# Bioconductor/SparseArray

Hardware: AMD Instinct MI355X
Metric: GNZ/s, SVT crossprod(svt, dense) 1e6x1e4 @1% nnz (higher is better)
Workload: dtype f64

## Files before the change

include/svt_hip.h:

```cpp
#ifndef SVT_HIP_H
#define SVT_HIP_H

#include <stddef.h>
#include <stdint.h>

#ifdef __cplusplus
extern "C" {
#endif

#define SVT_UNSUPPORTED 1

#define SVT_LGLSXP 10
#define SVT_INTSXP 13
#define SVT_REALSXP 14

#define SVT_OP_ANYNA            1
#define SVT_OP_COUNTNAS         2
#define SVT_OP_ANY              3
#define SVT_OP_ALL              4
#define SVT_OP_MIN              5
#define SVT_OP_MAX              6
#define SVT_OP_RANGE            7
#define SVT_OP_SUM              8
#define SVT_OP_PROD             9
// ... 78 lines not shown
int svt_colsum_SVT(const svt_view *x, const int *group, int ngroup, int na_rm,
		   void *out, int *ovflow);
int svt_rowsum_dgCMatrix(int nrow, int ncol, const double *xx, const int *xi,
			 const int *xp, const int *group, int ngroup,
			 int na_rm, double *out);
int svt_colsum_dgCMatrix(int nrow, int ncol, const double *xx, const int *xi,
			 const int *xp, const int *group, int ngroup,
			 int na_rm, double *out);

int svt_colMins_dgCMatrix(int nrow, int ncol, const double *xx, const int *xp,
			  int na_rm, double *out);
int svt_colMaxs_dgCMatrix(int nrow, int ncol, const double *xx, const int *xp,
			  int na_rm, double *out);
int svt_colRanges_dgCMatrix(int nrow, int ncol, const double *xx, const int *xp,
			    int na_rm, double *out);
int svt_colVars_dgCMatrix(int nrow, int ncol, const double *xx, const int *xp,
			  int na_rm, double *out);


typedef struct svt_dev_csc {
	int32_t Rtype;
	int32_t owned;
	int64_t nrow;
	int64_t ncol;
	int64_t nnz;
	int64_t *col_ptr;
	int32_t *row_idx;
	void *val;
	int32_t na_background;
} svt_dev_csc;

svt_dev_csc *svt_upload(const svt_view *x);
svt_dev_csc *svt_wrap_device_csc(int Rtype, int64_t nrow, int64_t ncol,
				 int64_t nnz, int64_t *col_ptr,
				 int32_t *row_idx, void *val);
void svt_release(svt_dev_csc *h);

size_t svt_dev_crossprod_ws_bytes(int64_t nrow, int64_t ncol, int K);
int svt_dev_dense_prepare(const void *Y, int64_t ldY, int64_t nrow, int K,
			  int tr_y, int Rtype, void *ws, size_t ws_bytes,
			  void *stream);
int svt_dev_crossprod_prepared(const svt_dev_csc *A, const void *ws, int K,
			       double *out, int64_t out_stride_c,
			       int64_t out_stride_k, void *stream);
int svt_dev_crossprod_csc_dense(const svt_dev_csc *A, const void *Y,
				int64_t ldY, int K, int tr_y, double *out,
				int64_t out_stride_c, int64_t out_stride_k,
				void *ws, size_t ws_bytes, void *stream);

typedef struct svt_dev_pbc svt_dev_pbc;
svt_dev_pbc *svt_dev_pbc_build(const svt_dev_csc *A, int CBW, int WPB, int logR);
void svt_dev_pbc_release(svt_dev_pbc *P);
void svt_dev_pbc_trim(void);
size_t svt_dev_pbc_bytes(const svt_dev_pbc *P);
size_t svt_dev_crossprod_pbc_ws_bytes(const svt_dev_pbc *P, int K);
int svt_dev_crossprod_pbc(const svt_dev_pbc *P, const svt_dev_csc *A,
			  const double *Y, int64_t ldY, int K, int tr_y,
			  double *out, int64_t out_stride_c,
			  int64_t out_stride_k, void *ws, size_t ws_bytes,
			  void *stream);

void svt_dev_pbc_set_spare_cus(int n);
int svt_dev_pbc_spare_cus(void);

void svt_dev_pbc_set_gather_pacing(int dsync, int spin);

void svt_dev_pbc_set_round_launches(int on);

int svt_dev_crossprod_pbc_from(const svt_dev_pbc *P, const svt_dev_csc *A,
			       const double *Y, int64_t ldY, int K, int tr_y,
			       double *out, int64_t out_stride_c,
			       int64_t out_stride_k, void *ws, size_t ws_bytes,
			       void *stream, int64_t first_col);

enum { SVT_PBC_KERNEL_GENERAL = 0, SVT_PBC_KERNEL_DMA = 1, SVT_PBC_KERNEL_GATHER = 2, SVT_PBC_KERNEL_GATHER2 = 3,
       SVT_PBC_KERNEL_GATHERX = 4 };
typedef struct svt_pbc_plan {
	int kind, kernel, NV, nsplit;
	int64_t panels_per_split;
	int direct, launches, tail_splits, tail_blocks;
} svt_pbc_plan;
int svt_dev_crossprod_pbc_plan(const svt_dev_pbc *P, int K, int tr_y, int64_t out_stride_c,
			       int64_t out_stride_k, int64_t first_col, svt_pbc_plan *plan);

int svt_dev_crossprod_pbc_phase(const svt_dev_pbc *P, const svt_dev_csc *A,
				const double *Y, int64_t ldY, int K, int tr_y,
				double *out, int64_t out_stride_c,
				int64_t out_stride_k, void *ws, size_t ws_bytes,
				void *stream, int phase);

int svt_dev_colstats(const svt_dev_csc *A, int opcode, int na_rm,
		     double center, int64_t inner, void *out, int *warn_flag,
		     void *stream);

int svt_dev_colstats_form(int64_t nseg, int64_t nnz, int *nchunk);

size_t svt_dev_colmedians_ws_bytes(int64_t nnz, int64_t ncol);
int svt_dev_colmedians(const svt_dev_csc *A, int na_rm, double *out, void *ws, size_t ws_bytes,
		       void *stream);

size_t svt_dev_colquantiles_ws_bytes(int64_t nnz, int64_t ncol, int nprobs);
int svt_dev_colquantiles(const svt_dev_csc *A, const double *probs, int nprobs, int na_rm,
			 double *out, void *ws, size_t ws_bytes, void *stream);

size_t svt_dev_colmads_ws_bytes(int64_t nnz, int64_t ncol);
int svt_dev_colmads(const svt_dev_csc *A, const double *center , double constant,
// ... 96 lines not shown
```

sparsearray_amd/_abi.py:

```python
from ctypes import CFUNCTYPE, c_char_p, c_double as D, c_int as I, c_int64 as L, c_size_t as Z, c_void_p as P

ALLOC_FN = CFUNCTYPE(P, Z, P)
FREE_FN = CFUNCTYPE(None, P, P)

PROTOTYPES = {
    "svt_init": (I, [I]),
    "svt_last_error": (c_char_p, []),
    "svt_device_arch": (c_char_p, []),
    "svt_set_devices": (I, [P, I]),
    "svt_get_devices": (I, [P, I]),
    "svt_set_shard_min_nnz": (None, [L]),
    "svt_resident_set_limit": (I, [Z]),
    "svt_resident_clear": (None, []),
    "svt_resident_stats": (None, [P, P, P, P]),
    "svt_crossprod2_SVT_mat": (I, [P, P, I, I, I, I, P]),
    "svt_crossprod2_mat_SVT": (I, [P, I, I, I, P, I, P]),
    "svt_crossprod2_SVT_SVT": (I, [P, P, P]),
    "svt_crossprod1_SVT": (I, [P, P]),
    "svt_matmul_SVT_mat": (I, [P, P, I, I, I, P]),
    "svt_matmul_SVT_SVT": (I, [P, P, P]),
    "svt_tcrossprod1_SVT": (I, [P, P]),
    "svt_tcrossprod2_SVT_SVT": (I, [P, P, P]),
    "svt_colMedians_SVT": (I, [P, I, P]),
    "svt_rowMedians_SVT": (I, [P, I, P]),
    "svt_colQuantiles_SVT": (I, [P, P, I, I, P]),
    "svt_rowQuantiles_SVT": (I, [P, P, I, I, P]),
    "svt_colMads_SVT": (I, [P, P, D, I, P]),
    "svt_rowMads_SVT": (I, [P, P, D, I, P]),
    "svt_colRanks_SVT": (I, [P, I, I, P]),
    "svt_rowRanks_SVT": (I, [P, I, P]),
    "svt_summarize_SVT": (I, [P, I, I, D, P, P, P, P]),
    "svt_colStats_out_Rtype": (I, [I, I]),
    "svt_colStats_SVT": (I, [P, I, I, D, I, P, P]),
    "svt_rowStats_SVT": (I, [P, I, I, P, I, P, P]),
    "svt_rowStatsFull_SVT": (I, [P, I, I, P, I, P, P]),
    "svt_rowsum_SVT": (I, [P, P, I, I, P, P]),
    "svt_colsum_SVT": (I, [P, P, I, I, P, P]),
    "svt_rowsum_dgCMatrix": (I, [I, I, P, P, P, P, I, I, P]),
    "svt_colsum_dgCMatrix": (I, [I, I, P, P, P, P, I, I, P]),
    "svt_colMins_dgCMatrix": (I, [I, I, P, P, I, P]),
    "svt_colMaxs_dgCMatrix": (I, [I, I, P, P, I, P]),
    "svt_colRanges_dgCMatrix": (I, [I, I, P, P, I, P]),
    "svt_colVars_dgCMatrix": (I, [I, I, P, P, I, P]),
    "svt_upload": (P, [P]),
    "svt_wrap_device_csc": (P, [I, L, L, L, P, P, P]),
    "svt_release": (None, [P]),
    "svt_dev_crossprod_ws_bytes": (Z, [L, L, I]),
    "svt_dev_dense_prepare": (I, [P, L, L, I, I, I, P, Z, P]),
    "svt_dev_crossprod_prepared": (I, [P, P, I, P, L, L, P]),
    "svt_dev_crossprod_csc_dense": (I, [P, P, L, I, I, P, L, L, P, Z, P]),
    "svt_dev_pbc_build": (P, [P, I, I, I]),
    "svt_dev_pbc_release": (None, [P]),
    "svt_dev_pbc_trim": (None, []),
    "svt_dev_pbc_bytes": (Z, [P]),
    "svt_dev_crossprod_pbc_ws_bytes": (Z, [P, I]),
    "svt_dev_crossprod_pbc": (I, [P, P, P, L, I, I, P, L, L, P, Z, P]),
    "svt_dev_pbc_set_spare_cus": (None, [I]),
    "svt_dev_pbc_spare_cus": (I, []),
    "svt_dev_pbc_set_gather_pacing": (None, [I, I]),
    "svt_dev_pbc_set_round_launches": (None, [I]),
    "svt_dev_crossprod_pbc_from": (I, [P, P, P, L, I, I, P, L, L, P, Z, P, L]),
    "svt_dev_crossprod_pbc_plan": (I, [P, I, I, L, L, L, P]),
    "svt_dev_crossprod_pbc_phase": (I, [P, P, P, L, I, I, P, L, L, P, Z, P, I]),
    "svt_dev_colstats": (I, [P, I, I, D, L, P, P, P]),
    "svt_dev_colstats_form": (I, [L, L, P]),
    "svt_dev_colmedians_ws_bytes": (Z, [L, L]),
    "svt_dev_colmedians": (I, [P, I, P, P, Z, P]),
    "svt_dev_colquantiles_ws_bytes": (Z, [L, L, I]),
    "svt_dev_colquantiles": (I, [P, P, I, I, P, P, Z, P]),
    "svt_dev_colmads_ws_bytes": (Z, [L, L]),
    "svt_dev_colmads": (I, [P, P, D, I, P, P, Z, P]),
    "svt_dev_colranks_form": (I, [L]),
    "svt_dev_colranks_ws_bytes": (Z, [L, L]),
    "svt_dev_colranks": (I, [P, I, P, P, P, P, Z, P]),
    "svt_dev_rowstats_ws_bytes": (Z, [L, L]),
    "svt_dev_rowsums": (I, [P, I, L, P, P, Z, P]),
    "svt_dev_rowsums_prepare": (I, [P, L, P, Z, P]),
    "svt_dev_rowsums_prepared": (I, [P, I, L, P, P, Z, P]),
    "svt_dev_rowstats_ws_bytes_op": (Z, [P, I, L]),
    "svt_dev_rowstats": (I, [P, I, I, P, L, P, P, P, Z, P]),
    "svt_dev_rowstats_form": (I, [L, L, L, I, I, L, P, P]),
    "svt_dev_rowsum": (I, [P, P, I, I, P, P]),
    "svt_dev_rowsum_gid_bytes": (Z, [P]),
    "svt_dev_rowsum_prepare": (I, [P, P, I, P, Z, P]),
    "svt_dev_rowsum_prepared": (I, [P, P, I, I, P, P]),
    "svt_get_num_procs": (I, []),
    "svt_get_max_threads": (I, []),
    "svt_set_max_threads": (I, [I]),
    "svt_dev_transpose_ws_bytes": (Z, [L, L]),
    "svt_dev_transpose": (I, [P, P, P, P, P, Z, P]),
    "svt_dev_transpose_plan": (I, [L, L, L, L, P]),
    "svt_dev_set_box_nnz": (None, [L]),
    "svt_dev_boxed_calls": (L, [I]),
    "svt_dev_matmul_csc_csc_ws_bytes": (Z, [P]),
    "svt_dev_matmul_csc_csc": (I, [P, P, P, L, P, Z, P, P]),
    "svt_dev_matmul_csc_csc_prepare": (I, [P, P, Z, P]),
    "svt_dev_matmul_csc_csc_prepared": (I, [P, P, P, L, P, Z, P, P]),
    "svt_dev_crossprod_csc_csc_ws_bytes": (Z, [P]),
    "svt_dev_crossprod_csc_csc": (I, [P, P, I, P, L, P, Z, P, P]),
    "svt_dev_crossprod_csc_csc_set_panel": (None, [I, I]),
    "svt_dev_crossprod_csc_csc_dense_buffer": (I, [P, P, P]),
    "svt_sparse_crossprod_set_cost": (None, [D]),
    "svt_dev_aperm_ws_bytes": (Z, [L, I, P]),
    "svt_dev_aperm_perm_ws_bytes": (Z, [L, I, P, P]),
    "svt_dev_aperm": (I, [P, I, P, P, P, P, P, P, Z, P]),
    "svt_dev_aperm_route_counts": (None, [P, I]),
# ... 15 lines not shown
```

sparsearray_amd/csrc/kernels_colstats.hip:

```cpp
#include "svt_common.h"

#define F_NA    1
#define F_NAN   2
#define F_TRUE  4
#define F_ZERO  8
#define F_HAVE 16

template <typename V, typename F>
__device__ inline V grp16(V v, F f)
{
#pragma unroll
	for (int m = 8; m >= 1; m >>= 1) v = f(v, __shfl_xor(v, m, SVT_WAVE));
	return v;
}

template <int NT>
__device__ inline double red_sum(double v, double *sm)
{
	if (NT == 16) return grp16(v, [](double a, double b) { return a + b; });
	v = wave_sum(v);
	if (NT == SVT_WAVE)
		return __shfl(v, 0, SVT_WAVE);
	const int w = threadIdx.x >> 6, l = threadIdx.x & 63;
	__syncthreads();
// ... 444 lines not shown
template <typename T>
__global__ void __launch_bounds__(256)
colstats_thread_kernel(StatsArgs a)
{
	typedef ValTraits<T> VT;
	const bool is_dbl = sizeof(T) == 8;
	const int64_t g = (int64_t) blockIdx.x * blockDim.x + threadIdx.x;
	if (g >= a.nseg) return;
	const T *__restrict__ val = (const T *) a.val;
	const int64_t beg = a.col_ptr[g * a.inner], end = a.col_ptr[(g + 1) * a.inner];
	const int oc = a.opcode;
	const bool narm = a.na_rm != 0;
	const bool is_minmax = oc == SVT_OP_MIN || oc == SVT_OP_MAX, is_min = oc == SVT_OP_MIN;
	ColState st;
	st.flags = 0; st.pad = 0; st.nacnt = 0;
	st.acc = (oc == SVT_OP_PROD) ? 1.0 : 0.0;
	st.mm = is_min ? INFINITY : -INFINITY;
	for (int64_t k = beg; k < end; k++) {
		const T v = val[k];
		if (VT::is_missing(v)) {
			st.nacnt++;
			st.flags |= VT::is_na(v) ? F_NA : F_NAN;
			if (narm || !is_dbl) continue;
		} else {
			st.flags |= (v != (T) 0) ? F_TRUE : F_ZERO;
			st.flags |= F_HAVE;
		}
		const double d = VT::as_double(v);
		if (oc == SVT_OP_PROD) st.acc *= d;
		else if (is_minmax) { if (d == d) st.mm = is_min ? (d < st.mm ? d : st.mm) : (d > st.mm ? d : st.mm); }
		else st.acc += d;
	}
	double c = 0.0, acc2 = 0.0;
	if (oc == SVT_OP_CENTERED_X2_SUM || oc == SVT_OP_VAR1 || oc == SVT_OP_SD1) {
		c = colstats_center(a, st, end - beg);
		for (int64_t k = beg; k < end; k++) {
			const T v = val[k];
			if (VT::is_missing(v) && (narm || !is_dbl)) continue;
			const double d = VT::as_double(v) - c;
			acc2 += d * d;
		}
	}
	colstats_final(a, g, st, end - beg, c, acc2, is_dbl);
}

static int launch_colstats_split(const StatsArgs &a, int nchunk, hipStream_t s)
{
	const bool is_dbl = a.Rtype == SVT_REALSXP;
	const bool two_pass = a.opcode == SVT_OP_CENTERED_X2_SUM || a.opcode == SVT_OP_VAR1 ||
			      a.opcode == SVT_OP_SD1;
	const size_t n = (size_t) a.nseg * nchunk;
	const size_t b_st = (n * sizeof(ColState) + 255) / 256 * 256, b_c = ((size_t) a.nseg * 8 + 255) / 256 * 256;
	char *scr = NULL;
	HIP_TRY(hipMallocAsync((void **) &scr, b_st + b_c + n * 8 + 256, s));
	ColState *st = (ColState *) scr;
	double *centers = (double *) (scr + b_st), *acc2 = (double *) (scr + b_st + b_c);
	dim3 grid((unsigned) nchunk, (unsigned) a.nseg), cgrid((unsigned) ((a.nseg + 255) / 256));
	if (is_dbl) hipLaunchKernelGGL((colstats_chunk_kernel<double, 1>), grid, dim3(256), 0, s, a, nchunk, st, centers, acc2);
	else hipLaunchKernelGGL((colstats_chunk_kernel<int, 1>), grid, dim3(256), 0, s, a, nchunk, st, centers, acc2);
	hipLaunchKernelGGL(colstats_combine_kernel<1>, cgrid, dim3(256), 0, s, a, nchunk, st, centers, acc2,
			   (int) two_pass, (int) is_dbl);
	if (two_pass) {
		if (is_dbl) hipLaunchKernelGGL((colstats_chunk_kernel<double, 2>), grid, dim3(256), 0, s, a, nchunk, st, centers, acc2);
		else hipLaunchKernelGGL((colstats_chunk_kernel<int, 2>), grid, dim3(256), 0, s, a, nchunk, st, centers, acc2);
		hipLaunchKernelGGL(colstats_combine_kernel<2>, cgrid, dim3(256), 0, s, a, nchunk, st, centers, acc2,
				   (int) two_pass, (int) is_dbl);
	}
	HIP_TRY(hipGetLastError());
	HIP_TRY(hipFreeAsync(scr, s));
	return 0;
}

ColStatsRoute colstats_route(int64_t nseg, int64_t nnz)
{
	ColStatsRoute rt = { COLSTATS_LANES16, 1 };
	if (nseg <= 0)
		return rt;
	const int64_t avg = nnz / nseg;
	if (nseg < 512 && avg >= 65536 && nseg <= 65535) {
		int64_t nchunk = (1024 + nseg - 1) / nseg;
		if (nchunk > avg / 16384) nchunk = avg / 16384;
		if (nchunk >= 2) {
			rt.form = COLSTATS_SPLIT;
			rt.nchunk = (int) nchunk;
			return rt;
		}
	}
	if (avg >= 1024)
		rt.form = avg <= 256 * 40 ? COLSTATS_GROUP_CACHED : COLSTATS_GROUP_STREAM;
	else if (avg < 4 && nseg >= 4096)
		rt.form = COLSTATS_THREAD;
	else if (avg < 160)
		rt.form = COLSTATS_LANES16;
	else
		rt.form = COLSTATS_WAVE;
	return rt;
}

template <int NT, int CAP>
static void launch_colstats_form(const StatsArgs &a, hipStream_t s)
{
	const dim3 grid((unsigned) ((a.nseg + 256 / NT - 1) / (256 / NT))), block(256);
	if (a.Rtype == SVT_REALSXP) hipLaunchKernelGGL((colstats_kernel<double, NT, CAP>), grid, block, 0, s, a);
	else hipLaunchKernelGGL((colstats_kernel<int, NT, CAP>), grid, block, 0, s, a);
}

int launch_colstats(const StatsArgs &a, int64_t nnz, hipStream_t s)
{
	if (a.nseg <= 0)
		return 0;
	if (a.nseg > 0x7FFFFFFFLL)
		return svt_set_error("too many generalized columns");
	const ColStatsRoute rt = colstats_route(a.nseg, nnz);
	switch (rt.form) {
	case COLSTATS_SPLIT:
		return launch_colstats_split(a, rt.nchunk, s);
	case COLSTATS_GROUP_CACHED: launch_colstats_form<256, 48>(a, s); break;
	case COLSTATS_GROUP_STREAM: launch_colstats_form<256, 0>(a, s); break;
	case COLSTATS_WAVE: launch_colstats_form<64, 16>(a, s); break;
	case COLSTATS_LANES16: launch_colstats_form<16, 16>(a, s); break;
	case COLSTATS_THREAD: {
		const dim3 gridt((unsigned) ((a.nseg + 255) / 256)), block(256);
// ... 9 lines not shown
```

sparsearray_amd/csrc/kernels_mult_pbc.hip:

```cpp
#include "svt_common.h"

#include <string.h>

#include <mutex>

#include "svt_scan.h"

typedef double d16 __attribute__((ext_vector_type(16)));
typedef double d8 __attribute__((ext_vector_type(8)));

struct svt_dev_pbc {
	int64_t nrow, ncol, nnz, nrec;
	int CBW, WPB, logR;
	int kind;
	int64_t ngroups, nblocks, npanels;
	uint4 *rec;
	int64_t *tile_ptr;
	int *col_has_na;
	int64_t max_leaf_nnz;
	mutable hipStream_t use_s[4];
	mutable int nuse;
	mutable bool use_overflow;
	int device;
};
// ... 325 lines not shown
	}
	__syncthreads();
	if (tid < np) {
		const int start = s_tile0[tid], stop = s_tile0[tid + 1];
		uint32_t *last = (uint32_t *) (dst + ((stop - 8) >> 3) * 96);
		*last |= 0x8000u;
		const int w = (int) (g % 16);
		const int nb = (stop - start) >> 3;
		int bi = (int) pbc_stagger_batch(stag_mode, w, nb);
		if (bi > nb - 1) bi = nb - 1;
		uint32_t *issue = (uint32_t *) (dst + ((start >> 3) + bi) * 96);
		*issue |= 0x4000u;
	}
	if (!in_lds)
		return;
	__syncthreads();
	uint4 *out = (uint4 *) (rec + (base >> 3) * 96);
	for (int64_t i = tid; i < nbytes / 16; i += 256) out[i] = ((const uint4 *) img)[i];
}

__global__ void pbc_max_leaf_kernel(const int64_t *__restrict__ col_ptr, int64_t ncol, unsigned long long *__restrict__ out)
{
	unsigned long long n = 0ULL;
	for (int64_t c = (int64_t) blockIdx.x * blockDim.x + threadIdx.x; c < ncol; c += (int64_t) gridDim.x * blockDim.x) {
		const unsigned long long m = (unsigned long long) (col_ptr[c + 1] - col_ptr[c]);
		n = m > n ? m : n;
	}
	for (int off = 32; off > 0; off >>= 1) {
		const unsigned long long o = __shfl_xor(n, off, 64);
		n = o > n ? o : n;
	}
	if ((threadIdx.x & 63) == 0 && n > 0) atomicMax(out, n);
}

__global__ void pbc_group_limit_kernel(const int64_t *__restrict__ tile_ptr, int64_t npanels,
				       int64_t ngroups, int *__restrict__ flag)
{
	const int64_t g = (int64_t) blockIdx.x * blockDim.x + threadIdx.x;
	if (g >= ngroups) return;
	const int64_t n = tile_ptr[(g + 1) * npanels] - tile_ptr[g * npanels];
	if ((n + PBC_SLACK) * 16 >= ((int64_t) 1 << 32)) *flag = 1;
}

__global__ void pbc_build_finish_kernel(int64_t *__restrict__ tile_ptr, int64_t ntiles, char *__restrict__ rec,
					int rbytes, long long *__restrict__ meta)
{
	const int64_t nrec = tile_ptr[ntiles];
	if (threadIdx.x == 0) meta[0] = nrec;
	if (threadIdx.x < PBC_TP_PAD) tile_ptr[ntiles + 1 + threadIdx.x] = nrec;
	uint32_t *slack = (uint32_t *) (rec + (size_t) nrec * rbytes);
	for (int x = threadIdx.x; x < PBC_SLACK * 4; x += blockDim.x) slack[x] = 0u;
}

#define PBC_POOL_KEEP ((uint64_t) 3 << 30)
#define PBC_MAX_DEV 16
static hipMemPool_t g_pbc_pool[PBC_MAX_DEV];
static bool g_pbc_pool_ok[PBC_MAX_DEV];

static std::mutex g_pbc_pool_mu;

static hipMemPool_t pbc_pool(int dev)
{
	if (dev < 0 || dev >= PBC_MAX_DEV)
		return NULL;
	std::lock_guard<std::mutex> lk(g_pbc_pool_mu);
	if (!g_pbc_pool_ok[dev]) {
		hipMemPoolProps props;
		memset(&props, 0, sizeof(props));
		props.allocType = hipMemAllocationTypePinned;
		props.handleTypes = hipMemHandleTypeNone;
		props.location.type = hipMemLocationTypeDevice;
		props.location.id = dev;
		hipMemPool_t pool = NULL;
		if (hipMemPoolCreate(&pool, &props) != hipSuccess) {
			(void) hipGetLastError();
			return NULL;
		}
		uint64_t keep = PBC_POOL_KEEP;
		(void) hipMemPoolSetAttribute(pool, hipMemPoolAttrReleaseThreshold, &keep);
		g_pbc_pool[dev] = pool;
		g_pbc_pool_ok[dev] = true;
	}
	return g_pbc_pool[dev];
}

static hipError_t pbc_alloc(void **p, size_t n)
{
	int dev = 0;
	(void) hipGetDevice(&dev);
	hipMemPool_t pool = pbc_pool(dev);
	if (pool == NULL)
		return hipMallocAsync(p, n ? n : 16, 0);
	return hipMallocFromPoolAsync(p, n ? n : 16, pool, 0);
}
static void pbc_free(void *p) { if (p) (void) hipFreeAsync(p, 0); }

extern "C" void svt_dev_pbc_trim(void)
{
	for (int d = 0; d < PBC_MAX_DEV; d++)
		if (g_pbc_pool_ok[d])
			(void) hipMemPoolTrimTo(g_pbc_pool[d], 0);
}

static void pbc_note_use(const svt_dev_pbc *P, hipStream_t s)
{
	for (int i = 0; i < P->nuse; i++)
		if (P->use_s[i] == s) return;
	if (P->nuse == 4) { P->use_overflow = true; return; }
	P->use_s[P->nuse++] = s;
}

extern "C" void svt_dev_pbc_release(svt_dev_pbc *h)
{
	if (h == NULL) return;
	bool sync = h->use_overflow;
	for (int i = 0; i < h->nuse && !sync; i++) {
		if (h->use_s[i] == (hipStream_t) 0)
			continue;
		hipEvent_t ev;
		if (hipEventCreateWithFlags(&ev, hipEventDisableTiming) != hipSuccess) { sync = true; break; }
		if (hipEventRecord(ev, h->use_s[i]) != hipSuccess || hipStreamWaitEvent(0, ev, 0) != hipSuccess) {
			(void) hipGetLastError();
			sync = true;
		}
		(void) hipEventDestroy(ev);
	}
	if (sync)
		(void) hipDeviceSynchronize();
	pbc_free(h->rec);
	pbc_free(h->tile_ptr);
	pbc_free(h->col_has_na);
	free(h);
}

extern "C" size_t svt_dev_pbc_bytes(const svt_dev_pbc *h)
{
	if (h == NULL) return 0;
	return (size_t) h->nrec * (h->kind == PBC_KIND_DMA ? 12 : 16) + PBC_SLACK * 16 +
	       (size_t) (h->ngroups * h->npanels + 1 + PBC_TP_PAD) * 8 + (size_t) h->ncol * 4;
}

void pbc_auto_layout(int64_t nrow, int64_t ncol, int64_t nnz, int *CBW, int *WPB, int *logR)
{
	*CBW = 40;
	const double per_tile = (double) nnz * 40.0 * 128.0 /
				((double) (nrow > 0 ? nrow : 1) * (double) (ncol > 0 ? ncol : 1));
	if (per_tile < 12.0 && nrow >= 4096) {
		*WPB = 4;
		*logR = (nrow >> 11) >= 64 ? 11 : (nrow >> 10) >= 64 ? 10 : 9;
	} else { *WPB = 16; *logR = 7; }
}

int pbc_kind(int64_t nrow, int CBW, int WPB, int logR)
{
	if (CBW < 1 || CBW > 40)
		return PBC_KIND_BAD;
	if (WPB == 16 && logR == 7)
		return nrow >= 256 && nrow < ((int64_t) 1 << 28) ? PBC_KIND_DMA : PBC_KIND_NONE;
	return WPB == 4 && logR >= 9 && logR <= 15 ? PBC_KIND_GATHER : PBC_KIND_BAD;
}

extern "C" svt_dev_pbc *svt_dev_pbc_build(const svt_dev_csc *A, int CBW, int WPB, int logR)
{
	if (A->Rtype != SVT_REALSXP) {
		svt_set_error("svt_dev_pbc_build: f64 operands only");
		return NULL;
	}
	if (CBW == 0 && WPB == 0 && logR == 0)
		pbc_auto_layout(A->nrow, A->ncol, A->nnz, &CBW, &WPB, &logR);
	const int kind = pbc_kind(A->nrow, CBW, WPB, logR);
	if (kind == PBC_KIND_BAD) {
		svt_set_error("svt_dev_pbc_build: no product kernel reads the layout (CBW %d, WPB %d, logR %d): "
			      "(CBW <= 40, 16, 7) for the LDS-DMA kernel or (CBW <= 40, 4, 9 .. 15) for the gather kernels",
			      CBW, WPB, logR);
		return NULL;
	}
	svt_dev_pbc *h = (svt_dev_pbc *) calloc(1, sizeof(*h));
	h->nrow = A->nrow; h->ncol = A->ncol; h->nnz = A->nnz;
	h->CBW = CBW; h->WPB = WPB; h->logR = logR;
	h->kind = kind;
	const bool dma = kind == PBC_KIND_DMA;
// ... 36 lines not shown
				(void) hipFuncSetAttribute((const void *) pbc_count_stream_kernel,
							   hipFuncAttributeMaxDynamicSharedMemorySize, (int) lds);
				hipLaunchKernelGGL(pbc_count_stream_kernel, dim3((unsigned) h->ngroups), dim3(1024), lds, 0,
						   A->col_ptr, A->row_idx, A->ncol, CBW, logR, h->npanels, h->tile_ptr,
						   bounds, nchunks, logR + sl);
				bounds_done = true;
			}
		} else if (dma)
			hipLaunchKernelGGL((pbc_pass_kernel<0, 1>), grid, dim3(64), 0, 0, A->col_ptr, A->row_idx,
					   (const double *) A->val, A->ncol, CBW, logR, h->npanels,
					   h->tile_ptr, (uint4 *) NULL, h->col_has_na, g_pbc_stagger, 0);
		else
			hipLaunchKernelGGL((pbc_pass_kernel<0, 0>), grid, dim3(64), 0, 0, A->col_ptr, A->row_idx,
					   (const double *) A->val, A->ncol, CBW, logR, h->npanels,
					   h->tile_ptr, (uint4 *) NULL, h->col_has_na, g_pbc_stagger, 1);
		tmp_bytes = exclusive_scan_ws_bytes(ntiles + 1);
		ok = pbc_alloc(&tmp, tmp_bytes) == hipSuccess &&
		     launch_exclusive_scan_i64(h->tile_ptr, ntiles + 1, tmp, 0) == 0;
		if (ok) ok = pbc_alloc((void **) &h->rec, (size_t) nrec_max * rbytes + PBC_SLACK * 16) == hipSuccess;
		if (ok) {
			if (dma) {
				if (!bounds_done) ok = pbc_alloc((void **) &bounds, (size_t) nb_entries * 4) == hipSuccess;
				if (ok) {
					if (!bounds_done)
						hipLaunchKernelGGL(pbc_bounds_kernel, dim3((unsigned) ((nb_entries + 255) / 256)), dim3(256), 0, 0,
								   A->col_ptr, A->row_idx, A->ncol, nchunks, (int64_t) subp << logR, bounds);
					const size_t lds = PBC_IMG_BYTES + (size_t) 2 * subp * CBW * 4;
					(void) hipFuncSetAttribute((const void *) pbc_scatter_lds_kernel,
								   hipFuncAttributeMaxDynamicSharedMemorySize, (int) lds);
					dim3 sgrid((unsigned) h->ngroups, (unsigned) nchunks);
					hipLaunchKernelGGL(pbc_scatter_lds_kernel, sgrid, dim3(256), lds, 0, A->col_ptr, A->row_idx,
							   (const double *) A->val, A->ncol, CBW, logR, h->npanels,
							   h->tile_ptr, (char *) h->rec, h->col_has_na, g_pbc_stagger, subp,
							   bounds, nchunks);
				}
			} else {
				hipLaunchKernelGGL((pbc_pass_kernel<1, 0>), grid, dim3(64), 0, 0, A->col_ptr,
						   A->row_idx, (const double *) A->val, A->ncol, CBW, logR,
						   h->npanels, h->tile_ptr, h->rec, h->col_has_na, g_pbc_stagger, 1);
			}
		}
		long long hmeta[3] = {0, 0, 0};
		bool too_big = false;
		if (ok) {
			long long *meta = (long long *) tmp;
			ok = hipMemsetAsync(meta, 0, 24, 0) == hipSuccess;
			if (ok) {
				hipLaunchKernelGGL(pbc_max_leaf_kernel, dim3((unsigned) ((A->ncol + 255) / 256 < 512 ? (A->ncol + 255) / 256 : 512)), dim3(256), 0, 0,
						   A->col_ptr, A->ncol, (unsigned long long *) (meta + 1));
				hipLaunchKernelGGL(pbc_group_limit_kernel, dim3((unsigned) ((h->ngroups + 255) / 256)),
						   dim3(256), 0, 0, h->tile_ptr, h->npanels, h->ngroups, (int *) (meta + 2));
				hipLaunchKernelGGL(pbc_build_finish_kernel, dim3(1), dim3(256), 0, 0, h->tile_ptr, ntiles,
						   (char *) h->rec, (int) rbytes, meta);
				ok = hipMemcpy(hmeta, meta, 24, hipMemcpyDeviceToHost) == hipSuccess;
			}
			h->nrec = hmeta[0];
			h->max_leaf_nnz = hmeta[1];
			too_big = hmeta[2] != 0;
		}
		if (ok && too_big) {
			svt_set_error("svt_dev_pbc_build: a column group too large for 32-bit record offsets");
			pbc_free(tmp);
			pbc_free(bounds);
			svt_dev_pbc_release(h);
			return NULL;
		}
	}
	pbc_free(tmp);
	pbc_free(bounds);
	if (!ok) {
		svt_set_error("svt_dev_pbc_build failed: %s", hipGetErrorString(hipGetLastError()));
		svt_dev_pbc_release(h);
		return NULL;
	}
	return h;
}

static int g_pbc_spare_cus = 0;
extern "C" void svt_dev_pbc_set_spare_cus(int n)
{
	g_pbc_spare_cus = n < 0 ? 0 : n > 192 ? 192 : (n + 7) / 8 * 8;
}
extern "C" int svt_dev_pbc_spare_cus(void) { return g_pbc_spare_cus; }
#ifdef SVT_TUNING
extern "C" void svt_dev_pbc_set_debug(int mode)
{
	if (mode >= 300) g_pbc_ahead10 = mode - 300;
	else if (mode >= 200) g_pbc_stagger = mode - 200;
	else if (mode >= 100) g_pbc_nsplit = mode - 100;
	else g_pbc_debug = mode;
}
#endif

struct PbcFlags {
	int *y_nonfinite;
};

#define PBC_SUBFLAG0 16
#define PBC_NSUBFLAG 48
#define PBC_FLAG_BYTES 16384
#define PBC_PROG_OFFSET 8192
#ifdef SVT_TUNING
extern "C" int svt_dev_pbc_read_prof(const void *ws, unsigned long long *out)
{
	HIP_TRY(hipDeviceSynchronize());
	HIP_TRY(hipMemcpy(out, (const char *) ws + 7168, 16 * 8 * 8, hipMemcpyDeviceToHost));
// ... 1311 lines not shown
```

sparsearray_amd/csrc/kernels_rowstats.hip:

```cpp
#include "svt_common.h"

#define RF_NA   1
#define RF_NAN  2
#define RF_HAVE 4
#define RF_TRUE 8
#define RF_ZERO 16

struct MinMaxScratch {
	unsigned long long *best;
	int *flags;
	unsigned int *cov;
};

__host__ __device__ inline MinMaxScratch split_scratch(void *p, int64_t n)
{
	MinMaxScratch s;
	s.best = (unsigned long long *) p;
	s.flags = (int *) (s.best + n);
	s.cov = (unsigned int *) (s.flags + n);
	return s;
}

size_t rowstats_scratch_bytes(int opcode, int64_t out_len)
{
// ... 929 lines not shown
			}
			if (cur == NA_INT)
				continue;
			const long long y = (long long) cur + v;
			if (y > 2147483647LL || y < -2147483647LL) { out[r] = NA_INT; ov = 1; }
			else out[r] = (int) y;
		}
	}
	if (ov && a.ovflow_flag) *a.ovflow_flag = 1;
}

static int groupsum_common(const GroupSumArgs &a, int64_t out_len, bool colsum,
			   hipStream_t s)
{
	const bool is_dbl = a.Rtype == SVT_REALSXP;
	if (out_len <= 0)
		return 0;
	if (is_dbl)
		HIP_TRY(hipMemsetAsync(a.out, 0, (size_t) out_len * 8, s));
	else
		HIP_TRY(hipMemsetAsync(a.scratch, 0, groupsum_scratch_bytes(a.Rtype, out_len), s));
	if (a.ncol > 0) {
		const unsigned nb = (unsigned) ((a.ncol + 3) / 4);
		if (colsum) {
			if (is_dbl) hipLaunchKernelGGL((groupsum_atomic_kernel<double, 1>), dim3(nb), dim3(256), 0, s, a, out_len);
			else hipLaunchKernelGGL((groupsum_atomic_kernel<int, 1>), dim3(nb), dim3(256), 0, s, a, out_len);
		} else {
			if (is_dbl) hipLaunchKernelGGL((groupsum_atomic_kernel<double, 0>), dim3(nb), dim3(256), 0, s, a, out_len);
			else hipLaunchKernelGGL((groupsum_atomic_kernel<int, 0>), dim3(nb), dim3(256), 0, s, a, out_len);
		}
	}
	if (!is_dbl) {
		const int64_t col_len = colsum ? a.nrow : a.ngroup;
		const int64_t ncols_out = colsum ? a.ngroup : a.ncol;
		const unsigned nbo = (unsigned) ((out_len + 255) / 256);
		const unsigned nbc = (unsigned) ((ncols_out + 63) / 64);
		hipLaunchKernelGGL(groupsum_int_finish_kernel, dim3(nbo), dim3(256), 0, s, a, out_len, col_len);
		if (colsum) hipLaunchKernelGGL(groupsum_int_exact_kernel<1>, dim3(nbc), dim3(64), 0, s, a, out_len, ncols_out, col_len);
		else hipLaunchKernelGGL(groupsum_int_exact_kernel<0>, dim3(nbc), dim3(64), 0, s, a, out_len, ncols_out, col_len);
	}
	HIP_TRY(hipGetLastError());
	return 0;
}

__global__ void group16_kernel(const int *__restrict__ g, int64_t n, int ngroup, uint16_t *__restrict__ g16)
{
	const int64_t i = (int64_t) blockIdx.x * blockDim.x + threadIdx.x;
	if (i < n)
		g16[i] = (uint16_t) group_slot16(g[i], ngroup);
}

static int make_group16(const GroupSumArgs &a, uint16_t **g16, hipStream_t s)
{
	HIP_TRY(hipMallocAsync((void **) g16, (size_t) a.nrow * 2 + 16, s));
	hipLaunchKernelGGL(group16_kernel, dim3((unsigned) ((a.nrow + 255) / 256)), dim3(256), 0, s,
			   a.group, a.nrow, a.ngroup, *g16);
	return 0;
}

#define ROWSUM_WIN 49152
template <bool VALS, typename Use>
__device__ __forceinline__ void rowsum_window_walk(const int64_t *__restrict__ col_ptr, const int32_t *__restrict__ row_idx,
						   const double *__restrict__ val, const int64_t ncol, const int64_t nrow,
						   const int64_t j, Use use)
{
	const int lane = threadIdx.x & 63;
	const bool have = j < ncol;
	const int64_t beg = have ? col_ptr[j] : 0, end = have ? col_ptr[j + 1] : 0;
	int64_t k = beg;
	int32_t r = k + lane < end ? row_idx[k + lane] : 0x7FFFFFFF;
	double v = VALS && k + lane < end ? val[k + lane] : 0.0;
	for (int64_t R = ROWSUM_WIN; ; R += ROWSUM_WIN) {
		const int32_t Rc = R < 0x7FFFFFFF ? (int32_t) R : 0x7FFFFFFF;
		for (;;) {
			const bool in = r < Rc;
			const int cnt = __popcll(__ballot(in));
			const int64_t kn = k + cnt;
			const int32_t rn = kn + lane < end ? row_idx[kn + lane] : 0x7FFFFFFF;
			const double vn = VALS && kn + lane < end ? val[kn + lane] : 0.0;
			if (in) use(k + lane, r, v);
			k = kn; r = rn; v = vn;
			if (cnt < 64) break;
		}
		if (R >= nrow) break;
		__syncthreads();
	}
}

template <bool NARM>
__global__ void __launch_bounds__(1024)
rowsum_f64_cols_kernel(const int64_t *__restrict__ col_ptr, const int32_t *__restrict__ row_idx,
		       const double *__restrict__ val, int64_t ncol, int64_t nrow, int ngroup,
		       const uint16_t *__restrict__ g16, double *__restrict__ out, int C)
{
	extern __shared__ double acc[];
	const int w = threadIdx.x >> 6;
	for (int g = threadIdx.x; g < C * ngroup; g += C * 64) acc[g] = 0.0;
	__syncthreads();
	double *mine = acc + w * ngroup;
	rowsum_window_walk<true>(col_ptr, row_idx, val, ncol, nrow, (int64_t) blockIdx.x * C + w,
		[&](const int64_t, const int32_t r, const double v) {
			if (!(NARM && v != v)) atomicAdd(&mine[g16[r]], v);
		});
	__syncthreads();
	for (int g = threadIdx.x; g < C * ngroup; g += C * 64) {
		const int64_t jj = (int64_t) blockIdx.x * C + g / ngroup;
		if (jj < ncol) out[jj * (int64_t) ngroup + g % ngroup] = acc[g];
// ... 43 lines not shown
		const int64_t jj = (int64_t) blockIdx.x * C + g / ngroup;
		if (jj < ncol) out[jj * (int64_t) ngroup + g % ngroup] = acc[g];
	}
}

__global__ void __launch_bounds__(1024)
rowsum_gid_cols_kernel(const int64_t *__restrict__ col_ptr, const int32_t *__restrict__ row_idx, int64_t ncol,
		       int64_t nrow, const uint16_t *__restrict__ g16, uint16_t *__restrict__ gid, int C)
{
	rowsum_window_walk<false>(col_ptr, row_idx, (const double *) NULL, ncol, nrow,
				  (int64_t) blockIdx.x * C + (threadIdx.x >> 6),
				  [&](const int64_t k, const int32_t r, const double) { gid[k] = g16[r]; });
}

static int rowsum_cols_per_wg(int64_t ncol, int cmax, int cmin)
{
	int best = cmax;
	int64_t best_cost = -1;
	for (int c = cmax; c >= cmin; c--) {
		const int64_t nwg = (ncol + c - 1) / c, rounds = (nwg + 255) / 256, cost = rounds * c;
		if (best_cost < 0 || cost < best_cost) { best = c; best_cost = cost; }
	}
	return best;
}

template <typename... P, typename... A>
static void launch_rowsum_cols(int na_rm, void (*narm)(P...), void (*plain)(P...), int64_t ncol, int ngroup, int C,
			       hipStream_t s, A... args)
{
	void (*kernel)(P...) = na_rm ? narm : plain;
	const size_t lds = (size_t) C * ngroup * 8;
	(void) hipFuncSetAttribute((const void *) kernel, hipFuncAttributeMaxDynamicSharedMemorySize, (int) lds);
	hipLaunchKernelGGL(kernel, dim3((unsigned) ((ncol + C - 1) / C)), dim3(C * 64), lds, s, args..., C);
}

static int launch_rowsum_lds(const GroupSumArgs &a, hipStream_t s)
{
	if (a.ncol <= 0 || a.ngroup <= 0)
		return 0;
	if (a.ngroup < 65535 && a.nrow >= 65536) {
		uint16_t *g16 = NULL;
		if (make_group16(a, &g16, s))
			return -1;
		const int64_t cap = (int64_t) (160 * 1024) / ((int64_t) a.ngroup * 8);
		const int cmax = cap > 16 ? 16 : (int) cap;
		if (cmax >= 4 && a.ncol >= 64 && a.col_ptr64 != NULL)
			launch_rowsum_cols(a.na_rm, rowsum_f64_cols_kernel<true>, rowsum_f64_cols_kernel<false>, a.ncol, a.ngroup,
					   rowsum_cols_per_wg(a.ncol, cmax, 4), s, a.col_ptr64, a.row_idx, (const double *) a.val,
					   a.ncol, a.nrow, a.ngroup, (const uint16_t *) g16, (double *) a.out);
		else
			hipLaunchKernelGGL(rowsum_f64_lds_kernel<uint16_t>, dim3((unsigned) a.ncol), dim3(256),
					   (size_t) a.ngroup * 8, s, a, (const uint16_t *) g16);
		HIP_TRY(hipGetLastError());
		HIP_TRY(hipFreeAsync(g16, s));
		return 0;
	}
	hipLaunchKernelGGL(rowsum_f64_lds_kernel<int>, dim3((unsigned) a.ncol), dim3(256),
			   (size_t) a.ngroup * 8, s, a, a.group);
	HIP_TRY(hipGetLastError());
	return 0;
}

int launch_rowsum(const GroupSumArgs &a, hipStream_t s)
{
	if (a.Rtype == SVT_REALSXP && a.col_ptr64 != NULL && a.ngroup <= 8192 && a.ncol > 0 &&
	    a.nnz / a.ncol >= a.ngroup / 4)
		return launch_rowsum_lds(a, s);
	return groupsum_common(a, (int64_t) a.ngroup * a.ncol, false, s);
}

int launch_colsum(const GroupSumArgs &a, hipStream_t s)
{
	return groupsum_common(a, (int64_t) a.ngroup * a.nrow, true, s);
}

int launch_rowsum_gid(const GroupSumArgs &a, uint16_t *gid, hipStream_t s)
{
	if (a.nnz <= 0)
		return 0;
	if (a.col_ptr64 != NULL && a.ncol >= 64 && a.nrow >= 65536 && a.ngroup >= 1 && a.ngroup < 65535) {
		uint16_t *g16 = NULL;
		if (make_group16(a, &g16, s))
			return -1;
		const int C = rowsum_cols_per_wg(a.ncol, 16, 8);
		hipLaunchKernelGGL(rowsum_gid_cols_kernel, dim3((unsigned) ((a.ncol + C - 1) / C)), dim3(C * 64), 0, s,
				   a.col_ptr64, a.row_idx, a.ncol, a.nrow, g16, gid, C);
		HIP_TRY(hipGetLastError());
		HIP_TRY(hipFreeAsync(g16, s));
		return 0;
	}
	int64_t nb = ((a.nnz + 1) / 2 + 255) / 256;
	if (nb > 256 * 32) nb = 256 * 32;
	if (nb < 1) nb = 1;
	hipLaunchKernelGGL(rowsum_gid_kernel, dim3((unsigned) nb), dim3(256), 0, s, a.row_idx, a.nnz, a.group, a.ngroup, gid);
	HIP_TRY(hipGetLastError());
	return 0;
}

int launch_rowsum_prepared(const GroupSumArgs &a, const uint16_t *gid, hipStream_t s)
{
	if (a.ncol <= 0 || a.ngroup <= 0)
		return 0;
	const int64_t cap = (int64_t) (160 * 1024) / ((int64_t) a.ngroup * 8);
	if (cap < 1 || a.col_ptr64 == NULL)
		return 1;
	const int cmax = cap > 16 ? 16 : (int) cap;
	launch_rowsum_cols(a.na_rm, rowsum_f64_gid_kernel<true>, rowsum_f64_gid_kernel<false>, a.ncol, a.ngroup,
			   rowsum_cols_per_wg(a.ncol, cmax, cmax >= 4 ? 4 : 1), s, a.col_ptr64, (const double *) a.val, gid,
			   a.ncol, a.ngroup, (double *) a.out);
	HIP_TRY(hipGetLastError());
	return 0;
}
```

sparsearray_amd/csrc/kernels_transpose.hip:

```cpp
#include "svt_common.h"

#include <string.h>

#include <algorithm>
#include <atomic>
#include <utility>
#include <vector>

#include "svt_scan.h"

#include "svt_sort.h"

__device__ inline int64_t wave_incl_scan_i64(int64_t v)
{
	const int lane = threadIdx.x & 63;
#pragma unroll
	for (int o = 1; o < 64; o <<= 1) {
		const int64_t t = __shfl_up(v, o, SVT_WAVE);
		if (lane >= o) v += t;
	}
	return v;
}

__global__ void __launch_bounds__(SVT_SCAN_NT)
// ... 852 lines not shown
__global__ void __launch_bounds__(256)
box_place_kernel(const int64_t *__restrict__ bptr, const int32_t *__restrict__ bidx, const T *__restrict__ bval,
		 int64_t nleaf, int32_t add, const int64_t *__restrict__ out_ptr, int64_t *__restrict__ fill,
		 int32_t *__restrict__ out_idx, T *__restrict__ out_val)
{
	const int lane = threadIdx.x & 63;
	const int64_t L = (int64_t) blockIdx.x * 4 + (threadIdx.x >> 6);
	if (L >= nleaf) return;
	const int64_t b = bptr[L], n = bptr[L + 1] - b;
	if (n == 0) return;
	const int64_t dst = out_ptr[L] + fill[L];
	for (int64_t k0 = 0; k0 < n; k0 += 256) {
		int32_t r[4];
		T v[4];
#pragma unroll
		for (int u = 0; u < 4; u++) {
			const int64_t k = k0 + u * 64 + lane;
			if (k < n) { r[u] = bidx[b + k]; v[u] = bval[b + k]; }
		}
#pragma unroll
		for (int u = 0; u < 4; u++) {
			const int64_t k = k0 + u * 64 + lane;
			if (k < n) { out_idx[dst + k] = r[u] + add; out_val[dst + k] = v[u]; }
		}
	}
	if (lane == 0) fill[L] += n;
}

static void launch_box_place(int Rtype, const int64_t *bptr, const int32_t *bidx, const void *bval, int64_t nleaf,
			     int64_t first, const int64_t *out_ptr, int64_t *fill, int32_t *out_idx, void *out_val, hipStream_t s)
{
	svt_by_rtype(Rtype, bval, out_val, [&](auto *v, auto *o) {
		hipLaunchKernelGGL(box_place_kernel, dim3((unsigned) ((nleaf + 3) / 4)), dim3(256), 0, s, bptr, bidx, v, nleaf,
				   (int32_t) first, out_ptr, fill, out_idx, o);
	});
}

typedef std::vector<std::pair<int64_t, int64_t>> BoxBounds;
template <class F>
static int box_boundaries(const char *who, const int64_t *ptr, int64_t n, int64_t nnz, int64_t bsz, int64_t W,
			  int64_t npts_max, int64_t *pts, hipStream_t s, BoxBounds *bd, F queue_more)
{
	const int64_t nk = (nnz - 1) / bsz, nw = (n - 1) / W, npts = nk + nw;
	if (npts > npts_max)
		return svt_set_error("%s: internal error (box cuts)", who);
	std::vector<int64_t> hp((size_t) npts * 3 + 1);
	if (npts > 0) {
		hipLaunchKernelGGL(box_cut_kernel, dim3((unsigned) ((npts + 255) / 256)), dim3(256), 0, s, ptr, n, nk, bsz, W, npts, pts);
		HIP_TRY(hipGetLastError());
		HIP_TRY(hipMemcpyAsync(hp.data(), pts, (size_t) npts * 24, hipMemcpyDeviceToHost, s));
	}
	if (queue_more())
		return -1;
	HIP_TRY(hipStreamSynchronize(s));
	bd->reserve((size_t) npts * 2 + 2);
	bd->push_back({0, 0});
	bd->push_back({n, nnz});
	for (int64_t i = 0; i < npts; i++) {
		bd->push_back({hp[3 * i], hp[3 * i + 1]});
		bd->push_back({hp[3 * i] + 1, hp[3 * i + 2]});
	}
	std::sort(bd->begin(), bd->end());
	bd->erase(std::unique(bd->begin(), bd->end()), bd->end());
	return 0;
}

size_t transpose_ws_bytes_box(int64_t nrow, int64_t nnz, int64_t box_limit)
{
	if (!box_taken(nnz, box_limit))
		return transpose_ws_bytes(nrow, nnz);
	return box_layout(nrow, nnz, box_limit).total;
}

static int launch_transpose_boxed(const int64_t *col_ptr, const int32_t *row_idx, const void *val, int Rtype,
				  int64_t nrow, int64_t ncol, int64_t nnz, int64_t *out_ptr, int32_t *out_idx,
				  void *out_val, void *ws, int64_t box_limit, hipStream_t s)
{
	if (ncol > 0x7FFFFFFFLL)
		return svt_set_error("svt_dev_transpose: more than 2^31-1 columns");
	const BoxLayout Ly = box_layout(nrow, nnz, box_limit);
	char *w = (char *) ws;
	int64_t *pts = (int64_t *) (w + Ly.pts), *fill = (int64_t *) (w + Ly.fill);
	int64_t *bcp = (int64_t *) (w + Ly.bcp), *bptr = (int64_t *) (w + Ly.bptr);
	int32_t *bidx = (int32_t *) (w + Ly.bidx);
	void *bval = w + Ly.bval, *rws = w + Ly.route;
	const size_t esz = Rtype == SVT_REALSXP ? 8 : 4;
	HIP_TRY(hipMemsetAsync(out_ptr, 0, (size_t) (nrow + 1) * 8, s));
	HIP_TRY(hipMemsetAsync(fill, 0, (size_t) nrow * 8, s));
	bool lds = nrow <= BOX_HIST_LDS;
	if (lds && hipFuncSetAttribute((const void *) box_row_hist_kernel, hipFuncAttributeMaxDynamicSharedMemorySize,
				       BOX_HIST_LDS * 4) != hipSuccess) {
		(void) hipGetLastError();
		lds = false;
	}
	int64_t nbh = (nnz + BOX_HIST_NT * 4 - 1) / (BOX_HIST_NT * 4);
	if (nbh > 1024) nbh = 1024;
	hipLaunchKernelGGL(box_row_hist_kernel, dim3((unsigned) nbh), dim3(BOX_HIST_NT), lds ? (size_t) nrow * 4 : 0, s,
			   row_idx, nnz, nrow, lds ? 1 : 0, (unsigned long long *) out_ptr);
	HIP_TRY(hipGetLastError());
	if (launch_exclusive_scan_i64(out_ptr, nrow + 1, w + Ly.scan, s))
		return -1;
	BoxBounds bd;
	if (box_boundaries("svt_dev_transpose", col_ptr, ncol, nnz, Ly.bsz, Ly.W, Ly.npts_max, pts, s, &bd, [] { return 0; }))
		return -1;
	for (size_t b = 0; b + 1 < bd.size(); b++) {
		const int64_t c0 = bd[b].first, c1 = bd[b + 1].first, p0 = bd[b].second, nb = bd[b + 1].second - p0;
		if (nb == 0)
// ... 410 lines not shown
	const int64_t lp0 = g * d0;
#pragma unroll
	for (int u = 0; u < SLAB_ITEMS; u++) {
		const int sidx = u * SLAB_NT + tid;
		if (sidx >= n) continue;
		const int e = (int) (pay[u] & 8191u), k = (int) (pay[u] >> 13);
		out_idx[sb + sidx] = k;
		out_val[sb + sidx] = val[lbeg[k] + (e - off[k])];
		const int64_t i = key[u], prev = sidx > 0 ? (int64_t) skey[sidx - 1] : -1;
		for (int64_t ii = prev + 1; ii <= i; ii++) out_ptr[lp0 + ii] = sb + sidx;
	}
	const int64_t last = n > 0 ? (int64_t) skey[n - 1] : -1;
	for (int64_t ii = last + 1 + tid; ii < d0; ii += SLAB_NT) out_ptr[lp0 + ii] = sb + n;
	if (g == nslab - 1 && tid == 0) out_ptr[nslab * d0] = nnz;
}

struct SlabHead { size_t cnt, maxcnt, scan, total; };
static SlabHead aperm_slab_head(int64_t nslab)
{
	const size_t maxcnt = t2_a((size_t) (nslab + 2), 8);
	return SlabHead{0, maxcnt, maxcnt + 256, maxcnt + 256 + exclusive_scan_ws_bytes(nslab + 1)};
}

static int aperm_slab(const ApermCall &c)
{
	const int ndim = c.ndim, *perm = c.perm;
	const int64_t *dim = c.dim, nnz = c.nnz;
	if (!(ndim >= 3 && perm[1] == 0 && perm[0] >= 1 && dim[perm[0]] <= 1024 && dim[0] < ((int64_t) 1 << 30)))
		return APERM_NA;
	const int q = perm[0];
	int64_t os[8], st = 1;
	for (int a = 1; a < ndim; a++) { os[a] = st; st *= dim[a]; }
	SlabMap sm;
	sm.nother = ndim - 2;
	int64_t nslab = 1;
	for (int t = 0; t < ndim - 2; t++) {
		sm.new_ext[t] = dim[perm[2 + t]];
		sm.old_stride[t] = os[perm[2 + t]];
		nslab *= dim[perm[2 + t]];
	}
	if (!(nslab >= 1 && nslab < 2147483646LL && nnz / nslab <= SLAB_CAP * 9 / 10))
		return APERM_NA;
	const SlabHead H = aperm_slab_head(nslab);
	if (H.total > aperm_sort32_layout(nnz).ktmp)
		return APERM_NA;
	char *w = (char *) c.ws;
	int64_t *base = (int64_t *) (w + H.cnt);
	unsigned long long *maxcnt = (unsigned long long *) (w + H.maxcnt), mx = 0;
	hipStream_t s = c.s;
	HIP_TRY(hipMemsetAsync(maxcnt, 0, 8, s));
	hipLaunchKernelGGL(aperm_slab_count_kernel, dim3((unsigned) ((nslab + 1 + 255) / 256)), dim3(256), 0, s,
			   c.col_ptr, sm, nslab, dim[q], os[q], base, maxcnt);
	HIP_TRY(hipMemcpyAsync(&mx, maxcnt, 8, hipMemcpyDeviceToHost, s));
	HIP_TRY(hipStreamSynchronize(s));
	if (mx > SLAB_CAP) {
		g_route[R_SLAB_REFUSED]++;
		return APERM_REFUSED;
	}
	g_route[R_SLAB]++;
	if (launch_exclusive_scan_i64(base, nslab + 1, w + H.scan, s))
		return -1;
	const int bits = key_bits(dim[0]);
	svt_by_rtype(c.Rtype, c.val, c.out_val, [&](auto *v, auto *o) {
		hipLaunchKernelGGL(aperm_slab_kernel, dim3((unsigned) nslab), dim3(SLAB_NT), (size_t) SLAB_CAP * 4, s, c.col_ptr,
				   c.row_idx, v, sm, nslab, dim[0], (int) dim[q], os[q], bits, nnz, base, c.out_ptr, c.out_idx, o);
	});
	HIP_TRY(hipGetLastError());
	return 0;
}

static size_t aperm_swap01_bytes(int64_t nnz, const int64_t *dim, int ndim, T2Shape *sh, size_t *reserve)
{
	if (ndim < 3 || nnz <= 0 || nnz >= ((int64_t) 1 << 31))
		return 0;
	const double ns = extent_prod(dim, 2, ndim, -1, false);
	if (ns < 1.0 || ns > 1.0e9)
		return 0;
	if (!t2_shape(dim[0], dim[1], nnz, sh, (int64_t) ns))
		return 0;
	const size_t res = t2_a(t2_head(*sh).total + 256, 1);
	if (reserve) *reserve = res;
	return t2_body(res, (size_t) nnz, (size_t) (sh->ncoarse + 1) * (size_t) (sh->nslab * sh->scol)).total;
}

extern "C" int svt_dev_transpose_plan(int64_t nrow, int64_t ncol, int64_t nnz, int64_t nslab, int64_t out[8])
{
	if (out == NULL || nslab < 1)
		return svt_set_error("svt_dev_transpose_plan: NULL result or nslab < 1");
	T2Shape sh;
	memset(&sh, 0, sizeof(sh));
	int why;
	if (nnz <= 0 || nnz >= ((int64_t) 1 << 31)) {
		why = 1;
	} else if (nslab == 1) {
		size_t reserve = 0;
		why = t_route(nrow, ncol, nnz, &sh, &reserve);
	} else {
		const int64_t dim[3] = {nrow, ncol, nslab};
		why = aperm_swap01_bytes(nnz, dim, 3, &sh, NULL) > 0 ? 0 : 1;
	}
	out[0] = why == 0;
	out[1] = why == 1 ? -1 : sh.fbits;
	out[2] = why == 1 ? -1 : sh.cbits;
	out[3] = why == 1 ? 0 : sh.nfb;
	out[4] = why == 1 ? 0 : sh.ncoarse;
	out[5] = why == 1 ? 0 : sh.ngroups;
	out[6] = (key_bits(nrow) + 7) / 8;
// ... 505 lines not shown
```

sparsearray_amd/csrc/svt_common.h:

```cpp
#pragma once

#include <hip/hip_runtime.h>
#include <stdint.h>

#include "../../include/svt_hip.h"

#define SVT_WAVE 64
#define NA_INT (-2147483647 - 1)

__host__ __device__ inline double svt_na_real()
{
	union { unsigned long long u; double d; } x;
	x.u = 0x7FF00000000007A2ULL;
	return x.d;
}
__host__ __device__ inline bool svt_is_na(double v)
{
	union { double d; unsigned long long u; } x;
	x.d = v;
	return v != v && (unsigned int) (x.u & 0xFFFFFFFFu) == 1954u;
}
__host__ __device__ inline bool svt_is_finite(double v)
{
	union { double d; unsigned long long u; } x;
// ... 30 lines not shown
	for (int o = 32; o > 0; o >>= 1) {
		double t = __shfl_down(v, o, SVT_WAVE);
		v = t < v ? t : v;
	}
	return v;
}
__device__ inline double wave_max(double v)
{
	for (int o = 32; o > 0; o >>= 1) {
		double t = __shfl_down(v, o, SVT_WAVE);
		v = t > v ? t : v;
	}
	return v;
}
__device__ inline int wave_min_i(int v)
{
	for (int o = 32; o > 0; o >>= 1) {
		int t = __shfl_down(v, o, SVT_WAVE);
		v = t < v ? t : v;
	}
	return v;
}
__device__ inline int wave_max_i(int v)
{
	for (int o = 32; o > 0; o >>= 1) {
		int t = __shfl_down(v, o, SVT_WAVE);
		v = t > v ? t : v;
	}
	return v;
}

__device__ inline unsigned long long f64_to_ordered(double v)
{
	unsigned long long u = (unsigned long long) __double_as_longlong(v);
	return (u >> 63) ? ~u : (u | 0x8000000000000000ULL);
}
__device__ inline double ordered_to_f64(unsigned long long u)
{
	u = (u >> 63) ? (u & 0x7FFFFFFFFFFFFFFFULL) : ~u;
	return __longlong_as_double((long long) u);
}

int svt_set_error(const char *fmt, ...);
int svt_set_unsupported(const char *fmt, ...);
void svt_clear_unsupported(void);
#define HIP_TRY(expr)                                                         \
	do {                                                                  \
		hipError_t e__ = (expr);                                      \
		if (e__ != hipSuccess)                                        \
			return svt_set_error("%s failed: %s (%s:%d)", #expr, \
					     hipGetErrorString(e__),         \
					     __FILE__, __LINE__);             \
	} while (0)

template <class F>
static inline void svt_by_rtype(int Rtype, const void *in, void *out, F &&f)
{
	if (Rtype == SVT_REALSXP) f((const double *) in, (double *) out);
	else f((const int32_t *) in, (int32_t *) out);
}

struct StatsArgs {
	const int64_t *col_ptr;
	const void *val;
	int Rtype;
	int64_t nseg;
	int64_t inner;
	int64_t seg_len;
	int opcode;
	int na_rm;
	double center;
	void *out;
	int *warn_flag;
	int na_bg;
	int dgc;
};
enum {
	COLSTATS_THREAD = 0,
	COLSTATS_LANES16 = 1,
	COLSTATS_WAVE = 2,
	COLSTATS_GROUP_CACHED = 3,
	COLSTATS_GROUP_STREAM = 4,
	COLSTATS_SPLIT = 5
};
struct ColStatsRoute {
	int form;
	int nchunk;
};
ColStatsRoute colstats_route(int64_t nseg, int64_t nnz);
int launch_colstats(const StatsArgs &a, int64_t nnz, hipStream_t s);
enum { ORDER_MEDIANS = 0, ORDER_QUANTILES = 1, ORDER_MADS = 2 };
size_t order_stat_ws_bytes(int what, int64_t ncol);
int launch_order_stat(int what, const int64_t *col_ptr, const void *val, int Rtype, int64_t nrow, int64_t ncol,
		      int64_t nnz, const double *vec, int nprobs, double constant, int na_rm, double *out, void *ws,
		      hipStream_t s);
int ranks_form(int64_t col_nnz);
size_t ranks_ws_bytes(int64_t ncol, int64_t long_nnz);
int launch_ranks(const int64_t *col_ptr, const void *val, int Rtype, int64_t nrow, int64_t ncol, int64_t nnz, int ties,
		 void *rank_nz, void *zero_rank, int *flag, void *ws, size_t ws_bytes, hipStream_t s);

struct RowStatsArgs {
	const int64_t *col_ptr;
	const int32_t *row_idx;
	const void *val;
	int Rtype;
	int64_t ncol;
// ... 143 lines not shown
```

sparsearray_amd/csrc/svt_hip.cpp:

```cpp
#include "svt_common.h"
#include <unistd.h>

#include <stdarg.h>
#include <stdio.h>
#include <stdlib.h>
#include <string.h>

#include <algorithm>
#include <atomic>
#include <chrono>
#include <functional>
#include <mutex>
#include <thread>
#include <vector>

static thread_local char g_err[1024];
static int g_device = -1;
static char g_arch[64] = "";

int svt_set_error(const char *fmt, ...)
{
	va_list ap;
	va_start(ap, fmt);
	vsnprintf(g_err, sizeof(g_err), fmt, ap);
	va_end(ap);
	return -1;
}

static thread_local int g_unsupported = 0;
int svt_set_unsupported(const char *fmt, ...)
{
	va_list ap;
	va_start(ap, fmt);
	vsnprintf(g_err, sizeof(g_err), fmt, ap);
	va_end(ap);
	g_unsupported = 1;
	return -1;
}
void svt_clear_unsupported(void) { g_unsupported = 0; }
static inline int svt_status(int rc)
{
	return rc < 0 && g_unsupported ? 1 : rc;
}
template <class F> static int abi_status(F f)
{
	g_unsupported = 0;
	return svt_status(f());
}

extern "C" const char *svt_last_error(void) { return g_err; }
extern "C" const char *svt_device_arch(void) { return g_arch; }

static int select_device(int device)
{
	int n = 0;
	if (hipGetDeviceCount(&n) != hipSuccess || n <= 0)
		return svt_set_error("libsvt_hip: no HIP device visible -- the SVT "
				     "backend has no CPU fallback");
	if (device < 0 || device >= n)
		return svt_set_error("libsvt_hip: device %d out of range (0..%d)",
				     device, n - 1);
	HIP_TRY(hipSetDevice(device));
	hipDeviceProp_t prop;
	HIP_TRY(hipGetDeviceProperties(&prop, device));
	snprintf(g_arch, sizeof(g_arch), "%s", prop.gcnArchName);
	if (strncmp(g_arch, "gfx950", 6) != 0)
// ... 50 lines not shown
		}
	if (select_device(ordinals[0])) {
		if (g_device >= 0) (void) hipSetDevice(g_device);
		return -1;
	}
	g_devices.assign(ordinals, ordinals + n);
	return 0;
}

extern "C" int svt_get_devices(int *ordinals, int cap)
{
	const int n = (int) g_devices.size();
	for (int i = 0; i < n && i < cap; i++)
		if (ordinals) ordinals[i] = g_devices[(size_t) i];
	return n;
}

extern "C" void svt_set_shard_min_nnz(int64_t nnz)
{
	g_shard_min_nnz = nnz > 0 ? nnz : 0;
}

struct ShardCtx {
	int slot, nshard, device;
};
static thread_local const ShardCtx *t_shard = NULL;

static int cur_device() { return t_shard ? t_shard->device : g_device; }

static int g_max_threads = 0;
extern "C" int svt_get_num_procs(void)
{
	const long n = sysconf(_SC_NPROCESSORS_ONLN);
	return n > 0 ? (int) n : 0;
}
extern "C" int svt_get_max_threads(void)
{
	return g_max_threads > 0 ? g_max_threads : svt_get_num_procs();
}
extern "C" int svt_set_max_threads(int nthread)
{
	const int prev = svt_get_max_threads();
	if (nthread > 0) g_max_threads = nthread;
	return prev;
}

static int ensure_init()
{
	if (g_device >= 0)
		return 0;
	return svt_init(0);
}

struct Stager {
	static const size_t CHUNK = (size_t) 48 << 20;
	size_t chunk = CHUNK;
	int dev = -1;
	char *buf[2] = {NULL, NULL};
	hipEvent_t done[2];
	hipStream_t stream = NULL;
	bool ok = false;
	int next = 0;
	bool busy[2] = {false, false};

	int init()
	{
		if (ok) return 0;
		for (int i = 0; i < 2; i++) {
			HIP_TRY(hipHostMalloc((void **) &buf[i], chunk, hipHostMallocDefault));
			HIP_TRY(hipEventCreateWithFlags(&done[i], hipEventDisableTiming));
		}
		HIP_TRY(hipStreamCreateWithFlags(&stream, hipStreamNonBlocking));
		ok = true;
		return 0;
	}
	int acquire(char **p, int *slot)
	{
		if (init()) return -1;
		const int i = next;
		next ^= 1;
		if (busy[i]) { HIP_TRY(hipEventSynchronize(done[i])); busy[i] = false; }
		*p = buf[i]; *slot = i;
		return 0;
	}
	int send(int slot, void *dst, size_t off_in_buf, size_t n)
	{
		if (n) HIP_TRY(hipMemcpyAsync(dst, buf[slot] + off_in_buf, n, hipMemcpyHostToDevice, stream));
		return 0;
	}
	int commit(int slot)
	{
		HIP_TRY(hipEventRecord(done[slot], stream));
		busy[slot] = true;
		return 0;
	}
	int drain()
	{
		if (!ok) return 0;
		HIP_TRY(hipStreamSynchronize(stream));
		busy[0] = busy[1] = false;
		return 0;
	}
	void use(size_t bytes, int d)
	{
		if (ok && (bytes != chunk || d != dev)) {
			(void) hipStreamSynchronize(stream);
			(void) hipStreamDestroy(stream);
			for (int i = 0; i < 2; i++) {
				(void) hipEventDestroy(done[i]);
				(void) hipHostFree(buf[i]);
				buf[i] = NULL;
			}
			ok = false;
			next = 0;
			busy[0] = busy[1] = false;
		}
		chunk = bytes;
		dev = d;
	}
};
static Stager g_stager;
static Stager g_shard_stager[SVT_MAX_SHARDS];
static Stager &cur_stager() { return t_shard ? g_shard_stager[t_shard->slot] : g_stager; }

static size_t g_stager_chunk()
{
	static size_t v = 0;
	if (v == 0) {
		v = Stager::CHUNK;
		const char *e = getenv("SVT_STAGING_CHUNK");
		if (e != NULL) {
			const long long t = atoll(e);
			if (t >= 4096 && (size_t) t < Stager::CHUNK) v = (size_t) t / 4096 * 4096;
		}
	}
	return v < cur_stager().chunk ? v : cur_stager().chunk;
}

static void team_run(int nt, const std::function<void(int, int)> &fn)
{
	std::vector<std::thread> th;
	for (int t = 1; t < nt; t++) th.emplace_back(fn, t, nt);
	fn(0, nt);
	for (auto &x : th) x.join();
}

static int team_size(size_t bytes)
{
	int nt = svt_get_max_threads();
	if (t_shard) nt /= t_shard->nshard;
	if (nt > 8) nt = 8;
	if (bytes < ((size_t) 4 << 20) || nt < 1) nt = 1;
	return nt;
}

static int staged_copy(void *dst, const void *src, size_t n)
{
	if (n < ((size_t) 1 << 20)) {
		if (n) HIP_TRY(hipMemcpy(dst, src, n, hipMemcpyHostToDevice));
		return 0;
	}
	Stager &st = cur_stager();
	for (size_t off = 0; off < n; off += st.chunk) {
		const size_t len = n - off < st.chunk ? n - off : st.chunk;
		char *b; int slot;
		if (st.acquire(&b, &slot)) return -1;
		const char *s0 = (const char *) src + off;
		team_run(team_size(len), [&](int t, int nt) {
			const size_t a = len * t / nt, e = len * (t + 1) / nt;
			memcpy(b + a, s0 + a, e - a);
		});
		if (st.send(slot, (char *) dst + off, 0, len) || st.commit(slot)) return -1;
	}
	return st.drain();
}

static int staged_copy_2d(void *dst, const void *src, size_t run, size_t ncols, size_t ld)
{
	if (run == ld || ncols <= 1)
		return staged_copy(dst, src, run * ncols);
	const size_t n = run * ncols;
	Stager &st = cur_stager();
	for (size_t off = 0; off < n; off += st.chunk) {
		const size_t len = n - off < st.chunk ? n - off : st.chunk;
		char *b; int slot;
		if (st.acquire(&b, &slot)) return -1;
		team_run(team_size(len), [&](int t, int nt) {
			size_t a = off + len * t / nt;
			const size_t e = off + len * (t + 1) / nt;
			while (a < e) {
				const size_t c = a / run, in = a - c * run;
				const size_t m = std::min(run - in, e - a);
				memcpy(b + (a - off), (const char *) src + c * ld + in, m);
				a += m;
			}
		});
		if (st.send(slot, (char *) dst + off, 0, len) || st.commit(slot)) return -1;
	}
	return st.drain();
}

static int staged_download(void *dst, const void *src, size_t n)
{
	if (n < ((size_t) 4 << 20)) {
		if (n) HIP_TRY(hipMemcpy(dst, src, n, hipMemcpyDeviceToHost));
		return 0;
	}
	Stager &st = cur_stager();
	if (st.init() || st.drain()) return -1;
	HIP_TRY(hipDeviceSynchronize());
	const size_t C = st.chunk;
	const size_t nchunk = (n + C - 1) / C;
	for (size_t c = 0; c <= nchunk; c++) {
		if (c < nchunk) {
			const size_t off = c * C, len = n - off < C ? n - off : C;
			HIP_TRY(hipMemcpyAsync(st.buf[c & 1], (const char *) src + off, len,
					       hipMemcpyDeviceToHost, st.stream));
			HIP_TRY(hipEventRecord(st.done[c & 1], st.stream));
		}
		if (c > 0) {
			const size_t off = (c - 1) * C, len = n - off < C ? n - off : C;
			HIP_TRY(hipEventSynchronize(st.done[(c - 1) & 1]));
			const char *b = st.buf[(c - 1) & 1];
			char *d0 = (char *) dst + off;
			team_run(team_size(len), [&](int t, int nt) {
				const size_t a = len * t / nt, e = len * (t + 1) / nt;
				memcpy(d0 + a, b + a, e - a);
			});
		}
	}
	return 0;
}

struct DevBuf {
	void *p = nullptr;
	size_t bytes = 0;
	DevBuf() {}
	DevBuf(const DevBuf &) = delete;
	~DevBuf() { if (p) (void) hipFree(p); }
	int alloc(size_t n)
	{
		if (n == 0) n = 16;
		HIP_TRY(hipMalloc(&p, n));
		bytes = n;
		return 0;
	}
	int upload(const void *src, size_t n)
	{
		if (alloc(n)) return -1;
		return staged_copy(p, src, n);
	}
	int zero()
	{
		HIP_TRY(hipMemset(p, 0, bytes));
		return 0;
	}
	template <typename T> T *as() { return (T *) p; }
};

static size_t elt_size(int Rtype) { return Rtype == SVT_REALSXP ? 8 : 4; }

static int check_view(const svt_view *x)
{
	if (x == NULL || x->ndim < 1 || x->dim == NULL)
		return svt_set_error("invalid svt_view");
	if (x->Rtype != SVT_REALSXP && x->Rtype != SVT_INTSXP &&
	    x->Rtype != SVT_LGLSXP)
		return svt_set_error("does not support SparseArray objects of "
				     "type code %d", x->Rtype);
	int64_t n = 1;
	for (int a = 1; a < x->ndim; a++) n *= x->dim[a];
	if (n != x->nleaves)
		return svt_set_error("svt_view: nleaves does not match dim");
	return 0;
}

static int check_leaves(const svt_view *x)
{
	if (x->svt_is_null) return 0;
	const int dim0 = x->dim[0];
	for (int64_t j = 0; j < x->nleaves; j++) {
		const int c = x->nzcount[j];
		if (c < 0 || c > dim0)
			return svt_set_error("invalid SVT leaf (nzcount %d, dim %d)", c, dim0);
		if (c > 0 && x->nzoffs[j] == NULL)
			return svt_set_error("invalid SVT leaf (NULL nzoffs)");
	}
	return 0;
}

extern "C" svt_dev_csc *svt_upload(const svt_view *x)
{
	if (ensure_init() || check_view(x))
		return NULL;
	const int64_t n = x->nleaves;
	const size_t esz = elt_size(x->Rtype);
	const int dim0 = x->dim[0];
	std::vector<int64_t> col_ptr((size_t) n + 1, 0);
	for (int64_t j = 0; j < n; j++) {
		const int c = x->svt_is_null ? 0 : x->nzcount[j];
		if (c < 0 || c > dim0) {
			svt_set_error("invalid SVT leaf (nzcount %d, dim %d)", c, dim0);
			return NULL;
		}
		if (c > 0 && x->nzoffs[j] == NULL) {
			svt_set_error("invalid SVT leaf (NULL nzoffs)");
			return NULL;
		}
		col_ptr[j + 1] = col_ptr[j] + c;
	}
	svt_dev_csc *d = (svt_dev_csc *) calloc(1, sizeof(*d));
	d->Rtype = x->Rtype;
	d->owned = 1;
	d->na_background = x->na_background != 0;
	d->nrow = dim0;
	d->ncol = n;
	d->nnz = col_ptr[(size_t) n];
	const size_t nn = (size_t) (d->nnz > 0 ? d->nnz : 1);
	if (hipMalloc((void **) &d->col_ptr, (size_t) (d->ncol + 1) * 8) != hipSuccess ||
	    hipMalloc((void **) &d->row_idx, nn * 4) != hipSuccess ||
	    hipMalloc(&d->val, nn * esz) != hipSuccess) {
		svt_set_error("hipMalloc failed while uploading an SVT (%lld nnz)",
			      (long long) d->nnz);
		svt_release(d);
		return NULL;
	}
	bool ok = hipMemcpy(d->col_ptr, col_ptr.data(), (size_t) (d->ncol + 1) * 8,
			    hipMemcpyHostToDevice) == hipSuccess;
	const int64_t cap = (int64_t) (g_stager_chunk() / (4 + esz));
	const int64_t nnz = d->nnz;
	Stager &st = cur_stager();
	for (int64_t k0 = 0; ok && k0 < nnz; k0 += cap) {
		const int64_t cnt = nnz - k0 < cap ? nnz - k0 : cap;
		char *b; int slot;
		if (st.acquire(&b, &slot)) { ok = false; break; }
		int32_t *so = (int32_t *) b;
		char *sv = b + (size_t) cnt * 4;
		team_run(team_size((size_t) cnt * (4 + esz)), [&](int t, int nt) {
			const int64_t ka = k0 + cnt * t / nt, kb = k0 + cnt * (t + 1) / nt;
			if (ka >= kb) return;
			int64_t j = std::upper_bound(col_ptr.begin(), col_ptr.end(), ka) - col_ptr.begin() - 1;
			for (; j < n && col_ptr[j] < kb; j++) {
				const int64_t a = col_ptr[j] > ka ? col_ptr[j] : ka;
				const int64_t e = col_ptr[j + 1] < kb ? col_ptr[j + 1] : kb;
				if (e <= a) continue;
				const int64_t in_leaf = a - col_ptr[j], s = a - k0, c = e - a;
				memcpy(so + s, x->nzoffs[j] + in_leaf, (size_t) c * 4);
				const void *v = x->nzvals[j];
				if (v != NULL) {
					memcpy(sv + (size_t) s * esz, (const char *) v + (size_t) in_leaf * esz,
					       (size_t) c * esz);
				} else if (esz == 8) {
					double *o = (double *) sv + s;
					for (int64_t k = 0; k < c; k++) o[k] = 1.0;
				} else {
					int *o = (int *) sv + s;
					for (int64_t k = 0; k < c; k++) o[k] = 1;
				}
			}
		});
		ok = st.send(slot, d->row_idx + k0, 0, (size_t) cnt * 4) == 0 &&
		     st.send(slot, (char *) d->val + (size_t) k0 * esz, (size_t) cnt * 4,
				   (size_t) cnt * esz) == 0 &&
		     st.commit(slot) == 0;
	}
	if (ok) ok = st.drain() == 0;
	if (!ok) {
		if (svt_last_error()[0] == '\0') svt_set_error("H2D copy failed");
		svt_release(d);
		return NULL;
	}
	return d;
}

extern "C" svt_dev_csc *svt_wrap_device_csc(int Rtype, int64_t nrow, int64_t ncol,
					    int64_t nnz, int64_t *col_ptr,
					    int32_t *row_idx, void *val)
{
	svt_dev_csc *d = (svt_dev_csc *) calloc(1, sizeof(*d));
	d->Rtype = Rtype;
	d->owned = 0;
	d->nrow = nrow;
	d->ncol = ncol;
	d->nnz = nnz;
	d->col_ptr = col_ptr;
	d->row_idx = row_idx;
	d->val = val;
	return d;
}

extern "C" void svt_release(svt_dev_csc *h)
{
	if (h == NULL)
		return;
	if (h->owned) {
		if (h->col_ptr) (void) hipFree(h->col_ptr);
		if (h->row_idx) (void) hipFree(h->row_idx);
		if (h->val) (void) hipFree(h->val);
	}
	free(h);
}

struct Resident {
	uint64_t key;
	svt_dev_csc *csc;
	svt_dev_pbc *pbc;
	svt_dev_csc *tr;
	svt_dev_pbc *tr_pbc;
	size_t bytes;
	uint64_t stamp;
	int pins;
};
static std::vector<Resident> g_res;
static std::mutex g_res_mu;
static size_t g_res_limit = 0, g_res_bytes = 0;
static uint64_t g_res_clock = 0, g_res_hits = 0, g_res_misses = 0;

static size_t csc_bytes(const svt_dev_csc *c)
{
	return (size_t) (c->ncol + 1) * 8 + (size_t) c->nnz * (4 + elt_size(c->Rtype));
}

static size_t pbc_bytes(const svt_dev_pbc *P) { return svt_dev_pbc_bytes(P); }

static void resident_free(Resident &r)
{
	if (r.pbc) svt_dev_pbc_release(r.pbc);
	if (r.tr_pbc) svt_dev_pbc_release(r.tr_pbc);
	svt_release(r.tr);
	svt_release(r.csc);
}

static void resident_make_room(size_t need)
{
	while (g_res_bytes + need > g_res_limit) {
		int victim = -1;
		for (size_t i = 0; i < g_res.size(); i++)
			if (g_res[i].pins == 0 && (victim < 0 || g_res[i].stamp < g_res[victim].stamp))
				victim = (int) i;
		if (victim < 0) return;
		g_res_bytes -= g_res[victim].bytes;
		resident_free(g_res[victim]);
		g_res.erase(g_res.begin() + victim);
	}
}

extern "C" int svt_resident_set_limit(size_t bytes)
{
// ... 14 lines not shown

extern "C" void svt_resident_stats(size_t *bytes, int64_t *entries, int64_t *hits, int64_t *misses)
{
	std::lock_guard<std::mutex> lk(g_res_mu);
	if (bytes) *bytes = g_res_bytes;
	if (entries) *entries = (int64_t) g_res.size();
	if (hits) *hits = (int64_t) g_res_hits;
	if (misses) *misses = (int64_t) g_res_misses;
}

static inline uint64_t fp_mix(uint64_t h, uint64_t v)
{
	h ^= v + 0x9E3779B97F4A7C15ULL + (h << 6) + (h >> 2);
	h *= 0xFF51AFD7ED558CCDULL;
	return h ^ (h >> 33);
}

static uint64_t view_fingerprint(const svt_view *x)
{
	uint64_t h = fp_mix(0x5356545F48495031ULL, (uint64_t) x->Rtype);
	h = fp_mix(h, (uint64_t) x->ndim);
	for (int a = 0; a < x->ndim; a++) h = fp_mix(h, (uint64_t) x->dim[a]);
	h = fp_mix(h, (uint64_t) x->svt_is_null * 2 + (uint64_t) (x->na_background != 0));
	h = fp_mix(h, (uint64_t) x->nleaves);
	if (x->svt_is_null) return h;
	const size_t esz = elt_size(x->Rtype);
	for (int64_t j = 0; j < x->nleaves; j++) {
		const int n = x->nzcount[j];
		h = fp_mix(h, (uint64_t) n);
		if (n <= 0) continue;
		h = fp_mix(h, (uint64_t) (uintptr_t) x->nzoffs[j]);
		h = fp_mix(h, (uint64_t) (uintptr_t) x->nzvals[j]);
		int at[8];
		for (int t = 0; t < 8; t++) at[t] = (int) ((int64_t) (n - 1) * t / 7);
		for (int t = 0; t < 8; t++) {
			uint64_t v = (uint64_t) (uint32_t) x->nzoffs[j][at[t]];
			if (x->nzvals[j] != NULL) {
				uint64_t bits = 0;
				memcpy(&bits, (const char *) x->nzvals[j] + (size_t) at[t] * esz, esz);
				v ^= bits * 0x9E3779B97F4A7C15ULL;
			}
			h = fp_mix(h, v);
		}
	}
	return h;
}

struct CscGuard {
	svt_dev_csc *h;
	uint64_t key;
	explicit CscGuard(svt_dev_csc *p) : h(p), key(0) {}
	explicit CscGuard(const svt_view *x) : h(NULL), key(0)
	{
		if (g_res_limit == 0) { h = svt_upload(x); return; }
		if (check_view(x) || check_leaves(x)) return;
		const uint64_t k = view_fingerprint(x) | 1;
		{
			std::lock_guard<std::mutex> lk(g_res_mu);
			for (Resident &r : g_res)
				if (r.key == k) {
					r.pins++; r.stamp = ++g_res_clock; g_res_hits++;
					h = r.csc; key = k;
					return;
				}
			g_res_misses++;
		}
		h = svt_upload(x);
		if (h == NULL) return;
		std::lock_guard<std::mutex> lk(g_res_mu);
		const size_t nb = csc_bytes(h);
		resident_make_room(nb);
		if (g_res_bytes + nb > g_res_limit) return;
		Resident r = { k, h, NULL, NULL, NULL, nb, ++g_res_clock, 1 };
		g_res.push_back(r);
		g_res_bytes += nb;
		key = k;
	}
	~CscGuard()
	{
		if (key == 0) { svt_release(h); return; }
		std::lock_guard<std::mutex> lk(g_res_mu);
		for (Resident &r : g_res)
			if (r.key == key) { r.pins--; return; }
	}
	void drop()
	{
		if (key == 0) { svt_release(h); h = NULL; }
	}
	CscGuard(const CscGuard &) = delete;
	CscGuard &operator=(const CscGuard &) = delete;
};

static int resident_find(const svt_dev_csc *A)
{
	for (size_t i = 0; i < g_res.size(); i++)
		if (g_res[i].csc == A || g_res[i].tr == A) return (int) i;
	return -1;
}

static svt_dev_pbc *pbc_for(const svt_dev_csc *A, int *owned)
{
	*owned = 1;
	{
		std::lock_guard<std::mutex> lk(g_res_mu);
		for (Resident &r : g_res)
			if (r.csc == A || r.tr == A) {
				svt_dev_pbc *&slot = r.csc == A ? r.pbc : r.tr_pbc;
// ... 349 lines not shown
	return form;
}

extern "C" size_t svt_dev_transpose_ws_bytes(int64_t nrow, int64_t nnz)
{
	return transpose_ws_bytes_box(nrow, nnz, box_nnz_get());
}

static int dev_transpose_impl(const svt_dev_csc *A, int64_t *out_col_ptr, int32_t *out_row_idx,
				 void *out_val, void *ws, size_t ws_bytes, void *stream)
{
	const int64_t box = box_nnz_get();
	if (ws_bytes < transpose_ws_bytes_box(A->nrow, A->nnz, box))
		return svt_set_error("svt_dev_transpose: workspace too small");
	return launch_transpose_box(A->col_ptr, A->row_idx, A->val, A->Rtype, A->nrow, A->ncol, A->nnz,
				    out_col_ptr, out_row_idx, out_val, ws, box, (hipStream_t) stream);
}

extern "C" void svt_dev_set_box_nnz(int64_t n)
{
	box_nnz_set(n);
}

extern "C" int64_t svt_dev_boxed_calls(int reset)
{
	return boxed_calls(reset);
}
extern "C" int svt_dev_transpose(const svt_dev_csc *A, int64_t *out_col_ptr, int32_t *out_row_idx,
				 void *out_val, void *ws, size_t ws_bytes, void *stream)
{
	return abi_status([&] { return dev_transpose_impl(A, out_col_ptr, out_row_idx, out_val, ws, ws_bytes, stream); });
}

enum { SUBSET_GATHER = 0, SUBSET_FILTER = 1, SUBSET_GENERAL = 2 };
static std::atomic<int64_t> g_subset_route[3];

extern "C" int svt_dev_subset_tile(void)
{
	return subset_tile();
}

extern "C" void svt_dev_subset_route_counts(int64_t *counts, int reset)
{
	for (int i = 0; i < 3; i++) {
		if (counts) counts[i] = g_subset_route[i].load();
		if (reset) g_subset_route[i] = 0;
	}
}

static int subset_read_head(const void *ws, hipStream_t s, int *flag, int64_t *total)
{
	int64_t head[2] = { 0, 0 };
	HIP_TRY(hipMemcpyAsync(head, ws, sizeof(head), hipMemcpyDeviceToHost, s));
	HIP_TRY(hipStreamSynchronize(s));
	*flag = (int) (head[0] & 0xFFFFFFFFLL);
	*total = head[1];
	return 0;
}

extern "C" size_t svt_dev_subset_cols_ws_bytes(int64_t ncols_sel)
{
	return subset_cols_ws_bytes(ncols_sel);
}

static int dev_subset_cols_count_impl(const svt_dev_csc *A, const int32_t *cols, int64_t ncols_sel, int64_t *out_col_ptr,
				      int64_t *out_nnz, void *ws, size_t ws_bytes, void *stream)
{
	if (ncols_sel < 0 || ncols_sel > 0x7FFFFFFELL)
		return svt_set_error("svt_dev_subset_cols_count: between 0 and 2^31-2 columns");
	if (ws_bytes < subset_cols_ws_bytes(ncols_sel))
		return svt_set_error("svt_dev_subset_cols_count: workspace too small");
	if (ncols_sel == 0) {
		HIP_TRY(hipMemsetAsync(out_col_ptr, 0, 8, (hipStream_t) stream));
		*out_nnz = 0;
		return 0;
	}
	if (launch_subset_cols_count(A->col_ptr, A->ncol, cols, ncols_sel, out_col_ptr, ws, (hipStream_t) stream))
		return -1;
	int flag = 0;
	int64_t total = 0;
	if (subset_read_head(ws, (hipStream_t) stream, &flag, &total))
		return -1;
	if (flag)
		return svt_set_error("subscript out of bounds");
	*out_nnz = total;
	return 0;
}
extern "C" int svt_dev_subset_cols_count(const svt_dev_csc *A, const int32_t *cols, int64_t ncols_sel, int64_t *out_col_ptr,
					 int64_t *out_nnz, void *ws, size_t ws_bytes, void *stream)
{
	return abi_status([&] { return dev_subset_cols_count_impl(A, cols, ncols_sel, out_col_ptr, out_nnz, ws, ws_bytes, stream); });
}

static int dev_subset_cols_fill_impl(const svt_dev_csc *A, const int32_t *cols, int64_t ncols_sel, const int64_t *out_col_ptr,
				     int32_t *out_row_idx, void *out_val, void *stream)
{
	g_subset_route[SUBSET_GATHER]++;
	if (ncols_sel <= 0 || A->nnz == 0)
		return 0;
	return launch_subset_cols_fill(A->col_ptr, A->row_idx, A->val, A->Rtype, A->ncol, A->nnz, cols, ncols_sel, out_col_ptr,
				       out_row_idx, out_val, (hipStream_t) stream);
}
extern "C" int svt_dev_subset_cols_fill(const svt_dev_csc *A, const int32_t *cols, int64_t ncols_sel, const int64_t *out_col_ptr,
					int32_t *out_row_idx, void *out_val, void *stream)
{
	return abi_status([&] { return dev_subset_cols_fill_impl(A, cols, ncols_sel, out_col_ptr, out_row_idx, out_val, stream); });
}
// ... 339 lines not shown
	if (ndim < 1 || ndim > 8)
		return aperm_ws_bytes_box(nnz, dim, ndim, box_nnz_get());
	for (int a = 0; a < ndim; a++) perm0[a] = perm[a] - 1;
	return aperm_perm_ws_bytes_box(nnz, dim, ndim, perm0, box_nnz_get());
}

static int dev_aperm_impl(const svt_dev_csc *A, int ndim, const int64_t *dim, const int *perm,
			     int64_t *out_col_ptr, int32_t *out_row_idx, void *out_val,
			     void *ws, size_t ws_bytes, void *stream)
{
	int perm0[8];
	if (aperm_args(ndim, perm, perm0))
		return -1;
	int64_t nl = 1;
	for (int a = 1; a < ndim; a++) nl *= dim[a];
	if (dim[0] != A->nrow || nl != A->ncol)
		return svt_set_error("aperm: 'dim' does not match the operand");
	const int64_t box = box_nnz_get();
	if (ws_bytes < aperm_perm_ws_bytes_box(A->nnz, dim, ndim, perm0, box))
		return svt_set_error("svt_dev_aperm: workspace too small");
	return launch_aperm_box(A->col_ptr, A->row_idx, A->val, A->Rtype, A->ncol, A->nnz, dim, ndim,
				perm0, out_col_ptr, out_row_idx, out_val, ws, box, (hipStream_t) stream);
}
extern "C" int svt_dev_aperm(const svt_dev_csc *A, int ndim, const int64_t *dim, const int *perm,
			     int64_t *out_col_ptr, int32_t *out_row_idx, void *out_val,
			     void *ws, size_t ws_bytes, void *stream)
{
	return abi_status([&] { return dev_aperm_impl(A, ndim, dim, perm, out_col_ptr, out_row_idx, out_val, ws, ws_bytes, stream); });
}

static int aperm_SVT_impl(const svt_view *x, const int *perm, int64_t *out_col_ptr,
			     int32_t *out_row_idx, void *out_val)
{
	if (ensure_init() || check_view(x))
		return -1;
	int perm0[8];
	if (aperm_args(x->ndim, perm, perm0))
		return -1;
	int64_t dim[8], new_nl = 1;
	for (int a = 0; a < x->ndim; a++) dim[a] = x->dim[a];
	for (int a = 1; a < x->ndim; a++) new_nl *= dim[perm0[a]];
	CscGuard A(x);
	if (A.h == NULL) return -1;
	const size_t esz = elt_size(x->Rtype);
	const size_t nn = (size_t) (A.h->nnz > 0 ? A.h->nnz : 1);
	const int64_t box = box_nnz_get();
	DevBuf P, I, V, W;
	if (P.alloc((size_t) (new_nl + 1) * 8) || I.alloc(nn * 4) || V.alloc(nn * esz) ||
	    W.alloc(aperm_perm_ws_bytes_box(A.h->nnz, dim, x->ndim, perm0, box)))
		return -1;
	if (launch_aperm_box(A.h->col_ptr, A.h->row_idx, A.h->val, A.h->Rtype, A.h->ncol, A.h->nnz, dim,
			     x->ndim, perm0, P.as<int64_t>(), I.as<int32_t>(), V.p, W.p, box, 0))
		return -1;
	HIP_TRY(hipMemcpy(out_col_ptr, P.p, (size_t) (new_nl + 1) * 8, hipMemcpyDeviceToHost));
	if (A.h->nnz) {
		if (staged_download(out_row_idx, I.p, (size_t) A.h->nnz * 4) ||
		    staged_download(out_val, V.p, (size_t) A.h->nnz * esz))
			return -1;
	}
	return 0;
}
extern "C" int svt_aperm_SVT(const svt_view *x, const int *perm, int64_t *out_col_ptr,
			     int32_t *out_row_idx, void *out_val)
{
	return abi_status([&] { return aperm_SVT_impl(x, perm, out_col_ptr, out_row_idx, out_val); });
}

static GroupSumArgs groupsum_args(const svt_dev_csc *A, const int32_t *col_ptr32, const int *group, int ngroup,
				  int na_rm, void *out)
{
	GroupSumArgs a;
	memset(&a, 0, sizeof(a));
	a.col_ptr64 = col_ptr32 ? NULL : A->col_ptr; a.col_ptr32 = col_ptr32;
	a.row_idx = A->row_idx; a.val = A->val; a.Rtype = A->Rtype;
	a.nrow = A->nrow; a.ncol = A->ncol; a.nnz = A->nnz;
	a.group = group; a.ngroup = ngroup; a.na_rm = na_rm; a.out = out;
	return a;
}

extern "C" int svt_dev_rowsum(const svt_dev_csc *A, const int *group, int ngroup,
			      int na_rm, double *out, void *stream)
{
	if (A->Rtype != SVT_REALSXP)
		return svt_set_error("svt_dev_rowsum: f64 input only");
	return launch_rowsum(groupsum_args(A, NULL, group, ngroup, na_rm, out), (hipStream_t) stream);
}

extern "C" size_t svt_dev_rowsum_gid_bytes(const svt_dev_csc *A)
{
	return (size_t) (A->nnz > 0 ? A->nnz : 1) * 2 + 16;
}

extern "C" int svt_dev_rowsum_prepare(const svt_dev_csc *A, const int *group, int ngroup, void *gid,
				      size_t gid_bytes, void *stream)
{
	if (ngroup < 1 || ngroup > 65535)
		return svt_set_error("svt_dev_rowsum_prepare: between 1 and 65535 groups");
	if (gid_bytes < svt_dev_rowsum_gid_bytes(A))
		return svt_set_error("svt_dev_rowsum_prepare: id buffer too small");
	return launch_rowsum_gid(groupsum_args(A, NULL, group, ngroup, 0, NULL), (uint16_t *) gid, (hipStream_t) stream);
}

extern "C" int svt_dev_rowsum_prepared(const svt_dev_csc *A, const void *gid, int ngroup, int na_rm,
				       double *out, void *stream)
{
	if (A->Rtype != SVT_REALSXP)
		return svt_set_error("svt_dev_rowsum: f64 input only");
	if (ngroup < 1 || ngroup > 65535)
		return svt_set_error("svt_dev_rowsum_prepared: between 1 and 65535 groups");
	if ((int64_t) ngroup * 8 > 160 * 1024)
		return svt_set_error("svt_dev_rowsum_prepared: more groups than a workgroup's LDS holds (20480)");
	const int rc = launch_rowsum_prepared(groupsum_args(A, NULL, NULL, ngroup, na_rm, out), (const uint16_t *) gid,
					      (hipStream_t) stream);
// ... 57 lines not shown
}

struct SubView {
	svt_view v;
	int32_t dim[2];
	std::vector<int32_t> cnt;
	std::vector<const int32_t *> offs;
	std::vector<const void *> vals;
};

static void row_block_view(const svt_view *x, int r0, int r1, SubView &sv)
{
	sv.v = *x;
	sv.dim[0] = r1 - r0;
	sv.dim[1] = x->dim[1];
	sv.v.dim = sv.dim;
	if (x->svt_is_null) return;
	const size_t n = (size_t) x->nleaves, esz = elt_size(x->Rtype);
	sv.cnt.assign(n, 0);
	sv.offs.assign(n, NULL);
	sv.vals.assign(n, NULL);
	for (size_t j = 0; j < n; j++) {
		const int c = x->nzcount[j];
		if (c <= 0) continue;
		const int32_t *o = x->nzoffs[j];
		const int32_t *lo = std::lower_bound(o, o + c, r0), *hi = std::lower_bound(lo, o + c, r1);
		sv.cnt[j] = (int32_t) (hi - lo);
		sv.offs[j] = lo;
		if (x->nzvals[j] != NULL) sv.vals[j] = (const char *) x->nzvals[j] + (size_t) (lo - o) * esz;
	}
	sv.v.nzcount = sv.cnt.data();
	sv.v.nzoffs = sv.offs.data();
	sv.v.nzvals = sv.vals.data();
}

static void col_block_view(const svt_view *x, int64_t c0, int64_t c1, SubView &sv)
{
	sv.v = *x;
	sv.v.ndim = 2;
	sv.dim[0] = x->dim[0];
	sv.dim[1] = (int32_t) (c1 - c0);
	sv.v.dim = sv.dim;
	sv.v.nleaves = c1 - c0;
	if (x->svt_is_null) return;
	sv.v.nzcount = x->nzcount + c0;
	sv.v.nzoffs = x->nzoffs + c0;
	sv.v.nzvals = x->nzvals + c0;
}

static svt_dev_csc *row_block_upload(const svt_view *x, int64_t r0, int64_t r1)
{
	SubView sv;
	row_block_view(x, (int) r0, (int) r1, sv);
	svt_dev_csc *d = svt_upload(&sv.v);
	if (d == NULL || r0 == 0) return d;
	if (launch_rebase_rows(d->row_idx, d->nnz, (int32_t) r0, 0) || hipStreamSynchronize(0) != hipSuccess) {
		if (svt_last_error()[0] == '\0') svt_set_error("device error while rebasing a row block");
		svt_release(d);
		return NULL;
	}
	return d;
}

static void shard_rows(int64_t nrow, int s, int N, int64_t *r0, int64_t *r1)
{
	const int64_t units = (nrow + 127) / 128, base = units / N, rem = units % N;
	const int64_t u0 = s * base + (s < rem ? s : rem), u1 = u0 + base + (s < rem ? 1 : 0);
	*r0 = u0 * 128 < nrow ? u0 * 128 : nrow;
	*r1 = u1 * 128 < nrow ? u1 * 128 : nrow;
}

static std::vector<int64_t> shard_cuts(const svt_view *x, int64_t unit, int64_t nunits, int N)
{
	std::vector<int64_t> pre((size_t) nunits + 1, 0);
	for (int64_t u = 0; u < nunits; u++) {
		int64_t w = 1;
		if (!x->svt_is_null)
			for (int64_t j = u * unit; j < (u + 1) * unit; j++) w += x->nzcount[j];
		pre[(size_t) u + 1] = pre[(size_t) u] + w;
	}
	const int64_t total = pre[(size_t) nunits];
	std::vector<int64_t> cut((size_t) N + 1, nunits);
	cut[0] = 0;
	for (int s = 1; s < N; s++) {
		const int64_t target = total / N * s + total % N * s / N;
		cut[(size_t) s] = std::lower_bound(pre.begin(), pre.end(), target) - pre.begin();
		if (cut[(size_t) s] > nunits) cut[(size_t) s] = nunits;
		if (cut[(size_t) s] < cut[(size_t) s - 1]) cut[(size_t) s] = cut[(size_t) s - 1];
	}
	return cut;
}

struct ShardBufs {
	std::vector<void *> p;
	std::vector<int> dev;
	explicit ShardBufs(const std::vector<int> &devs) : p(devs.size(), nullptr), dev(devs) {}
	~ShardBufs()
	{
		for (size_t s = 0; s < p.size(); s++)
			if (p[s] && hipSetDevice(dev[s]) == hipSuccess) (void) hipFree(p[s]);
		if (g_device >= 0) (void) hipSetDevice(g_device);
	}
	ShardBufs(const ShardBufs &) = delete;
	ShardBufs &operator=(const ShardBufs &) = delete;
};

static int check_mult_view(const svt_view *x, const char *what)
{
	if (check_view(x))
		return -1;
	if (x->ndim != 2)
		return svt_set_error("%s must have 2 dimensions", what);
	if (x->Rtype != SVT_REALSXP && x->Rtype != SVT_INTSXP)
		return svt_set_error("input type is not supported yet");
	if (x->na_background)
		return svt_set_error("NaArray objects are not supported by this operation");
	return 0;
}

static int chunk_K(int64_t nrow, int64_t K)
{
	const int64_t budget = (int64_t) 1 << 30;
	int64_t kc = budget / (8 * (nrow > 0 ? nrow : 1));
	kc = kc / 64 * 64;
	if (kc < 64) kc = 64;
	if (kc > K) kc = K;
	return (int) kc;
}

static bool pbc_shape_ok(int64_t nrow, int64_t ncol, int64_t nnz)
{
	int cbw, wpb, logr;
	pbc_auto_layout(nrow, ncol, nnz, &cbw, &wpb, &logr);
	if (pbc_kind(nrow, cbw, wpb, logr) <= PBC_KIND_NONE)
		return false;
	const int64_t cb = (int64_t) cbw * wpb;
	const double ngroups = (double) ((ncol + cb - 1) / cb) * (double) wpb;
	const double npanels = (double) ((nrow + ((int64_t) 1 << logr) - 1) >> logr);
	const double ntiles = ngroups * npanels;
	return ntiles + 1.0 < 2147483647.0 && (double) nnz >= 4.0 * ntiles;
}

static bool pbc_applies(const svt_dev_csc *A, int64_t K)
{
	return A->ncol > 0 && (double) A->nnz * (double) K >= 268435456.0 && pbc_shape_ok(A->nrow, A->ncol, A->nnz);
}

struct PbcAhead {
	std::thread th;
	svt_dev_pbc *P = NULL;
	int own = 1;
	bool started = false, taken = false;
	void start(const svt_dev_csc *A, int64_t K)
// ... 16 lines not shown
	~PbcAhead()
	{
		if (th.joinable()) th.join();
		if (P && own && !taken) svt_dev_pbc_release(P);
	}
};

static int widen_int(DevBuf &dst, const void *src, int64_t n)
{
	if (dst.alloc((size_t) (n > 0 ? n : 1) * 8))
		return -1;
	return launch_int_to_f64((const int *) src, n, dst.as<double>(), 0);
}

struct Widened {
	svt_dev_csc view;
	DevBuf val;
	int widen(const svt_dev_csc *A)
	{
		if (widen_int(val, A->val, A->nnz))
			return -1;
		view = *A;
		view.Rtype = SVT_REALSXP; view.val = val.p; view.owned = 0;
		return 0;
	}
};

static int dev_crossprod_chunked(const svt_dev_csc *A, const void *Y_dev, int64_t ldY,
				 int64_t K, int tr_y, double *out_dev,
				 int64_t sc, int64_t sk, PbcAhead *ahead = NULL)
{
	if (K <= 0 || A->ncol <= 0)
		return 0;
	if (A->Rtype == SVT_INTSXP && !tr_y && ldY == A->nrow && pbc_applies(A, K)) {
		Widened Af;
		DevBuf Yf;
		if (Af.widen(A) || widen_int(Yf, Y_dev, A->nrow * K))
			return -1;
		return dev_crossprod_chunked(&Af.view, Yf.p, ldY, K, 0, out_dev, sc, sk, NULL);
	}
	if (A->Rtype == SVT_REALSXP && pbc_applies(A, K)) {
		int own_P = 1;
		svt_dev_pbc *P = (ahead && ahead->started) ? ahead->get(&own_P) : pbc_for(A, &own_P);
		if (P == NULL)
			goto general;
		const int kc = K < 512 ? (int) K : 512;
		DevBuf ws;
		int rc = ws.alloc(svt_dev_crossprod_pbc_ws_bytes(P, kc));
		for (int64_t k0 = 0; rc == 0 && k0 < K; k0 += kc) {
			const int kn = (int) (K - k0 < kc ? K - k0 : kc);
			rc = svt_dev_crossprod_pbc(P, A, (const double *) Y_dev + (tr_y ? k0 : k0 * ldY), ldY, kn,
						   tr_y, out_dev + k0 * sk, sc, sk, ws.p, ws.bytes, 0);
		}
		if (rc == 0 && hipDeviceSynchronize() != hipSuccess)
			rc = svt_set_error("device error in the panel-blocked crossprod");
		if (own_P) svt_dev_pbc_release(P);
		return rc;
	}
general:
	const int kc = chunk_K(A->nrow, K);
	DevBuf ws;
	if (ws.alloc(crossprod_ws_bytes(A->nrow, A->ncol, kc)))
		return -1;
	const size_t esz = elt_size(A->Rtype);
	for (int64_t k0 = 0; k0 < K; k0 += kc) {
		const int kn = (int) (K - k0 < kc ? K - k0 : kc);
		const char *Yc = (const char *) Y_dev +
			(tr_y ? (size_t) k0 : (size_t) k0 * (size_t) ldY) * esz;
		if (svt_dev_crossprod_csc_dense(A, Yc, ldY, kn, tr_y,
						out_dev + k0 * sk, sc, sk,
						ws.p, ws.bytes, 0))
			return -1;
	}
	HIP_TRY(hipDeviceSynchronize());
	return 0;
}

template <class PutY>
static int dense_product(const svt_dev_csc *A, int64_t K, int y_Rtype, size_t y_elems, PutY put_y, int64_t ldY,
			 int tr_y, double *O, int64_t sc, int64_t sk)
{
	PbcAhead ahead;
	ahead.start(A, K);
	DevBuf Y;
	if (Y.alloc(y_elems * elt_size(y_Rtype)) || put_y(Y.p))
		return -1;
	const void *Yp = Y.p;
	Widened Aw;
	DevBuf Yw;
	if (A->Rtype != y_Rtype) {
		if (A->Rtype == SVT_INTSXP) {
			if (Aw.widen(A)) return -1;
			A = &Aw.view;
		} else {
			if (widen_int(Yw, Y.p, (int64_t) y_elems)) return -1;
			Yp = Yw.p;
		}
	}
	return dev_crossprod_chunked(A, Yp, ldY, K, tr_y, O, sc, sk, &ahead);
}

static bool mult_types_ok(int a, int b)
{
	return (a == SVT_REALSXP || a == SVT_INTSXP) && (b == SVT_REALSXP || b == SVT_INTSXP);
}

static int crossprod2_SVT_mat_sharded(const svt_view *x, const void *y, int y_nrow, int y_ncol, int y_Rtype,
				      int tr_y, double *out)
{
	if (check_leaves(x))
		return -1;
	const std::vector<int> devs = g_devices;
	const int N = (int) devs.size();
	const int64_t nrow = x->dim[0], ncol = x->dim[1], K = tr_y ? y_nrow : y_ncol;
	const size_t out_n = (size_t) ncol * (size_t) K, ysz = elt_size(y_Rtype);
	ShardBufs part(devs);
	const bool timing = getenv("SVT_SHARD_TIMING") != NULL;
	std::vector<double> t_up((size_t) N, 0.0), t_mul((size_t) N, 0.0), t_red((size_t) N, 0.0);
	auto ms_since = [](std::chrono::steady_clock::time_point t0) {
		return std::chrono::duration<double, std::milli>(std::chrono::steady_clock::now() - t0).count();
	};
	int rc = run_shards(devs, [&](int s) -> int {
		const auto t0 = std::chrono::steady_clock::now();
		int64_t r0, r1;
		shard_rows(nrow, s, N, &r0, &r1);
		const int64_t rs = r1 - r0;
		DevBuf O;
		if (O.alloc(out_n * 8) || O.zero())
			return -1;
		if (rs > 0) {
			CscGuard A(row_block_upload(x, r0, r1));
			if (A.h == NULL) return -1;
			auto put_y = [&](void *d) -> int {
				const int rc = tr_y ? staged_copy(d, (const char *) y + (size_t) r0 * y_nrow * ysz,
								  (size_t) rs * y_nrow * ysz)
						    : staged_copy_2d(d, (const char *) y + (size_t) r0 * ysz, (size_t) rs * ysz,
								     (size_t) K, (size_t) y_nrow * ysz);
				t_up[(size_t) s] = ms_since(t0);
				return rc;
			};
			if (dense_product(A.h, K, y_Rtype, (size_t) rs * K, put_y, tr_y ? y_nrow : rs, tr_y, O.as<double>(), 1,
					  ncol))
				return -1;
		}
		HIP_TRY(hipDeviceSynchronize());
		t_mul[(size_t) s] = ms_since(t0) - t_up[(size_t) s];
		part.p[(size_t) s] = O.p;
		O.p = nullptr;
		return 0;
	});
	if (rc) return -1;
	std::vector<size_t> q((size_t) N + 1, out_n);
	for (int s = 0; s < N; s++) q[(size_t) s] = (out_n / N * s + out_n % N * s / N) & ~(size_t) 1;
	rc = run_shards(devs, [&](int s) -> int {
		const auto t0 = std::chrono::steady_clock::now();
		const size_t c0 = q[(size_t) s], len = q[(size_t) s + 1] - c0;
		if (len == 0) return 0;
		const size_t stride = (len + 1) & ~(size_t) 1;
		DevBuf F, R;
		if (F.alloc(stride * N * 8) || R.alloc(len * 8))
			return -1;
		for (int t = 0; t < N; t++) {
			double *dst = F.as<double>() + (size_t) t * stride;
			const double *src = (const double *) part.p[(size_t) t] + c0;
			if (devs[(size_t) t] == devs[(size_t) s])
				HIP_TRY(hipMemcpyAsync(dst, src, len * 8, hipMemcpyDeviceToDevice, 0));
			else
				HIP_TRY(hipMemcpyPeerAsync(dst, devs[(size_t) s], src, devs[(size_t) t], len * 8, 0));
		}
		if (launch_shard_sum(F.as<double>(), N, (int64_t) stride, (int64_t) len, R.as<double>(), 0))
			return -1;
		HIP_TRY(hipStreamSynchronize(0));
		const int rd = staged_download(out + c0, R.p, len * 8);
		t_red[(size_t) s] = ms_since(t0);
		return rd;
	});
	if (timing)
		for (int s = 0; s < N; s++)
			fprintf(stderr, "svt shard %d/%d device %d: upload %.3f ms, product %.3f ms, reduce-scatter %.3f ms\n",
				s, N, devs[(size_t) s], t_up[(size_t) s], t_mul[(size_t) s], t_red[(size_t) s]);
	return rc;
}

static int crossprod2_SVT_mat_impl(const svt_view *x, const void *y, int y_nrow,
				      int y_ncol, int y_Rtype, int tr_y, double *out)
{
	if (ensure_init() || check_mult_view(x, "input objects"))
		return -1;
	const int in_nrow = x->dim[0], out_nrow = x->dim[1];
	if (in_nrow != (tr_y ? y_ncol : y_nrow))
		return svt_set_error("input objects are non-conformable");
	if (y_Rtype == SVT_LGLSXP) y_Rtype = SVT_INTSXP;
	if (!mult_types_ok(x->Rtype, y_Rtype))
		return svt_set_error("SparseArray internal error in "
				     "C_crossprod2_SVT_mat():\n"
				     "    'x_Rtype != TYPEOF(y)' not supported yet");
	const int out_ncol = tr_y ? y_nrow : y_ncol;
	const size_t out_n = (size_t) out_nrow * out_ncol;
	memset(out, 0, out_n * sizeof(double));
	if (x->svt_is_null || out_n == 0)
		return 0;
	if (shard_applies(x))
		return crossprod2_SVT_mat_sharded(x, y, y_nrow, y_ncol, y_Rtype, tr_y, out);
	CscGuard A(x);
	if (A.h == NULL) return -1;
	const size_t y_elems = (size_t) y_nrow * y_ncol;
	auto put_y = [&](void *d) { return staged_copy(d, y, y_elems * elt_size(y_Rtype)); };
	DevBuf O;
	if (O.alloc(out_n * 8) || O.zero() ||
	    dense_product(A.h, out_ncol, y_Rtype, y_elems, put_y, y_nrow, tr_y, O.as<double>(), 1, out_nrow))
		return -1;
	return staged_download(out, O.p, out_n * 8);
}
extern "C" int svt_crossprod2_SVT_mat(const svt_view *x, const void *y, int y_nrow,
				      int y_ncol, int y_Rtype, int tr_y, double *out)
{
	return abi_status([&] { return crossprod2_SVT_mat_impl(x, y, y_nrow, y_ncol, y_Rtype, tr_y, out); });
}

static int crossprod2_mat_SVT_impl(const void *x, int x_nrow, int x_ncol,
				      int x_Rtype, const svt_view *y, int tr_x,
				      double *out)
{
	if (ensure_init() || check_mult_view(y, "input objects"))
		return -1;
// ... 23 lines not shown
				      double *out)
{
	return abi_status([&] { return crossprod2_mat_SVT_impl(x, x_nrow, x_ncol, x_Rtype, y, tr_x, out); });
}

static int dev_crossprod_pp(const svt_dev_csc *other, const svt_dev_csc *pp, bool sym,
			    double *out_dev, int64_t sc, int64_t sk)
{
	const int64_t K = pp->ncol, nrow = pp->nrow;
	if (K <= 0 || other->ncol <= 0)
		return 0;
	const bool big = pbc_applies(other, K);
	if (other->Rtype == SVT_INTSXP && big) {
		Widened of, pf;
		if (of.widen(other) || (!sym && pf.widen(pp)))
			return -1;
		return dev_crossprod_pp(&of.view, sym ? &of.view : &pf.view, sym, out_dev, sc, sk);
	}
	int kc = chunk_K(nrow, K);
	const size_t esz = elt_size(pp->Rtype);
	svt_dev_pbc *P = NULL;
	int own_P = 1;
	if (other->Rtype == SVT_REALSXP && big) {
		P = pbc_for(other, &own_P);
		if (P != NULL && kc > 512) kc = 512;
	}
	DevBuf dense, ws;
	int rc = 0;
	if (dense.alloc((size_t) (nrow > 0 ? nrow : 1) * kc * esz) ||
	    ws.alloc(P ? svt_dev_crossprod_pbc_ws_bytes(P, kc)
		       : crossprod_ws_bytes(nrow, other->ncol, kc)))
		rc = -1;
	for (int64_t k0 = 0; rc == 0 && k0 < K; k0 += kc) {
		const int kn = (int) (K - k0 < kc ? K - k0 : kc);
		if (launch_densify(pp->col_ptr, pp->row_idx, pp->val, pp->Rtype, nrow,
				   k0, kn, dense.p, 0)) {
			rc = -1;
		} else if (P) {
			rc = svt_dev_crossprod_pbc_from(P, other, (const double *) dense.p, nrow, kn, 0,
							out_dev + k0 * sk, sc, sk, ws.p, ws.bytes, 0,
							sym ? k0 : 0);
		} else if (sym && k0 > 0) {
			svt_dev_csc tail = *other;
			tail.col_ptr += k0; tail.ncol -= k0; tail.owned = 0;
			rc = svt_dev_crossprod_csc_dense(&tail, dense.p, nrow, kn, 0,
							 out_dev + k0 * sk + k0 * sc, sc, sk,
							 ws.p, ws.bytes, 0);
		} else {
			rc = svt_dev_crossprod_csc_dense(other, dense.p, nrow, kn, 0,
							 out_dev + k0 * sk, sc, sk,
							 ws.p, ws.bytes, 0);
		}
	}
	if (rc == 0 && hipDeviceSynchronize() != hipSuccess)
		rc = svt_set_error("device error in the sparse x sparse crossprod");
	if (P && own_P) svt_dev_pbc_release(P);
	return rc;
}

struct OwnedCsc {
	svt_dev_csc *t;
	bool own;
	OwnedCsc(svt_dev_csc *p, bool o) : t(p), own(o) {}
	OwnedCsc(OwnedCsc &&o) : t(o.t), own(o.own) { o.own = false; }
	OwnedCsc(const OwnedCsc &) = delete;
	OwnedCsc &operator=(const OwnedCsc &) = delete;
	~OwnedCsc() { if (own) svt_release(t); }
};
static OwnedCsc transposed_for(const CscGuard &A);

static double g_gram_cost = 1.0;
extern "C" void svt_sparse_crossprod_set_cost(double factor)
{
	g_gram_cost = factor;
}

static double dense_route_seconds(double dense_ops) { return 1.0e-3 + dense_ops / 3.0e12; }
static double sparse_route_seconds(double pairs, int64_t nnz_x) { return 0.2e-3 + pairs / 2.6e11 + (double) nnz_x * 2.5e-11; }

static bool sparse_route_pays(int64_t nnz_x, int64_t nnz_y, int64_t nrow, double dense_ops, bool sym)
{
	if (g_gram_cost < 0.0 || nrow <= 0 || nnz_x <= 0 || nnz_y <= 0)
		return false;
	double pairs = (double) nnz_x * (double) nnz_y / (double) nrow;
	if (g_gram_cost > 0.0 && dense_ops < 268435456.0)
		return false;
	if (sym) { pairs *= 0.5; dense_ops *= 0.5; }
	return sparse_route_seconds(pairs, nnz_x) * g_gram_cost < dense_route_seconds(dense_ops);
}

static int dev_crossprod_sparse_on(const svt_dev_csc *T, const svt_dev_csc *Y, bool sym, double *O, int64_t ldo, double dense_ops)
{
	DevBuf Ws;
	int bad = 1;
	if (Ws.alloc(svt_dev_crossprod_csc_csc_ws_bytes(T)))
		return -1;
	if (sym && g_gram_cost > 0.0) {
		double pairs = 0.0;
		if (launch_gram_pairs(T->col_ptr, T->ncol, (double *) Ws.p, 0))
			return -1;
		HIP_TRY(hipMemcpy(&pairs, Ws.p, 8, hipMemcpyDeviceToHost));
		if (sparse_route_seconds(pairs, 0) * g_gram_cost > 1.5 * dense_route_seconds(0.5 * dense_ops))
			return 1;
	}
	const int rc = svt_dev_crossprod_csc_csc(T, Y, sym ? 1 : 0, O, ldo, Ws.p, Ws.bytes, NULL, 0);
	if (rc > 0) { g_unsupported = 0; return 1; }
	if (rc < 0) return -1;
	HIP_TRY(hipMemcpy(&bad, Ws.p, 4, hipMemcpyDeviceToHost));
	return bad ? 1 : 0;
}

static int dev_crossprod_sparse(const CscGuard &X, const svt_dev_csc *Y, bool sym, double *O, int64_t ldo, double dense_ops)
{
	if (X.h->nnz >= ((int64_t) 1 << 31))
		return 1;
	const OwnedCsc T = transposed_for(X);
	if (T.t == NULL) {
		if (g_unsupported) { g_unsupported = 0; return 1; }
		return -1;
	}
	return dev_crossprod_sparse_on(T.t, Y, sym, O, ldo, dense_ops);
}

static int dense_buffer_route(const svt_dev_csc *X, const svt_dev_csc *Y, bool sym, double *O)
{
	const int64_t nx = X->ncol, ny = Y->ncol;
	HIP_TRY(hipMemset(O, 0, (size_t) nx * ny * 8));
	if (sym)
		return dev_crossprod_pp(X, X, true, O, 1, nx) || launch_mirror_lower(O, nx, 0) ? -1 : 0;
	if (Y->nnz * nx < X->nnz * ny)
		return dev_crossprod_pp(Y, X, false, O, nx, 1);
	return dev_crossprod_pp(X, Y, false, O, 1, nx);
}

extern "C" int svt_dev_crossprod_csc_csc_dense_buffer(const svt_dev_csc *X, const svt_dev_csc *Y, double *out)
{
	if (X->nrow != Y->nrow)
		return svt_set_error("svt_dev_crossprod_csc_csc_dense_buffer: non-conformable operands");
	if (X->ncol == 0 || Y->ncol == 0) return 0;
	if (dense_buffer_route(X, Y, X == Y, out)) return -1;
	HIP_TRY(hipDeviceSynchronize());
	return 0;
}

template <class S, class D> static int sparse_then_dense(double *out, size_t out_n, S sparse, D dense)
{
	DevBuf O;
	if (O.alloc(out_n * 8))
		return -1;
	const int st = sparse(O.as<double>());
	if (st < 0 || (st > 0 && dense(O.as<double>())))
		return -1;
	return staged_download(out, O.p, out_n * 8);
}

static int64_t view_nzcount(const svt_view *x)
{
	int64_t t = 0;
	if (x->svt_is_null) return 0;
	for (int64_t j = 0; j < x->nleaves; j++) t += x->nzcount[j];
	return t;
}

static int crossprod2_SVT_SVT_impl(const svt_view *x, const svt_view *y, double *out)
{
	if (ensure_init() || check_mult_view(x, "input objects") ||
	    check_mult_view(y, "input objects"))
		return -1;
	const int in_nrow = x->dim[0];
	if (in_nrow != y->dim[0])
		return svt_set_error("input SVT_SparseMatrix objects are non-conformable");
	if (x->Rtype != y->Rtype)
		return svt_set_error("input SVT_SparseMatrix objects must have the "
				     "same type() for now");
	const int out_nrow = x->dim[1], out_ncol = y->dim[1];
	const size_t out_n = (size_t) out_nrow * out_ncol;
	memset(out, 0, out_n * sizeof(double));
	if (out_n == 0)
		return 0;
	const int64_t Lpp_nops = view_nzcount(y) * out_nrow;
	const int64_t Rpp_nops = view_nzcount(x) * out_ncol;
	const double dense_ops = (double) (Lpp_nops < Rpp_nops ? Lpp_nops : Rpp_nops);
	CscGuard X(x), Y(y);
	if (X.h == NULL || Y.h == NULL) return -1;
	const bool pays = !x->svt_is_null && !y->svt_is_null &&
			  sparse_route_pays(X.h->nnz, Y.h->nnz, in_nrow, dense_ops, false);
	return sparse_then_dense(out, out_n,
		[&](double *O) { return pays ? dev_crossprod_sparse(X, Y.h, false, O, out_nrow, dense_ops) : 1; },
		[&](double *O) { return dense_buffer_route(X.h, Y.h, false, O); });
}
extern "C" int svt_crossprod2_SVT_SVT(const svt_view *x, const svt_view *y, double *out)
{
	return abi_status([&] { return crossprod2_SVT_SVT_impl(x, y, out); });
}

static svt_dev_csc *dev_transposed(const svt_dev_csc *A)
{
	svt_dev_csc *T = (svt_dev_csc *) calloc(1, sizeof(*T));
	if (T == NULL) { svt_set_error("out of memory"); return NULL; }
	T->Rtype = A->Rtype; T->owned = 1; T->na_background = A->na_background;
	T->nrow = A->ncol; T->ncol = A->nrow; T->nnz = A->nnz;
	const size_t n = A->nnz > 0 ? (size_t) A->nnz : 1;
	const int64_t box = box_nnz_get();
	DevBuf ws;
	if (hipMalloc((void **) &T->col_ptr, ((size_t) T->ncol + 1) * 8) != hipSuccess ||
	    hipMalloc((void **) &T->row_idx, n * 4) != hipSuccess ||
	    hipMalloc(&T->val, n * elt_size(A->Rtype)) != hipSuccess ||
	    ws.alloc(transpose_ws_bytes_box(A->nrow, A->nnz, box))) {
		svt_set_error("device allocation failed (transposed operand)");
		svt_release(T);
		return NULL;
	}
	if (launch_transpose_box(A->col_ptr, A->row_idx, A->val, A->Rtype, A->nrow, A->ncol, A->nnz,
				 T->col_ptr, T->row_idx, T->val, ws.p, box, 0) ||
	    hipDeviceSynchronize() != hipSuccess) {
		if (svt_last_error()[0] == '\0') svt_set_error("device transposition failed");
		svt_release(T);
		return NULL;
	}
	return T;
}

static OwnedCsc transposed_for(const CscGuard &A)
{
	if (A.key != 0) {
		std::lock_guard<std::mutex> lk(g_res_mu);
		for (Resident &r : g_res)
			if (r.key == A.key && r.tr != NULL) return OwnedCsc(r.tr, false);
	}
	svt_dev_csc *T = dev_transposed(A.h);
	if (T == NULL || A.key == 0) return OwnedCsc(T, true);
	std::lock_guard<std::mutex> lk(g_res_mu);
	const size_t nb = csc_bytes(T);
	resident_make_room(nb);
	if (g_res_bytes + nb <= g_res_limit)
		for (Resident &r : g_res)
			if (r.key == A.key) {
				r.tr = T; r.bytes += nb; g_res_bytes += nb;
				return OwnedCsc(T, false);
			}
	return OwnedCsc(T, true);
}

static int transpose_2D_SVT_impl(const svt_view *x, int64_t *out_col_ptr,
				    int32_t *out_row_idx, void *out_val)
{
	if (ensure_init() || check_view(x))
		return -1;
	if (x->ndim != 2)
		return svt_set_error("object to transpose must have exactly 2 dimensions");
	const int64_t nrow = x->dim[0];
	if (x->svt_is_null || x->dim[1] == 0 || nrow == 0) {
		for (int64_t i = 0; i <= nrow; i++) out_col_ptr[i] = 0;
		return 0;
	}
	CscGuard A(x);
	if (A.h == NULL) return -1;
	const OwnedCsc TA = transposed_for(A);
	const svt_dev_csc *T = TA.t;
	if (T == NULL) return -1;
	HIP_TRY(hipMemcpy(out_col_ptr, T->col_ptr, (size_t) (nrow + 1) * 8, hipMemcpyDeviceToHost));
	if (T->nnz > 0) {
		if (staged_download(out_row_idx, T->row_idx, (size_t) T->nnz * 4) ||
		    staged_download(out_val, T->val, (size_t) T->nnz * elt_size(T->Rtype)))
			return -1;
	}
	return 0;
}
extern "C" int svt_transpose_2D_SVT(const svt_view *x, int64_t *out_col_ptr,
				    int32_t *out_row_idx, void *out_val)
{
	return abi_status([&] { return transpose_2D_SVT_impl(x, out_col_ptr, out_row_idx, out_val); });
}

struct svt_subset_result {
	svt_dev_csc *h;
};

static int subset_index0(const int *idx, int64_t n, int extent, std::vector<int32_t> &out)
{
	if (n < 0 || (n > 0 && idx == NULL))
		return svt_set_error("invalid subscript");
	out.resize((size_t) n);
	for (int64_t k = 0; k < n; k++) {
		const int v = idx[k];
		if (v == NA_INT)
			return svt_set_error("subscript contains NAs");
		if (v < 1 || v > extent)
			return svt_set_error("subscript out of bounds");
		out[(size_t) k] = v - 1;
	}
	return 0;
}

static void *subset_hip_alloc(size_t n, void *)
{
	void *p = NULL;
	return hipMalloc(&p, n) == hipSuccess ? p : NULL;
}
static void subset_hip_free(void *p, void *) { (void) hipFree(p); }

static int subset_SVT_begin_impl(const svt_view *x, const int *rows, int64_t nrows_sel, const int *cols, int64_t ncols_sel,
				 svt_subset_result **res, int64_t *out_nnz)
{
	if (res == NULL || out_nnz == NULL)
		return svt_set_error("svt_subset_SVT_begin: 'res' and 'out_nnz' are needed");
	*res = NULL;
	if (ensure_init() || check_view(x))
		return -1;
	if (x->ndim != 2)
		return svt_set_unsupported("N-index subsetting on the device takes 2-D operands only");
	std::vector<int32_t> r0, c0;
	if ((rows != NULL && subset_index0(rows, nrows_sel, x->dim[0], r0)) ||
	    (cols != NULL && subset_index0(cols, ncols_sel, x->dim[1], c0)))
		return -1;
	CscGuard A(x);
	if (A.h == NULL) return -1;
	DevBuf dr, dc;
	if ((rows != NULL && dr.upload(r0.data(), r0.size() * 4)) || (cols != NULL && dc.upload(c0.data(), c0.size() * 4)))
		return -1;
	svt_dev_csc *h = (svt_dev_csc *) calloc(1, sizeof(*h));
	if (h == NULL) return svt_set_error("out of memory");
	h->Rtype = A.h->Rtype; h->owned = 1; h->na_background = A.h->na_background;
	h->nrow = rows != NULL ? nrows_sel : A.h->nrow;
	h->ncol = cols != NULL ? ncols_sel : A.h->ncol;
	if (dev_subset_impl(A.h, dr.as<int32_t>(), rows != NULL ? nrows_sel : -1, dc.as<int32_t>(), cols != NULL ? ncols_sel : -1,
			    subset_hip_alloc, subset_hip_free, NULL, &h->nnz, &h->col_ptr, &h->row_idx, &h->val, NULL) ||
	    hipStreamSynchronize(0) != hipSuccess) {
		if (svt_last_error()[0] == '\0') svt_set_error("device error while subsetting");
		svt_release(h);
		return -1;
	}
	svt_subset_result *r = (svt_subset_result *) calloc(1, sizeof(*r));
	if (r == NULL) { svt_release(h); return svt_set_error("out of memory"); }
	r->h = h;
	*res = r;
	*out_nnz = h->nnz;
	return 0;
}
extern "C" int svt_subset_SVT_begin(const svt_view *x, const int *rows, int64_t nrows_sel, const int *cols, int64_t ncols_sel,
				    svt_subset_result **res, int64_t *out_nnz)
{
	return abi_status([&] { return subset_SVT_begin_impl(x, rows, nrows_sel, cols, ncols_sel, res, out_nnz); });
}

static int subset_SVT_end_impl(svt_subset_result *res, int64_t *out_col_ptr, int32_t *out_row_idx, void *out_val)
{
	if (res == NULL) return 0;
	const svt_dev_csc *h = res->h;
	int rc = 0;
	if (out_col_ptr != NULL || out_row_idx != NULL || out_val != NULL) {
		if (out_col_ptr == NULL || (h->nnz > 0 && (out_row_idx == NULL || out_val == NULL)))
			rc = svt_set_error("svt_subset_SVT_end: all three outputs, or none");
		else if (hipMemcpy(out_col_ptr, h->col_ptr, ((size_t) h->ncol + 1) * 8, hipMemcpyDeviceToHost) != hipSuccess)
			rc = svt_set_error("svt_subset_SVT_end: D2H copy failed");
		else if (h->nnz > 0 && (staged_download(out_row_idx, h->row_idx, (size_t) h->nnz * 4) ||
					staged_download(out_val, h->val, (size_t) h->nnz * elt_size(h->Rtype))))
			rc = -1;
	}
	svt_release(res->h);
	free(res);
	return rc;
}
extern "C" int svt_subset_SVT_end(svt_subset_result *res, int64_t *out_col_ptr, int32_t *out_row_idx, void *out_val)
{
	return abi_status([&] { return subset_SVT_end_impl(res, out_col_ptr, out_row_idx, out_val); });
}

static int matmul_SVT_mat_sharded(const svt_view *x, const void *y, int y_nrow, int y_ncol, int y_Rtype, double *out)
{
	if (check_leaves(x))
		return -1;
	const std::vector<int> devs = g_devices;
	const int N = (int) devs.size();
	const int64_t nrow = x->dim[0], K = y_ncol;
	const size_t y_elems = (size_t) y_nrow * y_ncol;
	return run_shards(devs, [&](int s) -> int {
		int64_t r0, r1;
		shard_rows(nrow, s, N, &r0, &r1);
		const int64_t rs = r1 - r0;
		if (rs == 0) return 0;
		CscGuard A(row_block_upload(x, r0, r1));
		if (A.h == NULL) return -1;
		const OwnedCsc T = transposed_for(A);
		if (T.t == NULL) return -1;
		A.drop();
		auto put_y = [&](void *d) { return staged_copy(d, y, y_elems * elt_size(y_Rtype)); };
		DevBuf O;
		if (O.alloc((size_t) rs * K * 8) || O.zero() ||
		    dense_product(T.t, K, y_Rtype, y_elems, put_y, y_nrow, 0, O.as<double>(), 1, rs))
			return -1;
		HIP_TRY(hipMemcpy2D(out + r0, (size_t) nrow * 8, O.p, (size_t) rs * 8, (size_t) rs * 8, (size_t) K,
				    hipMemcpyDeviceToHost));
		return 0;
	});
}

static int matmul_SVT_mat_impl(const svt_view *x, const void *y, int y_nrow,
				  int y_ncol, int y_Rtype, double *out)
{
	if (ensure_init() || check_mult_view(x, "input objects"))
		return -1;
	const int out_nrow = x->dim[0], in_nrow = x->dim[1];
	if (in_nrow != y_nrow)
		return svt_set_error("input objects are non-conformable");
	if (y_Rtype == SVT_LGLSXP) y_Rtype = SVT_INTSXP;
	if (!mult_types_ok(x->Rtype, y_Rtype))
		return svt_set_error("SparseArray internal error in "
				     "C_crossprod2_SVT_mat():\n"
				     "    'x_Rtype != TYPEOF(y)' not supported yet");
	const size_t out_n = (size_t) out_nrow * y_ncol;
	memset(out, 0, out_n * sizeof(double));
	if (x->svt_is_null || out_n == 0)
		return 0;
	if (shard_applies(x))
		return matmul_SVT_mat_sharded(x, y, y_nrow, y_ncol, y_Rtype, out);
	CscGuard A(x);
	if (A.h == NULL) return -1;
	const OwnedCsc T = transposed_for(A);
	if (T.t == NULL) return -1;
	A.drop();
	const size_t y_elems = (size_t) y_nrow * y_ncol;
	auto put_y = [&](void *d) { return staged_copy(d, y, y_elems * elt_size(y_Rtype)); };
	DevBuf O;
	if (O.alloc(out_n * 8) || O.zero() ||
	    dense_product(T.t, y_ncol, y_Rtype, y_elems, put_y, y_nrow, 0, O.as<double>(), 1, out_nrow))
		return -1;
	return staged_download(out, O.p, out_n * 8);
}
extern "C" int svt_matmul_SVT_mat(const svt_view *x, const void *y, int y_nrow,
				  int y_ncol, int y_Rtype, double *out)
{
	return abi_status([&] { return matmul_SVT_mat_impl(x, y, y_nrow, y_ncol, y_Rtype, out); });
}

static int matmul_SVT_SVT_impl(const svt_view *x, const svt_view *y, double *out)
{
	if (ensure_init() || check_mult_view(x, "input objects") ||
	    check_mult_view(y, "input objects"))
		return -1;
	if (x->dim[1] != y->dim[0])
		return svt_set_error("input SVT_SparseMatrix objects are non-conformable");
	if (x->Rtype != y->Rtype)
		return svt_set_error("input SVT_SparseMatrix objects must have the "
				     "same type() for now");
	const int out_nrow = x->dim[0], out_ncol = y->dim[1];
	const size_t out_n = (size_t) out_nrow * out_ncol;
	memset(out, 0, out_n * sizeof(double));
	if (out_n == 0)
		return 0;
	CscGuard X(x);
	if (X.h == NULL) return -1;
	CscGuard Y(y);
	if (Y.h == NULL) return -1;
	if (view_nzcount(y) * 20 <= (int64_t) y->dim[0] * y->dim[1]) {
		DevBuf Os, Ws;
		int bad = 1;
		if (Os.alloc(out_n * 8) || Ws.alloc(svt_dev_matmul_csc_csc_ws_bytes(X.h)))
			return -1;
		const int rc_s = svt_dev_matmul_csc_csc(X.h, Y.h, Os.as<double>(), out_nrow, Ws.p, Ws.bytes, NULL, 0);
		if (rc_s < 0)
			return -1;
		if (rc_s == 0) {
			HIP_TRY(hipMemcpy(&bad, (char *) Ws.p + 4, 4, hipMemcpyDeviceToHost));
			if (!bad)
				return staged_download(out, Os.p, out_n * 8) ? -1 : 0;
		} else
			g_unsupported = 0;
	}
	const OwnedCsc T = transposed_for(X);
	if (T.t == NULL) return -1;
	X.drop();
	return sparse_then_dense(out, out_n, [](double *) { return 1; },
				 [&](double *O) { return dense_buffer_route(T.t, Y.h, false, O); });
}
extern "C" int svt_matmul_SVT_SVT(const svt_view *x, const svt_view *y, double *out)
{
	return abi_status([&] { return matmul_SVT_SVT_impl(x, y, out); });
}

static int crossprod1_SVT_impl(const svt_view *x, double *out)
{
	if (ensure_init() || check_mult_view(x, "'x'"))
		return -1;
	const int n = x->dim[1];
	const size_t out_n = (size_t) n * n;
	memset(out, 0, out_n * sizeof(double));
	if (x->svt_is_null || out_n == 0)
		return 0;
	CscGuard X(x);
	if (X.h == NULL) return -1;
	const double dense_ops = (double) X.h->nnz * (double) n;
	const bool pays = sparse_route_pays(X.h->nnz, X.h->nnz, x->dim[0], dense_ops, true);
	return sparse_then_dense(out, out_n,
		[&](double *O) { return pays ? dev_crossprod_sparse(X, X.h, true, O, n, dense_ops) : 1; },
		[&](double *O) { return dense_buffer_route(X.h, X.h, true, O); });
}
extern "C" int svt_crossprod1_SVT(const svt_view *x, double *out)
{
	return abi_status([&] { return crossprod1_SVT_impl(x, out); });
}

static int tcrossprod1_SVT_impl(const svt_view *x, double *out)
{
	if (ensure_init() || check_mult_view(x, "'x'"))
		return -1;
	const int n = x->dim[0];
	const size_t out_n = (size_t) n * n;
	memset(out, 0, out_n * sizeof(double));
	if (x->svt_is_null || out_n == 0 || x->dim[1] == 0)
		return 0;
	CscGuard X(x);
	if (X.h == NULL) return -1;
	const OwnedCsc TM = transposed_for(X);
	const svt_dev_csc *M = TM.t;
	if (M == NULL) return -1;
	const double dense_ops = (double) M->nnz * (double) n;
	const bool pays = sparse_route_pays(M->nnz, M->nnz, M->nrow, dense_ops, true);
	return sparse_then_dense(out, out_n,
		[&](double *O) { return pays ? dev_crossprod_sparse_on(X.h, M, true, O, n, dense_ops) : 1; },
		[&](double *O) { return dense_buffer_route(M, M, true, O); });
}
extern "C" int svt_tcrossprod1_SVT(const svt_view *x, double *out)
{
	return abi_status([&] { return tcrossprod1_SVT_impl(x, out); });
}

static int tcrossprod2_SVT_SVT_impl(const svt_view *x, const svt_view *y, double *out)
{
	if (ensure_init() || check_mult_view(x, "input objects") ||
	    check_mult_view(y, "input objects"))
		return -1;
	if (x->dim[1] != y->dim[1])
		return svt_set_error("input SVT_SparseMatrix objects are non-conformable");
	if (x->Rtype != y->Rtype)
		return svt_set_error("input SVT_SparseMatrix objects must have the "
				     "same type() for now");
	const int out_nrow = x->dim[0], out_ncol = y->dim[0];
	const size_t out_n = (size_t) out_nrow * out_ncol;
	memset(out, 0, out_n * sizeof(double));
	if (out_n == 0)
		return 0;
	const int64_t Lpp_nops = view_nzcount(y) * out_nrow;
	const int64_t Rpp_nops = view_nzcount(x) * out_ncol;
	const double dense_ops = (double) (Lpp_nops < Rpp_nops ? Lpp_nops : Rpp_nops);
	CscGuard X(x), Y(y);
	if (X.h == NULL || Y.h == NULL) return -1;
	const OwnedCsc Ty = transposed_for(Y);
	if (Ty.t == NULL) return -1;
	const bool pays = !x->svt_is_null && !y->svt_is_null && x->dim[1] > 0 &&
			  sparse_route_pays(X.h->nnz, Y.h->nnz, x->dim[1], dense_ops, false);
	return sparse_then_dense(out, out_n,
		[&](double *O) { return pays ? dev_crossprod_sparse_on(X.h, Ty.t, false, O, out_nrow, dense_ops) : 1; },
		[&](double *O) {
			const OwnedCsc Tx = transposed_for(X);
			return Tx.t == NULL ? -1 : dense_buffer_route(Tx.t, Ty.t, false, O);
		});
}
extern "C" int svt_tcrossprod2_SVT_SVT(const svt_view *x, const svt_view *y, double *out)
{
	return abi_status([&] { return tcrossprod2_SVT_SVT_impl(x, y, out); });
}

static int run_colstats(const svt_dev_csc *A, int opcode, int na_rm, double center,
			int64_t inner, void *out_host, int out_Rtype, int *warn)
{
	const int64_t nseg = A->ncol / inner;
	const size_t osz = out_Rtype == SVT_REALSXP ? 8 : 4;
	DevBuf O, W;
	if (O.alloc((size_t) nseg * osz) || W.alloc(16) || W.zero())
		return -1;
	if (svt_dev_colstats(A, opcode, na_rm, center, inner, O.p, W.as<int>(), 0))
		return -1;
	int w = 0;
	HIP_TRY(hipMemcpy(out_host, O.p, (size_t) nseg * osz, hipMemcpyDeviceToHost));
	HIP_TRY(hipMemcpy(&w, W.p, 4, hipMemcpyDeviceToHost));
	if (w) *warn = 1;
	return 0;
}

template <class F> static int run_leaf_shards(const svt_view *x, int64_t unit, int64_t nunits, int *flag, F fn)
{
	const std::vector<int> devs = g_devices;
	const int N = (int) devs.size();
	const std::vector<int64_t> cut = shard_cuts(x, unit, nunits, N);
	std::vector<int> f((size_t) N, 0);
	const int rc = run_shards(devs, [&](int s) -> int {
		const int64_t u0 = cut[(size_t) s], u1 = cut[(size_t) s + 1];
		if (u1 <= u0) return 0;
		SubView sv;
		col_block_view(x, u0 * unit, u1 * unit, sv);
		CscGuard A(svt_upload(&sv.v));
		if (A.h == NULL) return -1;
		return fn(A.h, u0, &f[(size_t) s]);
	});
	for (int s = 0; s < N; s++)
		if (f[(size_t) s]) *flag = 1;
	return rc;
}

static int colStats_SVT_impl(const svt_view *x, int opcode, int na_rm, double center,
				int dims, void *out, int *warn)
{
	*warn = 0;
	if (ensure_init() || check_view(x) || check_stat_op(opcode, x->Rtype))
		return -1;
	if (dims < 1 || dims > x->ndim)
		return svt_set_error("'dims' must be >= 1 and <= %d", x->ndim);
	if (device_op_supported(opcode))
		return -1;
	int64_t inner = 1, nout = 1;
	for (int a = 1; a < dims; a++) inner *= x->dim[a];
	for (int a = dims; a < x->ndim; a++) nout *= x->dim[a];
	if (nout == 0)
		return 0;
	const int out_Rtype = svt_colStats_out_Rtype(opcode, x->Rtype);
	if (inner > 0 && shard_applies(x)) {
		const size_t osz = out_Rtype == SVT_REALSXP ? 8 : 4;
		return run_leaf_shards(x, inner, nout, warn, [&](const svt_dev_csc *A, int64_t g0, int *w) {
			return run_colstats(A, opcode, na_rm, center, inner, (char *) out + (size_t) g0 * osz, out_Rtype, w);
		});
	}
	CscGuard A(x);
	if (A.h == NULL) return -1;
	if (inner == 0) {
		std::vector<int64_t> cp((size_t) nout + 1, 0);
		DevBuf P;
		if (P.upload(cp.data(), cp.size() * 8)) return -1;
		svt_dev_csc E = *A.h;
		E.owned = 0; E.ncol = nout; E.nnz = 0; E.nrow = 0; E.col_ptr = P.as<int64_t>();
		return run_colstats(&E, opcode, na_rm, center, 1, out, out_Rtype, warn);
	}
	return run_colstats(A.h, opcode, na_rm, center, inner, out, out_Rtype, warn);
}
extern "C" int svt_colStats_SVT(const svt_view *x, int opcode, int na_rm, double center,
				int dims, void *out, int *warn)
{
	return abi_status([&] { return colStats_SVT_impl(x, opcode, na_rm, center, dims, out, warn); });
}

static int order_stat_SVT(const svt_view *x, int what, const double *vec, int nprobs, double constant, int na_rm,
			  int by_row, double *out)
{
	const bool quant = what == ORDER_QUANTILES;
	const char *col = order_stat_names[what][0];
	const double *probs = vec;
	if (ensure_init() || check_view(x))
		return -1;
	if (x->ndim != 2)
		return svt_set_error("the %s() method for SparseArray objects only supports 2D "
				     "objects (i.e. SparseMatrix objects) at the moment",
				     order_stat_names[what][by_row ? 1 : 0]);
	if (x->Rtype != SVT_REALSXP && x->Rtype != SVT_INTSXP && x->Rtype != SVT_LGLSXP)
		return svt_set_error("%s(): unsupported type", col);
	if (x->na_background)
		return svt_set_error("%s() is not supported on NaArray objects", col);
	if (quant) {
		if (nprobs < 0 || (nprobs > 0 && probs == NULL))
			return svt_set_error("invalid 'probs'");
		for (int q = 0; q < nprobs; q++)
			if (!(probs[q] >= 0.0 && probs[q] <= 1.0))
				return svt_set_error("'probs' outside [0,1]");
	}
	const int64_t nout = x->dim[by_row ? 0 : 1];
	if (nout == 0 || (quant && nprobs == 0))
		return 0;
	CscGuard A(x);
	if (A.h == NULL) return -1;
	const OwnedCsc T = by_row ? transposed_for(A) : OwnedCsc(NULL, false);
	if (by_row && T.t == NULL) return -1;
	const svt_dev_csc *M = by_row ? T.t : A.h;
	DevBuf P, O, W;
	const size_t out_bytes = (size_t) nout * (quant ? (size_t) nprobs : 1) * 8;
	const size_t vec_bytes = quant ? (size_t) nprobs * 8 : what == ORDER_MADS && vec ? (size_t) nout * 8 : 0;
	if ((vec_bytes && P.upload(vec, vec_bytes)) || O.alloc(out_bytes) || W.alloc(order_stat_ws_bytes(what, nout)))
		return -1;
	if (launch_order_stat(what, M->col_ptr, M->val, M->Rtype, M->nrow, nout, M->nnz, P.as<double>(), nprobs, constant,
			      na_rm, O.as<double>(), W.p, 0))
		return -1;
	HIP_TRY(hipDeviceSynchronize());
	return staged_download(out, O.p, out_bytes);
}

extern "C" int svt_colMedians_SVT(const svt_view *x, int na_rm, double *out)
{
	return abi_status([&] { return order_stat_SVT(x, ORDER_MEDIANS, NULL, 0, 0.0, na_rm, 0, out); });
}

extern "C" int svt_rowMedians_SVT(const svt_view *x, int na_rm, double *out)
{
	return abi_status([&] { return order_stat_SVT(x, ORDER_MEDIANS, NULL, 0, 0.0, na_rm, 1, out); });
}

extern "C" int svt_colQuantiles_SVT(const svt_view *x, const double *probs, int nprobs, int na_rm, double *out)
{
	return abi_status([&] { return order_stat_SVT(x, ORDER_QUANTILES, probs, nprobs, 0.0, na_rm, 0, out); });
}

extern "C" int svt_rowQuantiles_SVT(const svt_view *x, const double *probs, int nprobs, int na_rm, double *out)
{
	return abi_status([&] { return order_stat_SVT(x, ORDER_QUANTILES, probs, nprobs, 0.0, na_rm, 1, out); });
}

extern "C" int svt_colMads_SVT(const svt_view *x, const double *center, double constant, int na_rm, double *out)
{
	return abi_status([&] { return order_stat_SVT(x, ORDER_MADS, center, 0, constant, na_rm, 0, out); });
}

extern "C" int svt_rowMads_SVT(const svt_view *x, const double *center, double constant, int na_rm, double *out)
{
	return abi_status([&] { return order_stat_SVT(x, ORDER_MADS, center, 0, constant, na_rm, 1, out); });
}

template <typename R>
static void expand_ranks(const int64_t *cp, const int32_t *ri, const R *rank_nz, const R *zero_rank, int64_t mrow,
			 int64_t mcol, bool transposed, R *out)
{
	const size_t cells = (size_t) mrow * (size_t) mcol * sizeof(R);
	if (transposed) {
		team_run(team_size(cells), [&](int t, int nt) {
			for (int64_t i = mrow * t / nt; i < mrow * (t + 1) / nt; i++)
				memcpy(out + i * mcol, zero_rank, (size_t) mcol * sizeof(R));
		});
		team_run(team_size(cells), [&](int t, int nt) {
			for (int64_t j = mcol * t / nt; j < mcol * (t + 1) / nt; j++)
				for (int64_t k = cp[j]; k < cp[j + 1]; k++)
					out[j + (int64_t) ri[k] * mcol] = rank_nz[k];
		});
		return;
	}
	team_run(team_size(cells), [&](int t, int nt) {
		for (int64_t j = mcol * t / nt; j < mcol * (t + 1) / nt; j++) {
			R *col = out + j * mrow;
			for (int64_t i = 0; i < mrow; i++) col[i] = zero_rank[j];
			for (int64_t k = cp[j]; k < cp[j + 1]; k++) col[ri[k]] = rank_nz[k];
		}
	});
}

static int ranks_SVT(const svt_view *x, int ties, int preserve_shape, int by_row, void *out)
{
	if (ensure_init() || check_view(x))
		return -1;
	if (x->ndim != 2)
		return svt_set_error("the %s() method for SparseArray objects only supports 2D "
				     "objects (i.e. SparseMatrix objects) at the moment", by_row ? "rowRanks" : "colRanks");
	if (x->Rtype != SVT_REALSXP && x->Rtype != SVT_INTSXP && x->Rtype != SVT_LGLSXP)
		return svt_set_error("colRanks(): unsupported type");
	if (x->na_background)
		return svt_set_error("colRanks() is not supported on NaArray objects");
	if (check_ties(ties))
		return -1;
	if (x->dim[0] == 0 || x->dim[1] == 0)
		return 0;
	CscGuard A(x);
	if (A.h == NULL) return -1;
	const OwnedCsc T = by_row ? transposed_for(A) : OwnedCsc(NULL, false);
	if (by_row && T.t == NULL) return -1;
	const svt_dev_csc *M = by_row ? T.t : A.h;
	const int64_t mrow = M->nrow, mcol = M->ncol, nnz = M->nnz;
	if (mcol > 0x7FFFFFFFLL)
		return svt_set_unsupported("colRanks: more than 2^31-1 columns");
	std::vector<int64_t> cp((size_t) mcol + 1);
	std::vector<int32_t> ri((size_t) nnz);
	HIP_TRY(hipMemcpy(cp.data(), M->col_ptr, cp.size() * 8, hipMemcpyDeviceToHost));
	if (nnz > 0 && staged_download(ri.data(), M->row_idx, (size_t) nnz * 4))
		return -1;
	int64_t long_nnz = 0;
	for (int64_t j = 0; j < mcol; j++)
		if (ranks_form(cp[(size_t) j + 1] - cp[(size_t) j]) == 2) long_nnz += cp[(size_t) j + 1] - cp[(size_t) j];
	if (long_nnz > 0xFFFFFFFFLL)
		return svt_set_unsupported("colRanks: 2^32 or more stored values in the columns sorted in the workspace");
	const size_t esz = ties == SVT_TIES_AVERAGE ? 8 : 4;
	const size_t wsb = ranks_ws_bytes(mcol, long_nnz);
	DevBuf RN, RZ, F, W;
	if (RN.alloc((size_t) nnz * esz) || RZ.alloc((size_t) mcol * esz) || F.alloc(sizeof(int)) || W.alloc(wsb))
		return -1;
	if (launch_ranks(M->col_ptr, M->val, M->Rtype, mrow, mcol, nnz, ties, RN.p, RZ.p, F.as<int>(), W.p, wsb, 0))
		return -1;
	HIP_TRY(hipDeviceSynchronize());
	int flag = 0;
	HIP_TRY(hipMemcpy(&flag, F.p, sizeof(int), hipMemcpyDeviceToHost));
	if (flag)
		return svt_set_error("colRanks: the workspace did not hold the long columns");
	std::vector<char> rn((size_t) nnz * esz), rz((size_t) mcol * esz);
	if ((nnz > 0 && staged_download(rn.data(), RN.p, rn.size())) || staged_download(rz.data(), RZ.p, rz.size()))
		return -1;
	const bool transposed = by_row || !preserve_shape;
	if (esz == 8)
		expand_ranks<double>(cp.data(), ri.data(), (const double *) rn.data(), (const double *) rz.data(), mrow, mcol,
				     transposed, (double *) out);
	else
		expand_ranks<int32_t>(cp.data(), ri.data(), (const int32_t *) rn.data(), (const int32_t *) rz.data(), mrow, mcol,
				      transposed, (int32_t *) out);
	return 0;
}

extern "C" int svt_colRanks_SVT(const svt_view *x, int ties, int preserve_shape, void *out)
{
	return abi_status([&] { return ranks_SVT(x, ties, preserve_shape, 0, out); });
}

extern "C" int svt_rowRanks_SVT(const svt_view *x, int ties, void *out)
{
	return abi_status([&] { return ranks_SVT(x, ties, 0, 1, out); });
}

static int summarize_SVT_impl(const svt_view *x, int opcode, int na_rm, double center,
				 double *out_d, int *out_i, int *out_Rtype, int *warn)
{
	*warn = 0;
	if (ensure_init() || check_view(x) || check_stat_op(opcode, x->Rtype))
		return -1;
	if (opcode == SVT_OP_SUM_X_X2 || opcode == SVT_OP_VAR2 || opcode == SVT_OP_SD2)
		return device_op_supported(opcode);
	const int rt = svt_colStats_out_Rtype(opcode, x->Rtype);
	*out_Rtype = rt;
	out_d[0] = out_d[1] = 0.0;
	out_i[0] = out_i[1] = 0;
	CscGuard A(x);
	if (A.h == NULL) return -1;
	svt_dev_csc V = *A.h;
	V.owned = 0;
	int64_t inner = V.ncol;
	DevBuf P;
	if (inner == 0) {
		int64_t cp[2] = {0, 0};
		if (P.upload(cp, sizeof(cp))) return -1;
		V.ncol = 1; V.nrow = 0; V.nnz = 0; V.col_ptr = P.as<int64_t>();
		inner = 1;
	}
	const int ops[2] = { opcode == SVT_OP_RANGE ? SVT_OP_MIN : opcode, SVT_OP_MAX };
	const int nops = opcode == SVT_OP_RANGE ? 2 : 1;
	for (int t = 0; t < nops; t++) {
		double d = 0.0;
		int i = 0;
		void *dst = rt == SVT_REALSXP ? (void *) &d : (void *) &i;
		if (run_colstats(&V, ops[t], na_rm, center, inner, dst, rt, warn))
			return -1;
		out_d[t] = d;
// ... 10 lines not shown
static int rowStats_SVT_impl(const svt_view *x, int opcode, int na_rm,
				const double *center, int dims, void *out, int *warn)
{
	*warn = 0;
	if (ensure_init() || check_view(x) || check_stat_op(opcode, x->Rtype))
		return -1;
	if (dims < 1 || dims > x->ndim - 1)
		return svt_set_error("'dims' must be >= 1 and <= %d", x->ndim - 1);
	if (x->na_background && opcode == SVT_OP_CENTERED_X2_SUM)
		return svt_set_error("operation not yet supported on NaArray objects");
	if (opcode != SVT_OP_COUNTNAS && opcode != SVT_OP_ANYNA &&
	    opcode != SVT_OP_MIN && opcode != SVT_OP_MAX &&
	    opcode != SVT_OP_SUM && opcode != SVT_OP_CENTERED_X2_SUM)
		return svt_set_error("SparseArray internal error in C_rowStats_SVT():\n"
				     "    operation not supported");
	const int out_Rtype = svt_colStats_out_Rtype(opcode, x->Rtype);
	const size_t osz = out_Rtype == SVT_REALSXP ? 8 : 4;
	int64_t inner = 1, nstrata = 1;
	for (int a = 1; a < dims; a++) inner *= x->dim[a];
	for (int a = dims; a < x->ndim; a++) nstrata *= x->dim[a];
	const int64_t out_len = inner * x->dim[0];
	if (out_len == 0)
		return 0;
	if ((opcode == SVT_OP_MIN || opcode == SVT_OP_MAX) && nstrata == 0) {
		for (int64_t i = 0; i < out_len; i++) {
			if (out_Rtype == SVT_REALSXP)
				((double *) out)[i] = opcode == SVT_OP_MIN ? INFINITY : -INFINITY;
			else
				((int *) out)[i] = NA_INT;
		}
		if (out_Rtype != SVT_REALSXP) *warn = 1;
		return 0;
	}
	if (nstrata > 0xFFFFFFFFLL)
		return svt_set_unsupported("too many strata for the device coverage counters");
	CscGuard A(x);
	if (A.h == NULL) return -1;
	DevBuf O, C, S, W;
	if (O.alloc((size_t) out_len * osz) ||
	    S.alloc(rowstats_scratch_bytes(opcode, out_len)) ||
	    W.alloc(16) || W.zero())
		return -1;
	if (center != NULL && C.upload(center, (size_t) out_len * 8))
		return -1;
	RowStatsArgs a = rowstats_args(A.h, opcode, na_rm, inner, nstrata, O.p);
	a.center = center ? C.as<double>() : NULL;
	a.scratch = S.p; a.warn_flag = W.as<int>();
	if (a.na_bg && inner > 65535)
		return svt_set_unsupported("row statistics of NaArray objects: more than 65535 output columns");
	if (inner <= 65535) {
		DevBuf T;
		if (T.alloc(rowstats_panel_ws_bytes(a.nrow, a.ncol)) || launch_rowstats_panel(a, T.p, 0))
			return -1;
		HIP_TRY(hipDeviceSynchronize());
	} else if (launch_rowstats(a, 0)) {
		return -1;
	}
	int w = 0;
	if (staged_download(out, O.p, (size_t) out_len * osz)) return -1;
	HIP_TRY(hipMemcpy(&w, W.p, 4, hipMemcpyDeviceToHost));
	if (w) *warn = 1;
	return 0;
}
extern "C" int svt_rowStats_SVT(const svt_view *x, int opcode, int na_rm,
				const double *center, int dims, void *out, int *warn)
{
	return abi_status([&] { return rowStats_SVT_impl(x, opcode, na_rm, center, dims, out, warn); });
}

static int rowStatsFull_SVT_impl(const svt_view *x, int opcode, int na_rm,
				 const double *center, int dims, void *out, int *warn)
{
	*warn = 0;
	if (ensure_init() || check_view(x) || check_stat_op(opcode, x->Rtype))
		return -1;
	if (dims < 1 || dims > x->ndim - 1)
		return svt_set_error("'dims' must be >= 1 and <= %d", x->ndim - 1);
	if (check_rowstats_op(opcode, x->Rtype, x->na_background))
		return -1;
	const bool range = opcode == SVT_OP_RANGE;
	const int out_Rtype = svt_colStats_out_Rtype(opcode, x->Rtype);
	const size_t osz = out_Rtype == SVT_REALSXP ? 8 : 4;
	int64_t inner = 1, nstrata = 1;
	for (int a = 1; a < dims; a++) inner *= x->dim[a];
	for (int a = dims; a < x->ndim; a++) nstrata *= x->dim[a];
	const int64_t out_len = inner * x->dim[0], nout = out_len * (range ? 2 : 1);
	if (out_len == 0)
		return 0;
	if ((opcode == SVT_OP_MIN || opcode == SVT_OP_MAX || range) && nstrata == 0) {
		for (int64_t i = 0; i < nout; i++) {
			if (out_Rtype == SVT_REALSXP)
				((double *) out)[i] = (range ? i < out_len : opcode == SVT_OP_MIN) ? INFINITY : -INFINITY;
			else
				((int *) out)[i] = NA_INT;
		}
		if (out_Rtype != SVT_REALSXP) *warn = 1;
		return 0;
	}
	if (nstrata > 0xFFFFFFFFLL)
		return svt_set_unsupported("too many strata for the device coverage counters");
	if (inner > 65535 && x->na_background)
		return svt_set_unsupported("row statistics of NaArray objects: more than 65535 output columns");
	if (inner > 65535 && !rowstats_reference_op(opcode))
		return svt_set_unsupported("row statistics: this operation is not served with more than 65535 output columns");
	CscGuard A(x);
	if (A.h == NULL) return -1;
	DevBuf O, C, W, T;
	if (O.alloc((size_t) nout * osz) || W.alloc(16) || W.zero() ||
	    T.alloc(svt_dev_rowstats_ws_bytes_op(A.h, opcode, inner)))
		return -1;
	if (center != NULL && C.upload(center, (size_t) out_len * 8))
		return -1;
	if (dev_rowstats_impl(A.h, opcode, na_rm, center ? C.as<double>() : NULL, inner, O.p, W.as<int>(), T.p,
			      svt_dev_rowstats_ws_bytes_op(A.h, opcode, inner), 0))
		return -1;
	HIP_TRY(hipDeviceSynchronize());
	int w = 0;
	if (staged_download(out, O.p, (size_t) nout * osz)) return -1;
	HIP_TRY(hipMemcpy(&w, W.p, 4, hipMemcpyDeviceToHost));
	if (w) *warn = 1;
	return 0;
}
extern "C" int svt_rowStatsFull_SVT(const svt_view *x, int opcode, int na_rm,
				    const double *center, int dims, void *out, int *warn)
{
	return abi_status([&] { return rowStatsFull_SVT_impl(x, opcode, na_rm, center, dims, out, warn); });
}

static int check_group(const int *group, int n, int ngroup)
{
	for (int i = 0; i < n; i++) {
		const int g = group[i];
		if (g == NA_INT) {
			if (ngroup < 1)
				return svt_set_error("'ngroup' must be >= 1 when 'group' "
						     "contains missing values");
		} else if (g < 1 || g > ngroup) {
			return svt_set_error("all non-NA values in 'group' must "
					     "be >= 1 and <= 'ngroup'");
		}
	}
	return 0;
}

static int groupsum_host(const svt_dev_csc *A, const int32_t *col_ptr32,
			 const int *group, int ngroup, int na_rm, bool colsum,
			 void *out, int *ovflow)
{
	const int64_t glen = colsum ? A->ncol : A->nrow;
	const int64_t out_len = colsum ? A->nrow * (int64_t) ngroup
				       : (int64_t) ngroup * A->ncol;
	if (out_len > 0x7FFFFFFFLL)
		return svt_set_error("too many groups (matrix of sums will be too big)");
	const size_t osz = elt_size(A->Rtype);
	if (out_len == 0)
		return 0;
	DevBuf G, O, S, W;
	if (G.upload(group, (size_t) glen * 4) || O.alloc((size_t) out_len * osz) ||
	    S.alloc(groupsum_scratch_bytes(A->Rtype, out_len)) || W.alloc(16) || W.zero())
		return -1;
	GroupSumArgs a = groupsum_args(A, col_ptr32, G.as<int>(), ngroup, na_rm, O.p);
	a.scratch = S.p; a.ovflow_flag = W.as<int>();
	if (colsum ? launch_colsum(a, 0) : launch_rowsum(a, 0)) return -1;
	int w = 0;
	if (staged_download(out, O.p, (size_t) out_len * osz)) return -1;
	HIP_TRY(hipMemcpy(&w, W.p, 4, hipMemcpyDeviceToHost));
	if (ovflow && w) *ovflow = 1;
	return 0;
}

static int xsum_SVT(const svt_view *x, const int *group, int ngroup, int na_rm,
		    bool colsum, void *out, int *ovflow)
{
	*ovflow = 0;
	if (ensure_init() || check_view(x))
		return -1;
	if (x->ndim != 2)
		return svt_set_error("input object must have 2 dimensions");
	if (x->na_background)
		return svt_set_error("NaArray objects are not supported by this operation");
	if (x->Rtype != SVT_REALSXP && x->Rtype != SVT_INTSXP)
		return svt_set_error("rowsum() and colsum() do not support "
				     "SVT_SparseMatrix objects of this type at the moment");
	if (check_group(group, colsum ? x->dim[1] : x->dim[0], ngroup))
		return -1;
	if (!colsum && shard_applies(x)) {
		const int64_t ncol = x->dim[1];
		if ((int64_t) ngroup * ncol > 0x7FFFFFFFLL)
			return svt_set_error("too many groups (matrix of sums will be too big)");
		const size_t osz = elt_size(x->Rtype);
		return run_leaf_shards(x, 1, ncol, ovflow, [&](const svt_dev_csc *A, int64_t c0, int *ov) {
			return groupsum_host(A, NULL, group, ngroup, na_rm, false, (char *) out + (size_t) ngroup * c0 * osz, ov);
		});
	}
	CscGuard A(x);
	if (A.h == NULL) return -1;
	return groupsum_host(A.h, NULL, group, ngroup, na_rm, colsum, out, ovflow);
}

extern "C" int svt_rowsum_SVT(const svt_view *x, const int *group, int ngroup,
			      int na_rm, void *out, int *ovflow)
{
	return abi_status([&] { return xsum_SVT(x, group, ngroup, na_rm, false, out, ovflow); });
}

extern "C" int svt_colsum_SVT(const svt_view *x, const int *group, int ngroup,
			      int na_rm, void *out, int *ovflow)
{
	return abi_status([&] { return xsum_SVT(x, group, ngroup, na_rm, true, out, ovflow); });
}

static int xsum_dgC(int nrow, int ncol, const double *xx, const int *xi, const int *xp,
		    const int *group, int ngroup, int na_rm, bool colsum, double *out)
{
	if (ensure_init() || check_group(group, colsum ? ncol : nrow, ngroup))
		return -1;
	const int64_t nnz = ncol > 0 ? xp[ncol] : 0;
	DevBuf P, I, X;
	if (P.upload(xp, (size_t) (ncol + 1) * 4) || I.upload(xi, (size_t) nnz * 4) ||
// ... 8 lines not shown

extern "C" int svt_rowsum_dgCMatrix(int nrow, int ncol, const double *xx, const int *xi,
				    const int *xp, const int *group, int ngroup,
				    int na_rm, double *out)
{
	return abi_status([&] { return xsum_dgC(nrow, ncol, xx, xi, xp, group, ngroup, na_rm, false, out); });
}
extern "C" int svt_colsum_dgCMatrix(int nrow, int ncol, const double *xx, const int *xi,
				    const int *xp, const int *group, int ngroup,
				    int na_rm, double *out)
{
	return abi_status([&] { return xsum_dgC(nrow, ncol, xx, xi, xp, group, ngroup, na_rm, true, out); });
}

static int colstat_dgC(int nrow, int ncol, const double *xx, const int *xp, int na_rm,
		       int which, double *out)
{
	if (ensure_init())
		return -1;
	if (nrow < 0 || ncol < 0 || xp == NULL)
		return svt_set_error("invalid dgCMatrix slots");
	if (ncol == 0)
		return 0;
	std::vector<int64_t> cp((size_t) ncol + 1);
	for (int j = 0; j <= ncol; j++) {
		if (xp[j] < 0 || (j > 0 && (xp[j] < xp[j - 1] || xp[j] - xp[j - 1] > nrow)))
			return svt_set_error("invalid dgCMatrix 'p' slot");
		cp[(size_t) j] = xp[j];
	}
	const int64_t nnz = cp[(size_t) ncol];
	if (nnz > 0 && xx == NULL)
		return svt_set_error("invalid dgCMatrix slots");
	DevBuf P, X, O;
	if (P.upload(cp.data(), cp.size() * 8) || X.upload(xx, (size_t) nnz * 8) ||
	    O.alloc((size_t) ncol * 8 * (which == 2 ? 2 : 1)))
		return -1;
	svt_dev_csc A;
	memset(&A, 0, sizeof(A));
	A.Rtype = SVT_REALSXP; A.nrow = nrow; A.ncol = ncol; A.nnz = nnz;
	A.col_ptr = P.as<int64_t>(); A.val = X.p;
	const double NA = svt_na_real();
	int rc;
	switch (which) {
	case 0: rc = dev_colstats_ex(&A, SVT_OP_MIN, na_rm, NA, 1, O.p, NULL, 0, 1); break;
	case 1: rc = dev_colstats_ex(&A, SVT_OP_MAX, na_rm, NA, 1, O.p, NULL, 0, 1); break;
	case 2:
		rc = dev_colstats_ex(&A, SVT_OP_MIN, na_rm, NA, 1, O.p, NULL, 0, 1);
		if (rc == 0)
			rc = dev_colstats_ex(&A, SVT_OP_MAX, na_rm, NA, 1, O.as<double>() + ncol, NULL, 0, 1);
		break;
	default: rc = dev_colstats_ex(&A, SVT_OP_VAR1, na_rm, NA, 1, O.p, NULL, 0, 1); break;
	}
	if (rc) return -1;
	HIP_TRY(hipDeviceSynchronize());
	return staged_download(out, O.p, (size_t) ncol * 8 * (which == 2 ? 2 : 1));
}

extern "C" int svt_colMins_dgCMatrix(int nrow, int ncol, const double *xx, const int *xp,
				     int na_rm, double *out)
{
	return abi_status([&] { return colstat_dgC(nrow, ncol, xx, xp, na_rm, 0, out); });
}
extern "C" int svt_colMaxs_dgCMatrix(int nrow, int ncol, const double *xx, const int *xp,
				     int na_rm, double *out)
{
	return abi_status([&] { return colstat_dgC(nrow, ncol, xx, xp, na_rm, 1, out); });
}
extern "C" int svt_colRanges_dgCMatrix(int nrow, int ncol, const double *xx, const int *xp,
				       int na_rm, double *out)
{
	return abi_status([&] { return colstat_dgC(nrow, ncol, xx, xp, na_rm, 2, out); });
}
extern "C" int svt_colVars_dgCMatrix(int nrow, int ncol, const double *xx, const int *xp,
				     int na_rm, double *out)
{
	return abi_status([&] { return colstat_dgC(nrow, ncol, xx, xp, na_rm, 3, out); });
}
```

Baseline: 57.64.

## Unify device pool allocator, add stream-ordered staging, and batch downloads to cut host syncs

Replaces the PBC-only memory pool with a shared per-device pool and a small host-side cache of idle blocks, and routes scratch allocations in colstats and rowsum through it. Uploads become stream-ordered: the stager waits on a compute event instead of draining, and only joins the default stream afterwards. Downloads are batched through a Fetch helper rather than issued as separate blocking memcpys, and several redundant device synchronizes are removed. The goal is fewer host blocks and less allocation overhead per call. The cost is more complex lifetime and ordering logic, with a risk of reuse or ordering bugs, plus counters for debugging.

```diff
diff --git a/include/svt_hip.h b/include/svt_hip.h
--- a/include/svt_hip.h
+++ b/include/svt_hip.h
@@ -154,6 +154,8 @@
 svt_dev_pbc *svt_dev_pbc_build(const svt_dev_csc *A, int CBW, int WPB, int logR);
 void svt_dev_pbc_release(svt_dev_pbc *P);
 void svt_dev_pbc_trim(void);
+size_t svt_debug_pool_reserved(int device);
+int64_t svt_debug_host_blocks(int reset);
 size_t svt_dev_pbc_bytes(const svt_dev_pbc *P);
 size_t svt_dev_crossprod_pbc_ws_bytes(const svt_dev_pbc *P, int K);
 int svt_dev_crossprod_pbc(const svt_dev_pbc *P, const svt_dev_csc *A,
diff --git a/sparsearray_amd/_abi.py b/sparsearray_amd/_abi.py
--- a/sparsearray_amd/_abi.py
+++ b/sparsearray_amd/_abi.py
@@ -52,6 +52,8 @@
     "svt_dev_pbc_build": (P, [P, I, I, I]),
     "svt_dev_pbc_release": (None, [P]),
     "svt_dev_pbc_trim": (None, []),
+    "svt_debug_pool_reserved": (Z, [I]),
+    "svt_debug_host_blocks": (L, [I]),
     "svt_dev_pbc_bytes": (Z, [P]),
     "svt_dev_crossprod_pbc_ws_bytes": (Z, [P, I]),
     "svt_dev_crossprod_pbc": (I, [P, P, P, L, I, I, P, L, L, P, Z, P]),
diff --git a/sparsearray_amd/csrc/kernels_colstats.hip b/sparsearray_amd/csrc/kernels_colstats.hip
--- a/sparsearray_amd/csrc/kernels_colstats.hip
+++ b/sparsearray_amd/csrc/kernels_colstats.hip
@@ -520,7 +520,7 @@
 	const size_t n = (size_t) a.nseg * nchunk;
 	const size_t b_st = (n * sizeof(ColState) + 255) / 256 * 256, b_c = ((size_t) a.nseg * 8 + 255) / 256 * 256;
 	char *scr = NULL;
-	HIP_TRY(hipMallocAsync((void **) &scr, b_st + b_c + n * 8 + 256, s));
+	HIP_TRY(svt_pool_alloc((void **) &scr, b_st + b_c + n * 8 + 256, s));
 	ColState *st = (ColState *) scr;
 	double *centers = (double *) (scr + b_st), *acc2 = (double *) (scr + b_st + b_c);
 	dim3 grid((unsigned) nchunk, (unsigned) a.nseg), cgrid((unsigned) ((a.nseg + 255) / 256));
@@ -535,7 +535,7 @@
 				   (int) two_pass, (int) is_dbl);
 	}
 	HIP_TRY(hipGetLastError());
-	HIP_TRY(hipFreeAsync(scr, s));
+	svt_pool_free(scr, s);
 	return 0;
 }
 
diff --git a/sparsearray_amd/csrc/kernels_mult_pbc.hip b/sparsearray_amd/csrc/kernels_mult_pbc.hip
--- a/sparsearray_amd/csrc/kernels_mult_pbc.hip
+++ b/sparsearray_amd/csrc/kernels_mult_pbc.hip
@@ -401,55 +401,8 @@
 	for (int x = threadIdx.x; x < PBC_SLACK * 4; x += blockDim.x) slack[x] = 0u;
 }
 
-#define PBC_POOL_KEEP ((uint64_t) 3 << 30)
-#define PBC_MAX_DEV 16
-static hipMemPool_t g_pbc_pool[PBC_MAX_DEV];
-static bool g_pbc_pool_ok[PBC_MAX_DEV];
-
-static std::mutex g_pbc_pool_mu;
-
-static hipMemPool_t pbc_pool(int dev)
-{
-	if (dev < 0 || dev >= PBC_MAX_DEV)
-		return NULL;
-	std::lock_guard<std::mutex> lk(g_pbc_pool_mu);
-	if (!g_pbc_pool_ok[dev]) {
-		hipMemPoolProps props;
-		memset(&props, 0, sizeof(props));
-		props.allocType = hipMemAllocationTypePinned;
-		props.handleTypes = hipMemHandleTypeNone;
-		props.location.type = hipMemLocationTypeDevice;
-		props.location.id = dev;
-		hipMemPool_t pool = NULL;
-		if (hipMemPoolCreate(&pool, &props) != hipSuccess) {
-			(void) hipGetLastError();
-			return NULL;
-		}
-		uint64_t keep = PBC_POOL_KEEP;
-		(void) hipMemPoolSetAttribute(pool, hipMemPoolAttrReleaseThreshold, &keep);
-		g_pbc_pool[dev] = pool;
-		g_pbc_pool_ok[dev] = true;
-	}
-	return g_pbc_pool[dev];
-}
-
-static hipError_t pbc_alloc(void **p, size_t n)
-{
-	int dev = 0;
-	(void) hipGetDevice(&dev);
-	hipMemPool_t pool = pbc_pool(dev);
-	if (pool == NULL)
-		return hipMallocAsync(p, n ? n : 16, 0);
-	return hipMallocFromPoolAsync(p, n ? n : 16, pool, 0);
-}
-static void pbc_free(void *p) { if (p) (void) hipFreeAsync(p, 0); }
-
-extern "C" void svt_dev_pbc_trim(void)
-{
-	for (int d = 0; d < PBC_MAX_DEV; d++)
-		if (g_pbc_pool_ok[d])
-			(void) hipMemPoolTrimTo(g_pbc_pool[d], 0);
-}
+static hipError_t pbc_alloc(void **p, size_t n) { return svt_pool_alloc(p, n, 0); }
+static void pbc_free(void *p) { svt_pool_free(p, 0); }
 
 static void pbc_note_use(const svt_dev_pbc *P, hipStream_t s)
 {
@@ -474,8 +427,10 @@
 		}
 		(void) hipEventDestroy(ev);
 	}
-	if (sync)
+	if (sync) {
+		svt_note_host_block();
 		(void) hipDeviceSynchronize();
+	}
 	pbc_free(h->rec);
 	pbc_free(h->tile_ptr);
 	pbc_free(h->col_has_na);
@@ -618,6 +573,7 @@
 						   dim3(256), 0, 0, h->tile_ptr, h->npanels, h->ngroups, (int *) (meta + 2));
 				hipLaunchKernelGGL(pbc_build_finish_kernel, dim3(1), dim3(256), 0, 0, h->tile_ptr, ntiles,
 						   (char *) h->rec, (int) rbytes, meta);
+				svt_note_host_block();
 				ok = hipMemcpy(hmeta, meta, 24, hipMemcpyDeviceToHost) == hipSuccess;
 			}
 			h->nrec = hmeta[0];
diff --git a/sparsearray_amd/csrc/kernels_rowstats.hip b/sparsearray_amd/csrc/kernels_rowstats.hip
--- a/sparsearray_amd/csrc/kernels_rowstats.hip
+++ b/sparsearray_amd/csrc/kernels_rowstats.hip
@@ -1005,7 +1005,7 @@
 
 static int make_group16(const GroupSumArgs &a, uint16_t **g16, hipStream_t s)
 {
-	HIP_TRY(hipMallocAsync((void **) g16, (size_t) a.nrow * 2 + 16, s));
+	HIP_TRY(svt_pool_alloc((void **) g16, (size_t) a.nrow * 2 + 16, s));
 	hipLaunchKernelGGL(group16_kernel, dim3((unsigned) ((a.nrow + 255) / 256)), dim3(256), 0, s,
 			   a.group, a.nrow, a.ngroup, *g16);
 	return 0;
@@ -1155,7 +1155,7 @@
 			hipLaunchKernelGGL(rowsum_f64_lds_kernel<uint16_t>, dim3((unsigned) a.ncol), dim3(256),
 					   (size_t) a.ngroup * 8, s, a, (const uint16_t *) g16);
 		HIP_TRY(hipGetLastError());
-		HIP_TRY(hipFreeAsync(g16, s));
+		svt_pool_free(g16, s);
 		return 0;
 	}
 	hipLaunchKernelGGL(rowsum_f64_lds_kernel<int>, dim3((unsigned) a.ncol), dim3(256),
@@ -1189,7 +1189,7 @@
 		hipLaunchKernelGGL(rowsum_gid_cols_kernel, dim3((unsigned) ((a.ncol + C - 1) / C)), dim3(C * 64), 0, s,
 				   a.col_ptr64, a.row_idx, a.ncol, a.nrow, g16, gid, C);
 		HIP_TRY(hipGetLastError());
-		HIP_TRY(hipFreeAsync(g16, s));
+		svt_pool_free(g16, s);
 		return 0;
 	}
 	int64_t nb = ((a.nnz + 1) / 2 + 255) / 256;
diff --git a/sparsearray_amd/csrc/kernels_transpose.hip b/sparsearray_amd/csrc/kernels_transpose.hip
--- a/sparsearray_amd/csrc/kernels_transpose.hip
+++ b/sparsearray_amd/csrc/kernels_transpose.hip
@@ -928,7 +928,7 @@
 	}
 	if (queue_more())
 		return -1;
-	HIP_TRY(hipStreamSynchronize(s));
+	HIP_BLOCK(hipStreamSynchronize(s));
 	bd->reserve((size_t) npts * 2 + 2);
 	bd->push_back({0, 0});
 	bd->push_back({n, nnz});
@@ -1445,7 +1445,7 @@
 	hipLaunchKernelGGL(aperm_slab_count_kernel, dim3((unsigned) ((nslab + 1 + 255) / 256)), dim3(256), 0, s,
 			   c.col_ptr, sm, nslab, dim[q], os[q], base, maxcnt);
 	HIP_TRY(hipMemcpyAsync(&mx, maxcnt, 8, hipMemcpyDeviceToHost, s));
-	HIP_TRY(hipStreamSynchronize(s));
+	HIP_BLOCK(hipStreamSynchronize(s));
 	if (mx > SLAB_CAP) {
 		g_route[R_SLAB_REFUSED]++;
 		return APERM_REFUSED;
diff --git a/sparsearray_amd/csrc/svt_common.h b/sparsearray_amd/csrc/svt_common.h
--- a/sparsearray_amd/csrc/svt_common.h
+++ b/sparsearray_amd/csrc/svt_common.h
@@ -106,6 +106,12 @@
 					     hipGetErrorString(e__),         \
 					     __FILE__, __LINE__);             \
 	} while (0)
+
+#define SVT_POOL_KEEP ((uint64_t) 3 << 30)
+hipError_t svt_pool_alloc(void **p, size_t n, hipStream_t s);
+void svt_pool_free(void *p, hipStream_t s);
+void svt_note_host_block(void);
+#define HIP_BLOCK(expr) do { svt_note_host_block(); HIP_TRY(expr); } while (0)
 
 template <class F>
 static inline void svt_by_rtype(int Rtype, const void *in, void *out, F &&f)
diff --git a/sparsearray_amd/csrc/svt_hip.cpp b/sparsearray_amd/csrc/svt_hip.cpp
--- a/sparsearray_amd/csrc/svt_hip.cpp
+++ b/sparsearray_amd/csrc/svt_hip.cpp
@@ -12,6 +12,7 @@
 #include <functional>
 #include <mutex>
 #include <thread>
+#include <unordered_map>
 #include <vector>
 
 static thread_local char g_err[1024];
@@ -168,16 +169,173 @@
 	return svt_init(0);
 }
 
+static std::atomic<int64_t> g_host_blocks{0};
+void svt_note_host_block(void) { g_host_blocks.fetch_add(1, std::memory_order_relaxed); }
+extern "C" int64_t svt_debug_host_blocks(int reset)
+{
+	return reset ? g_host_blocks.exchange(0) : g_host_blocks.load();
+}
+
+#define SVT_POOL_MAX_DEV 16
+enum { POOL_UNTRIED = 0, POOL_OWN = 1, POOL_DEFAULT = 2, POOL_NONE = 3 };
+static hipMemPool_t g_pool[SVT_POOL_MAX_DEV];
+static int g_pool_state[SVT_POOL_MAX_DEV];
+static std::mutex g_pool_mu[SVT_POOL_MAX_DEV];
+#define SVT_CACHE_KEEP ((size_t) 1 << 30)
+#define SVT_CACHE_BLOCKS 64
+struct PoolCache {
+	struct Blk { void *p; size_t n; };
+	std::vector<Blk> idle;
+	std::unordered_map<void *, size_t> live;
+	std::unordered_map<void *, size_t> raw;
+	size_t bytes = 0;
+};
+static PoolCache g_cache[SVT_POOL_MAX_DEV];
+
+static int pool_state(int dev)
+{
+	if (g_pool_state[dev] != POOL_UNTRIED)
+		return g_pool_state[dev];
+	int has = 0;
+	if (hipDeviceGetAttribute(&has, hipDeviceAttributeMemoryPoolsSupported, dev) != hipSuccess || !has) {
+		(void) hipGetLastError();
+		return g_pool_state[dev] = POOL_NONE;
+	}
+	hipMemPoolProps props;
+	memset(&props, 0, sizeof(props));
+	props.allocType = hipMemAllocationTypePinned;
+	props.handleTypes = hipMemHandleTypeNone;
+	props.location.type = hipMemLocationTypeDevice;
+	props.location.id = dev;
+	hipMemPool_t pool = NULL;
+	if (hipMemPoolCreate(&pool, &props) != hipSuccess) {
+		(void) hipGetLastError();
+		return g_pool_state[dev] = POOL_DEFAULT;
+	}
+	uint64_t keep = SVT_POOL_KEEP;
+	(void) hipMemPoolSetAttribute(pool, hipMemPoolAttrReleaseThreshold, &keep);
+	g_pool[dev] = pool;
+	return g_pool_state[dev] = POOL_OWN;
+}
+
+hipError_t svt_pool_alloc(void **p, size_t n, hipStream_t s)
+{
+	int dev = 0;
+	(void) hipGetDevice(&dev);
+	if (n == 0) n = 16;
+	if (dev < 0 || dev >= SVT_POOL_MAX_DEV)
+		return hipMallocAsync(p, n, s);
+	std::lock_guard<std::mutex> lk(g_pool_mu[dev]);
+	switch (pool_state(dev)) {
+	case POOL_OWN: break;
+	case POOL_DEFAULT: return hipMallocAsync(p, n, s);
+	default: return hipMalloc(p, n);
+	}
+	if (s != (hipStream_t) 0)
+		return hipMallocFromPoolAsync(p, n, g_pool[dev], s);
+	n = (n + 255) & ~(size_t) 255;
+	PoolCache &c = g_cache[dev];
+	int best = -1;
+	for (size_t i = 0; i < c.idle.size(); i++)
+		if (c.idle[i].n >= n && c.idle[i].n / 2 <= n && (best < 0 || c.idle[i].n < c.idle[(size_t) best].n))
+			best = (int) i;
+	if (best >= 0) {
+		const PoolCache::Blk b = c.idle[(size_t) best];
+		c.idle.erase(c.idle.begin() + best);
+		c.bytes -= b.n;
+		c.live[b.p] = b.n;
+		*p = b.p;
+		return hipSuccess;
+	}
+	const hipError_t e = hipMallocFromPoolAsync(p, n, g_pool[dev], s);
+	if (e == hipSuccess) c.live[*p] = n;
+	return e;
+}
+
+#define SVT_CALL_BIG ((size_t) 256 << 20)
+static hipError_t call_alloc(void **p, size_t n)
+{
+	if (n < SVT_CALL_BIG)
+		return svt_pool_alloc(p, n, 0);
+	int dev = 0;
+	(void) hipGetDevice(&dev);
+	const hipError_t e = hipMalloc(p, n);
+	if (e == hipSuccess && dev >= 0 && dev < SVT_POOL_MAX_DEV) {
+		std::lock_guard<std::mutex> lk(g_pool_mu[dev]);
+		g_cache[dev].raw[*p] = n;
+	}
+	return e;
+}
+
+void svt_pool_free(void *p, hipStream_t s)
+{
+	if (p == NULL) return;
+	int dev = 0;
+	(void) hipGetDevice(&dev);
+	if (dev < 0 || dev >= SVT_POOL_MAX_DEV) { (void) hipFreeAsync(p, s); return; }
+	std::unique_lock<std::mutex> lk(g_pool_mu[dev]);
+	if (g_cache[dev].raw.erase(p)) {
+		lk.unlock();
+		(void) hipFree(p);
+		return;
+	}
+	if (g_pool_state[dev] == POOL_NONE) { (void) hipFree(p); return; }
+	PoolCache &c = g_cache[dev];
+	const auto it = c.live.find(p);
+	if (it != c.live.end()) {
+		const size_t n = it->second;
+		c.live.erase(it);
+		if (s == (hipStream_t) 0 && c.bytes + n <= SVT_CACHE_KEEP && c.idle.size() < SVT_CACHE_BLOCKS) {
+			c.idle.push_back({p, n});
+			c.bytes += n;
+			return;
+		}
+	}
+	(void) hipFreeAsync(p, s);
+}
+
+extern "C" void svt_dev_pbc_trim(void)
+{
+	int cur = 0;
+	(void) hipGetDevice(&cur);
+	for (int d = 0; d < SVT_POOL_MAX_DEV; d++) {
+		std::lock_guard<std::mutex> lk(g_pool_mu[d]);
+		if (g_pool_state[d] != POOL_OWN || hipSetDevice(d) != hipSuccess) continue;
+		for (const PoolCache::Blk &b : g_cache[d].idle) (void) hipFreeAsync(b.p, 0);
+		g_cache[d].idle.clear();
+		g_cache[d].bytes = 0;
+		svt_note_host_block();
+		(void) hipDeviceSynchronize();
+		(void) hipMemPoolTrimTo(g_pool[d], 0);
+	}
+	(void) hipSetDevice(cur);
+}
+
+extern "C" size_t svt_debug_pool_reserved(int device)
+{
+	if (device < 0 || device >= SVT_POOL_MAX_DEV) return 0;
+	std::lock_guard<std::mutex> lk(g_pool_mu[device]);
+	uint64_t v = 0;
+	if (g_pool_state[device] != POOL_OWN ||
+	    hipMemPoolGetAttribute(g_pool[device], hipMemPoolAttrReservedMemCurrent, &v) != hipSuccess)
+		return 0;
+	return (size_t) v;
+}
+
 struct Stager {
 	static const size_t CHUNK = (size_t) 48 << 20;
 	size_t chunk = CHUNK;
 	int dev = -1;
+	static const size_t BOUNCE = ((size_t) 4 << 20) + 4096;
 	char *buf[2] = {NULL, NULL};
+	char *bounce = NULL;
 	hipEvent_t done[2];
+	hipEvent_t ev_compute, ev_staged;
 	hipStream_t stream = NULL;
 	bool ok = false;
 	int next = 0;
 	bool busy[2] = {false, false};
+	bool ordered = false;
 
 	int init()
 	{
@@ -186,6 +344,9 @@
 			HIP_TRY(hipHostMalloc((void **) &buf[i], chunk, hipHostMallocDefault));
 			HIP_TRY(hipEventCreateWithFlags(&done[i], hipEventDisableTiming));
 		}
+		HIP_TRY(hipHostMalloc((void **) &bounce, BOUNCE, hipHostMallocDefault));
+		HIP_TRY(hipEventCreateWithFlags(&ev_compute, hipEventDisableTiming));
+		HIP_TRY(hipEventCreateWithFlags(&ev_staged, hipEventDisableTiming));
 		HIP_TRY(hipStreamCreateWithFlags(&stream, hipStreamNonBlocking));
 		ok = true;
 		return 0;
@@ -195,8 +356,34 @@
 		if (init()) return -1;
 		const int i = next;
 		next ^= 1;
-		if (busy[i]) { HIP_TRY(hipEventSynchronize(done[i])); busy[i] = false; }
+		if (busy[i]) {
+			if (hipEventQuery(done[i]) != hipSuccess) {
+				(void) hipGetLastError();
+				HIP_BLOCK(hipEventSynchronize(done[i]));
+			}
+			busy[i] = false;
+		}
 		*p = buf[i]; *slot = i;
+		return 0;
+	}
+	int order_after_compute()
+	{
+		if (init()) return -1;
+		HIP_TRY(hipEventRecord(ev_compute, 0));
+		HIP_TRY(hipStreamWaitEvent(stream, ev_compute, 0));
+		ordered = true;
+		return 0;
+	}
+	int begin_upload()
+	{
+		if (!ordered && order_after_compute()) return -1;
+		ordered = false;
+		return 0;
+	}
+	int join_compute()
+	{
+		HIP_TRY(hipEventRecord(ev_staged, stream));
+		HIP_TRY(hipStreamWaitEvent(0, ev_staged, 0));
 		return 0;
 	}
 	int send(int slot, void *dst, size_t off_in_buf, size_t n)
@@ -213,7 +400,7 @@
 	int drain()
 	{
 		if (!ok) return 0;
-		HIP_TRY(hipStreamSynchronize(stream));
+		HIP_BLOCK(hipStreamSynchronize(stream));
 		busy[0] = busy[1] = false;
 		return 0;
 	}
@@ -227,6 +414,10 @@
 				(void) hipHostFree(buf[i]);
 				buf[i] = NULL;
 			}
+			(void) hipEventDestroy(ev_compute);
+			(void) hipEventDestroy(ev_staged);
+			(void) hipHostFree(bounce);
+			bounce = NULL;
 			ok = false;
 			next = 0;
 			busy[0] = busy[1] = false;
@@ -270,13 +461,8 @@
 	return nt;
 }
 
-static int staged_copy(void *dst, const void *src, size_t n)
-{
-	if (n < ((size_t) 1 << 20)) {
-		if (n) HIP_TRY(hipMemcpy(dst, src, n, hipMemcpyHostToDevice));
-		return 0;
-	}
-	Stager &st = cur_stager();
+static int staged_send(Stager &st, void *dst, const void *src, size_t n)
+{
 	for (size_t off = 0; off < n; off += st.chunk) {
 		const size_t len = n - off < st.chunk ? n - off : st.chunk;
 		char *b; int slot;
@@ -288,7 +474,14 @@
 		});
 		if (st.send(slot, (char *) dst + off, 0, len) || st.commit(slot)) return -1;
 	}
-	return st.drain();
+	return 0;
+}
+static int staged_copy(void *dst, const void *src, size_t n)
+{
+	if (n == 0) return 0;
+	Stager &st = cur_stager();
+	if (st.begin_upload() || staged_send(st, dst, src, n)) return -1;
+	return st.join_compute();
 }
 
 static int staged_copy_2d(void *dst, const void *src, size_t run, size_t ncols, size_t ld)
@@ -296,7 +489,9 @@
 	if (run == ld || ncols <= 1)
 		return staged_copy(dst, src, run * ncols);
 	const size_t n = run * ncols;
+	if (n == 0) return 0;
 	Stager &st = cur_stager();
+	if (st.begin_upload()) return -1;
 	for (size_t off = 0; off < n; off += st.chunk) {
 		const size_t len = n - off < st.chunk ? n - off : st.chunk;
 		char *b; int slot;
@@ -313,18 +508,14 @@
 		});
 		if (st.send(slot, (char *) dst + off, 0, len) || st.commit(slot)) return -1;
 	}
-	return st.drain();
-}
-
-static int staged_download(void *dst, const void *src, size_t n)
-{
-	if (n < ((size_t) 4 << 20)) {
-		if (n) HIP_TRY(hipMemcpy(dst, src, n, hipMemcpyDeviceToHost));
-		return 0;
-	}
+	return st.join_compute();
+}
+
+static int chunked_download(void *dst, const void *src, size_t n)
+{
 	Stager &st = cur_stager();
-	if (st.init() || st.drain()) return -1;
-	HIP_TRY(hipDeviceSynchronize());
+	if (st.order_after_compute()) return -1;
+	st.ordered = false;
 	const size_t C = st.chunk;
 	const size_t nchunk = (n + C - 1) / C;
 	for (size_t c = 0; c <= nchunk; c++) {
@@ -336,7 +527,7 @@
 		}
 		if (c > 0) {
 			const size_t off = (c - 1) * C, len = n - off < C ? n - off : C;
-			HIP_TRY(hipEventSynchronize(st.done[(c - 1) & 1]));
+			HIP_BLOCK(hipEventSynchronize(st.done[(c - 1) & 1]));
 			const char *b = st.buf[(c - 1) & 1];
 			char *d0 = (char *) dst + off;
 			team_run(team_size(len), [&](int t, int nt) {
@@ -345,7 +536,46 @@
 			});
 		}
 	}
+	st.busy[0] = st.busy[1] = false;
 	return 0;
+}
+
+struct Fetch {
+	struct Item { void *dst; const void *src; size_t n, off; };
+	std::vector<Item> small, large;
+	size_t used = 0;
+	int add(void *dst, const void *src, size_t n)
+	{
+		if (n == 0) return 0;
+		Stager &st = cur_stager();
+		if (st.init()) return -1;
+		const size_t at = (used + 15) & ~(size_t) 15;
+		if (n < ((size_t) 4 << 20) && at + n <= Stager::BOUNCE) {
+			HIP_TRY(hipMemcpyAsync(st.bounce + at, src, n, hipMemcpyDeviceToHost, 0));
+			small.push_back({dst, src, n, at});
+			used = at + n;
+		} else {
+			large.push_back({dst, src, n, 0});
+		}
+		return 0;
+	}
+	int wait()
+	{
+		for (const Item &it : large)
+			if (chunked_download(it.dst, it.src, it.n)) return -1;
+		if (large.empty() && !small.empty())
+			HIP_BLOCK(hipStreamSynchronize(0));
+		const Stager &st = cur_stager();
+		for (const Item &it : small) memcpy(it.dst, st.bounce + it.off, it.n);
+		small.clear(); large.clear(); used = 0;
+		return 0;
+	}
+};
+
+static int staged_download(void *dst, const void *src, size_t n)
+{
+	Fetch f;
+	return f.add(dst, src, n) || f.wait() ? -1 : 0;
 }
 
 struct DevBuf {
@@ -353,11 +583,15 @@
 	size_t bytes = 0;
 	DevBuf() {}
 	DevBuf(const DevBuf &) = delete;
-	~DevBuf() { if (p) (void) hipFree(p); }
+	~DevBuf() { svt_pool_free(p, 0); }
 	int alloc(size_t n)
 	{
 		if (n == 0) n = 16;
-		HIP_TRY(hipMalloc(&p, n));
+		const hipError_t e = call_alloc(&p, n);
+		if (e != hipSuccess) {
+			p = nullptr;
+			return svt_set_error("hipMalloc(&p, n) failed: %s (%s:%d)", hipGetErrorString(e), __FILE__, __LINE__);
+		}
 		bytes = n;
 		return 0;
 	}
@@ -368,7 +602,7 @@
 	}
 	int zero()
 	{
-		HIP_TRY(hipMemset(p, 0, bytes));
+		HIP_TRY(hipMemsetAsync(p, 0, bytes, 0));
 		return 0;
 	}
 	template <typename T> T *as() { return (T *) p; }
@@ -405,7 +639,27 @@
 	return 0;
 }
 
-extern "C" svt_dev_csc *svt_upload(const svt_view *x)
+enum { CSC_WRAPPED = 0, CSC_HIPMALLOC = 1, CSC_POOLED = 2 };
+
+static int csc_alloc(svt_dev_csc *d, bool pooled, size_t nn, size_t esz)
+{
+	d->owned = pooled ? CSC_POOLED : CSC_HIPMALLOC;
+	if (pooled) {
+		const size_t a = ((size_t) (d->ncol + 1) * 8 + 255) & ~(size_t) 255, b = a + ((nn * 4 + 255) & ~(size_t) 255);
+		char *base = NULL;
+		if (call_alloc((void **) &base, b + nn * esz) != hipSuccess)
+			return 1;
+		d->col_ptr = (int64_t *) base;
+		d->row_idx = (int32_t *) (base + a);
+		d->val = base + b;
+		return 0;
+	}
+	return hipMalloc((void **) &d->col_ptr, (size_t) (d->ncol + 1) * 8) != hipSuccess ||
+	       hipMalloc((void **) &d->row_idx, nn * 4) != hipSuccess ||
+	       hipMalloc(&d->val, nn * esz) != hipSuccess;
+}
+
+static svt_dev_csc *upload_csc(const svt_view *x, bool pooled)
 {
 	if (ensure_init() || check_view(x))
 		return NULL;
@@ -427,25 +681,22 @@
 	}
 	svt_dev_csc *d = (svt_dev_csc *) calloc(1, sizeof(*d));
 	d->Rtype = x->Rtype;
-	d->owned = 1;
 	d->na_background = x->na_background != 0;
 	d->nrow = dim0;
 	d->ncol = n;
 	d->nnz = col_ptr[(size_t) n];
 	const size_t nn = (size_t) (d->nnz > 0 ? d->nnz : 1);
-	if (hipMalloc((void **) &d->col_ptr, (size_t) (d->ncol + 1) * 8) != hipSuccess ||
-	    hipMalloc((void **) &d->row_idx, nn * 4) != hipSuccess ||
-	    hipMalloc(&d->val, nn * esz) != hipSuccess) {
+	if (csc_alloc(d, pooled, nn, esz)) {
 		svt_set_error("hipMalloc failed while uploading an SVT (%lld nnz)",
 			      (long long) d->nnz);
 		svt_release(d);
 		return NULL;
 	}
-	bool ok = hipMemcpy(d->col_ptr, col_ptr.data(), (size_t) (d->ncol + 1) * 8,
-			    hipMemcpyHostToDevice) == hipSuccess;
+	Stager &st = cur_stager();
+	bool ok = (pooled ? st.begin_upload() : st.init()) == 0 &&
+		  staged_send(st, d->col_ptr, col_ptr.data(), (size_t) (d->ncol + 1) * 8) == 0;
 	const int64_t cap = (int64_t) (g_stager_chunk() / (4 + esz));
 	const int64_t nnz = d->nnz;
-	Stager &st = cur_stager();
 	for (int64_t k0 = 0; ok && k0 < nnz; k0 += cap) {
 		const int64_t cnt = nnz - k0 < cap ? nnz - k0 : cap;
 		char *b; int slot;
@@ -480,7 +731,7 @@
 				   (size_t) cnt * esz) == 0 &&
 		     st.commit(slot) == 0;
 	}
-	if (ok) ok = st.drain() == 0;
+	if (ok) ok = (pooled ? st.join_compute() : st.drain()) == 0;
 	if (!ok) {
 		if (svt_last_error()[0] == '\0') svt_set_error("H2D copy failed");
 		svt_release(d);
@@ -489,13 +740,18 @@
 	return d;
 }
 
+extern "C" svt_dev_csc *svt_upload(const svt_view *x)
+{
+	return upload_csc(x, false);
+}
+
 extern "C" svt_dev_csc *svt_wrap_device_csc(int Rtype, int64_t nrow, int64_t ncol,
 					    int64_t nnz, int64_t *col_ptr,
 					    int32_t *row_idx, void *val)
 {
 	svt_dev_csc *d = (svt_dev_csc *) calloc(1, sizeof(*d));
 	d->Rtype = Rtype;
-	d->owned = 0;
+	d->owned = CSC_WRAPPED;
 	d->nrow = nrow;
 	d->ncol = ncol;
 	d->nnz = nnz;
@@ -509,7 +765,9 @@
 {
 	if (h == NULL)
 		return;
-	if (h->owned) {
+	if (h->owned == CSC_POOLED) {
+		svt_pool_free(h->col_ptr, 0);
+	} else if (h->owned) {
 		if (h->col_ptr) (void) hipFree(h->col_ptr);
 		if (h->row_idx) (void) hipFree(h->row_idx);
 		if (h->val) (void) hipFree(h->val);
@@ -630,7 +888,7 @@
 	explicit CscGuard(svt_dev_csc *p) : h(p), key(0) {}
 	explicit CscGuard(const svt_view *x) : h(NULL), key(0)
 	{
-		if (g_res_limit == 0) { h = svt_upload(x); return; }
+		if (g_res_limit == 0) { h = upload_csc(x, true); return; }
 		if (check_view(x) || check_leaves(x)) return;
 		const uint64_t k = view_fingerprint(x) | 1;
 		{
@@ -1086,7 +1344,7 @@
 {
 	int64_t head[2] = { 0, 0 };
 	HIP_TRY(hipMemcpyAsync(head, ws, sizeof(head), hipMemcpyDeviceToHost, s));
-	HIP_TRY(hipStreamSynchronize(s));
+	HIP_BLOCK(hipStreamSynchronize(s));
 	*flag = (int) (head[0] & 0xFFFFFFFFLL);
 	*total = head[1];
 	return 0;
@@ -1532,13 +1790,11 @@
 	if (launch_aperm_box(A.h->col_ptr, A.h->row_idx, A.h->val, A.h->Rtype, A.h->ncol, A.h->nnz, dim,
 			     x->ndim, perm0, P.as<int64_t>(), I.as<int32_t>(), V.p, W.p, box, 0))
 		return -1;
-	HIP_TRY(hipMemcpy(out_col_ptr, P.p, (size_t) (new_nl + 1) * 8, hipMemcpyDeviceToHost));
-	if (A.h->nnz) {
-		if (staged_download(out_row_idx, I.p, (size_t) A.h->nnz * 4) ||
-		    staged_download(out_val, V.p, (size_t) A.h->nnz * esz))
-			return -1;
-	}
-	return 0;
+	Fetch f;
+	if (f.add(out_col_ptr, P.p, (size_t) (new_nl + 1) * 8) ||
+	    (A.h->nnz && (f.add(out_row_idx, I.p, (size_t) A.h->nnz * 4) || f.add(out_val, V.p, (size_t) A.h->nnz * esz))))
+		return -1;
+	return f.wait();
 }
 extern "C" int svt_aperm_SVT(const svt_view *x, const int *perm, int64_t *out_col_ptr,
 			     int32_t *out_row_idx, void *out_val)
@@ -1702,9 +1958,9 @@
 {
 	SubView sv;
 	row_block_view(x, (int) r0, (int) r1, sv);
-	svt_dev_csc *d = svt_upload(&sv.v);
+	svt_dev_csc *d = upload_csc(&sv.v, true);
 	if (d == NULL || r0 == 0) return d;
-	if (launch_rebase_rows(d->row_idx, d->nnz, (int32_t) r0, 0) || hipStreamSynchronize(0) != hipSuccess) {
+	if (launch_rebase_rows(d->row_idx, d->nnz, (int32_t) r0, 0)) {
 		if (svt_last_error()[0] == '\0') svt_set_error("device error while rebasing a row block");
 		svt_release(d);
 		return NULL;
@@ -1748,7 +2004,7 @@
 	~ShardBufs()
 	{
 		for (size_t s = 0; s < p.size(); s++)
-			if (p[s] && hipSetDevice(dev[s]) == hipSuccess) (void) hipFree(p[s]);
+			if (p[s] && hipSetDevice(dev[s]) == hipSuccess) svt_pool_free(p[s], 0);
 		if (g_device >= 0) (void) hipSetDevice(g_device);
 	}
 	ShardBufs(const ShardBufs &) = delete;
@@ -1871,8 +2127,6 @@
 			rc = svt_dev_crossprod_pbc(P, A, (const double *) Y_dev + (tr_y ? k0 : k0 * ldY), ldY, kn,
 						   tr_y, out_dev + k0 * sk, sc, sk, ws.p, ws.bytes, 0);
 		}
-		if (rc == 0 && hipDeviceSynchronize() != hipSuccess)
-			rc = svt_set_error("device error in the panel-blocked crossprod");
 		if (own_P) svt_dev_pbc_release(P);
 		return rc;
 	}
@@ -1891,7 +2145,6 @@
 						ws.p, ws.bytes, 0))
 			return -1;
 	}
-	HIP_TRY(hipDeviceSynchronize());
 	return 0;
 }
 
@@ -1900,9 +2153,11 @@
 			 int tr_y, double *O, int64_t sc, int64_t sk)
 {
 	PbcAhead ahead;
+	DevBuf Y;
+	if (Y.alloc(y_elems * elt_size(y_Rtype)) || cur_stager().order_after_compute())
+		return -1;
 	ahead.start(A, K);
-	DevBuf Y;
-	if (Y.alloc(y_elems * elt_size(y_Rtype)) || put_y(Y.p))
+	if (put_y(Y.p))
 		return -1;
 	const void *Yp = Y.p;
 	Widened Aw;
@@ -1962,7 +2217,7 @@
 					  ncol))
 				return -1;
 		}
-		HIP_TRY(hipDeviceSynchronize());
+		HIP_BLOCK(hipStreamSynchronize(0));
 		t_mul[(size_t) s] = ms_since(t0) - t_up[(size_t) s];
 		part.p[(size_t) s] = O.p;
 		O.p = nullptr;
@@ -1989,7 +2244,6 @@
 		}
 		if (launch_shard_sum(F.as<double>(), N, (int64_t) stride, (int64_t) len, R.as<double>(), 0))
 			return -1;
-		HIP_TRY(hipStreamSynchronize(0));
 		const int rd = staged_download(out + c0, R.p, len * 8);
 		t_red[(size_t) s] = ms_since(t0);
 		return rd;
@@ -2119,8 +2373,6 @@
 							 ws.p, ws.bytes, 0);
 		}
 	}
-	if (rc == 0 && hipDeviceSynchronize() != hipSuccess)
-		rc = svt_set_error("device error in the sparse x sparse crossprod");
 	if (P && own_P) svt_dev_pbc_release(P);
 	return rc;
 }
@@ -2156,7 +2408,8 @@
 	return sparse_route_seconds(pairs, nnz_x) * g_gram_cost < dense_route_seconds(dense_ops);
 }
 
-static int dev_crossprod_sparse_on(const svt_dev_csc *T, const svt_dev_csc *Y, bool sym, double *O, int64_t ldo, double dense_ops)
+static int dev_crossprod_sparse_on(const svt_dev_csc *T, const svt_dev_csc *Y, bool sym, double *O, int64_t ldo, double dense_ops,
+				   double *out, size_t out_n)
 {
 	DevBuf Ws;
 	int bad = 1;
@@ -2166,18 +2419,22 @@
 		double pairs = 0.0;
 		if (launch_gram_pairs(T->col_ptr, T->ncol, (double *) Ws.p, 0))
 			return -1;
-		HIP_TRY(hipMemcpy(&pairs, Ws.p, 8, hipMemcpyDeviceToHost));
+		if (staged_download(&pairs, Ws.p, 8))
+			return -1;
 		if (sparse_route_seconds(pairs, 0) * g_gram_cost > 1.5 * dense_route_seconds(0.5 * dense_ops))
 			return 1;
 	}
 	const int rc = svt_dev_crossprod_csc_csc(T, Y, sym ? 1 : 0, O, ldo, Ws.p, Ws.bytes, NULL, 0);
 	if (rc > 0) { g_unsupported = 0; return 1; }
 	if (rc < 0) return -1;
-	HIP_TRY(hipMemcpy(&bad, Ws.p, 4, hipMemcpyDeviceToHost));
+	Fetch f;
+	if (f.add(&bad, Ws.p, 4) || f.add(out, O, out_n * 8) || f.wait())
+		return -1;
 	return bad ? 1 : 0;
 }
 
-static int dev_crossprod_sparse(const CscGuard &X, const svt_dev_csc *Y, bool sym, double *O, int64_t ldo, double dense_ops)
+static int dev_crossprod_sparse(const CscGuard &X, const svt_dev_csc *Y, bool sym, double *O, int64_t ldo, double dense_ops,
+				double *out, size_t out_n)
 {
 	if (X.h->nnz >= ((int64_t) 1 << 31))
 		return 1;
@@ -2186,13 +2443,13 @@
 		if (g_unsupported) { g_unsupported = 0; return 1; }
 		return -1;
 	}
-	return dev_crossprod_sparse_on(T.t, Y, sym, O, ldo, dense_ops);
+	return dev_crossprod_sparse_on(T.t, Y, sym, O, ldo, dense_ops, out, out_n);
 }
 
 static int dense_buffer_route(const svt_dev_csc *X, const svt_dev_csc *Y, bool sym, double *O)
 {
 	const int64_t nx = X->ncol, ny = Y->ncol;
-	HIP_TRY(hipMemset(O, 0, (size_t) nx * ny * 8));
+	HIP_TRY(hipMemsetAsync(O, 0, (size_t) nx * ny * 8, 0));
 	if (sym)
 		return dev_crossprod_pp(X, X, true, O, 1, nx) || launch_mirror_lower(O, nx, 0) ? -1 : 0;
 	if (Y->nnz * nx < X->nnz * ny)
@@ -2206,7 +2463,7 @@
 		return svt_set_error("svt_dev_crossprod_csc_csc_dense_buffer: non-conformable operands");
 	if (X->ncol == 0 || Y->ncol == 0) return 0;
 	if (dense_buffer_route(X, Y, X == Y, out)) return -1;
-	HIP_TRY(hipDeviceSynchronize());
+	HIP_BLOCK(hipDeviceSynchronize());
 	return 0;
 }
 
@@ -2218,7 +2475,7 @@
 	const int st = sparse(O.as<double>());
 	if (st < 0 || (st > 0 && dense(O.as<double>())))
 		return -1;
-	return staged_download(out, O.p, out_n * 8);
+	return st == 0 ? 0 : staged_download(out, O.p, out_n * 8);
 }
 
 static int64_t view_nzcount(const svt_view *x)
@@ -2253,7 +2510,7 @@
 	const bool pays = !x->svt_is_null && !y->svt_is_null &&
 			  sparse_route_pays(X.h->nnz, Y.h->nnz, in_nrow, dense_ops, false);
 	return sparse_then_dense(out, out_n,
-		[&](double *O) { return pays ? dev_crossprod_sparse(X, Y.h, false, O, out_nrow, dense_ops) : 1; },
+		[&](double *O) { return pays ? dev_crossprod_sparse(X, Y.h, false, O, out_nrow, dense_ops, out, out_n) : 1; },
 		[&](double *O) { return dense_buffer_route(X.h, Y.h, false, O); });
 }
 extern "C" int svt_crossprod2_SVT_SVT(const svt_view *x, const svt_view *y, double *out)
@@ -2261,18 +2518,16 @@
 	return abi_status([&] { return crossprod2_SVT_SVT_impl(x, y, out); });
 }
 
-static svt_dev_csc *dev_transposed(const svt_dev_csc *A)
+static svt_dev_csc *dev_transposed(const svt_dev_csc *A, bool pooled)
 {
 	svt_dev_csc *T = (svt_dev_csc *) calloc(1, sizeof(*T));
 	if (T == NULL) { svt_set_error("out of memory"); return NULL; }
-	T->Rtype = A->Rtype; T->owned = 1; T->na_background = A->na_background;
+	T->Rtype = A->Rtype; T->na_background = A->na_background;
 	T->nrow = A->ncol; T->ncol = A->nrow; T->nnz = A->nnz;
 	const size_t n = A->nnz > 0 ? (size_t) A->nnz : 1;
 	const int64_t box = box_nnz_get();
 	DevBuf ws;
-	if (hipMalloc((void **) &T->col_ptr, ((size_t) T->ncol + 1) * 8) != hipSuccess ||
-	    hipMalloc((void **) &T->row_idx, n * 4) != hipSuccess ||
-	    hipMalloc(&T->val, n * elt_size(A->Rtype)) != hipSuccess ||
+	if (csc_alloc(T, pooled, n, elt_size(A->Rtype)) ||
 	    ws.alloc(transpose_ws_bytes_box(A->nrow, A->nnz, box))) {
 		svt_set_error("device allocation failed (transposed operand)");
 		svt_release(T);
@@ -2280,7 +2535,7 @@
 	}
 	if (launch_transpose_box(A->col_ptr, A->row_idx, A->val, A->Rtype, A->nrow, A->ncol, A->nnz,
 				 T->col_ptr, T->row_idx, T->val, ws.p, box, 0) ||
-	    hipDeviceSynchronize() != hipSuccess) {
+	    (!pooled && (svt_note_host_block(), hipStreamSynchronize(0)) != hipSuccess)) {
 		if (svt_last_error()[0] == '\0') svt_set_error("device transposition failed");
 		svt_release(T);
 		return NULL;
@@ -2295,7 +2550,7 @@
 		for (Resident &r : g_res)
 			if (r.key == A.key && r.tr != NULL) return OwnedCsc(r.tr, false);
 	}
-	svt_dev_csc *T = dev_transposed(A.h);
+	svt_dev_csc *T = dev_transposed(A.h, A.key == 0);
 	if (T == NULL || A.key == 0) return OwnedCsc(T, true);
 	std::lock_guard<std::mutex> lk(g_res_mu);
 	const size_t nb = csc_bytes(T);
@@ -2326,13 +2581,12 @@
 	const OwnedCsc TA = transposed_for(A);
 	const svt_dev_csc *T = TA.t;
 	if (T == NULL) return -1;
-	HIP_TRY(hipMemcpy(out_col_ptr, T->col_ptr, (size_t) (nrow + 1) * 8, hipMemcpyDeviceToHost));
-	if (T->nnz > 0) {
-		if (staged_download(out_row_idx, T->row_idx, (size_t) T->nnz * 4) ||
-		    staged_download(out_val, T->val, (size_t) T->nnz * elt_size(T->Rtype)))
-			return -1;
-	}
-	return 0;
+	Fetch f;
+	if (f.add(out_col_ptr, T->col_ptr, (size_t) (nrow + 1) * 8) ||
+	    (T->nnz > 0 && (f.add(out_row_idx, T->row_idx, (size_t) T->nnz * 4) ||
+			    f.add(out_val, T->val, (size_t) T->nnz * elt_size(T->Rtype)))))
+		return -1;
+	return f.wait();
 }
 extern "C" int svt_transpose_2D_SVT(const svt_view *x, int64_t *out_col_ptr,
 				    int32_t *out_row_idx, void *out_val)
@@ -2393,7 +2647,7 @@
 	h->ncol = cols != NULL ? ncols_sel : A.h->ncol;
 	if (dev_subset_impl(A.h, dr.as<int32_t>(), rows != NULL ? nrows_sel : -1, dc.as<int32_t>(), cols != NULL ? ncols_sel : -1,
 			    subset_hip_alloc, subset_hip_free, NULL, &h->nnz, &h->col_ptr, &h->row_idx, &h->val, NULL) ||
-	    hipStreamSynchronize(0) != hipSuccess) {
+	    (svt_note_host_block(), hipStreamSynchronize(0)) != hipSuccess) {
 		if (svt_last_error()[0] == '\0') svt_set_error("device error while subsetting");
 		svt_release(h);
 		return -1;
@@ -2419,11 +2673,14 @@
 	if (out_col_ptr != NULL || out_row_idx != NULL || out_val != NULL) {
 		if (out_col_ptr == NULL || (h->nnz > 0 && (out_row_idx == NULL || out_val == NULL)))
 			rc = svt_set_error("svt_subset_SVT_end: all three outputs, or none");
-		else if (hipMemcpy(out_col_ptr, h->col_ptr, ((size_t) h->ncol + 1) * 8, hipMemcpyDeviceToHost) != hipSuccess)
-			rc = svt_set_error("svt_subset_SVT_end: D2H copy failed");
-		else if (h->nnz > 0 && (staged_download(out_row_idx, h->row_idx, (size_t) h->nnz * 4) ||
-					staged_download(out_val, h->val, (size_t) h->nnz * elt_size(h->Rtype))))
-			rc = -1;
+		else {
+			Fetch f;
+			if (f.add(out_col_ptr, h->col_ptr, ((size_t) h->ncol + 1) * 8) ||
+			    (h->nnz > 0 && (f.add(out_row_idx, h->row_idx, (size_t) h->nnz * 4) ||
+					    f.add(out_val, h->val, (size_t) h->nnz * elt_size(h->Rtype)))) ||
+			    f.wait())
+				rc = -1;
+		}
 	}
 	svt_release(res->h);
 	free(res);
@@ -2457,7 +2714,7 @@
 		if (O.alloc((size_t) rs * K * 8) || O.zero() ||
 		    dense_product(T.t, K, y_Rtype, y_elems, put_y, y_nrow, 0, O.as<double>(), 1, rs))
 			return -1;
-		HIP_TRY(hipMemcpy2D(out + r0, (size_t) nrow * 8, O.p, (size_t) rs * 8, (size_t) rs * 8, (size_t) K,
+		HIP_BLOCK(hipMemcpy2D(out + r0, (size_t) nrow * 8, O.p, (size_t) rs * 8, (size_t) rs * 8, (size_t) K,
 				    hipMemcpyDeviceToHost));
 		return 0;
 	});
@@ -2529,9 +2786,11 @@
 		if (rc_s < 0)
 			return -1;
 		if (rc_s == 0) {
-			HIP_TRY(hipMemcpy(&bad, (char *) Ws.p + 4, 4, hipMemcpyDeviceToHost));
+			Fetch f;
+			if (f.add(&bad, (char *) Ws.p + 4, 4) || f.add(out, Os.p, out_n * 8) || f.wait())
+				return -1;
 			if (!bad)
-				return staged_download(out, Os.p, out_n * 8) ? -1 : 0;
+				return 0;
 		} else
 			g_unsupported = 0;
 	}
@@ -2560,7 +2819,7 @@
 	const double dense_ops = (double) X.h->nnz * (double) n;
 	const bool pays = sparse_route_pays(X.h->nnz, X.h->nnz, x->dim[0], dense_ops, true);
 	return sparse_then_dense(out, out_n,
-		[&](double *O) { return pays ? dev_crossprod_sparse(X, X.h, true, O, n, dense_ops) : 1; },
+		[&](double *O) { return pays ? dev_crossprod_sparse(X, X.h, true, O, n, dense_ops, out, out_n) : 1; },
 		[&](double *O) { return dense_buffer_route(X.h, X.h, true, O); });
 }
 extern "C" int svt_crossprod1_SVT(const svt_view *x, double *out)
@@ -2585,7 +2844,7 @@
 	const double dense_ops = (double) M->nnz * (double) n;
 	const bool pays = sparse_route_pays(M->nnz, M->nnz, M->nrow, dense_ops, true);
 	return sparse_then_dense(out, out_n,
-		[&](double *O) { return pays ? dev_crossprod_sparse_on(X.h, M, true, O, n, dense_ops) : 1; },
+		[&](double *O) { return pays ? dev_crossprod_sparse_on(X.h, M, true, O, n, dense_ops, out, out_n) : 1; },
 		[&](double *O) { return dense_buffer_route(M, M, true, O); });
 }
 extern "C" int svt_tcrossprod1_SVT(const svt_view *x, double *out)
@@ -2618,7 +2877,7 @@
 	const bool pays = !x->svt_is_null && !y->svt_is_null && x->dim[1] > 0 &&
 			  sparse_route_pays(X.h->nnz, Y.h->nnz, x->dim[1], dense_ops, false);
 	return sparse_then_dense(out, out_n,
-		[&](double *O) { return pays ? dev_crossprod_sparse_on(X.h, Ty.t, false, O, out_nrow, dense_ops) : 1; },
+		[&](double *O) { return pays ? dev_crossprod_sparse_on(X.h, Ty.t, false, O, out_nrow, dense_ops, out, out_n) : 1; },
 		[&](double *O) {
 			const OwnedCsc Tx = transposed_for(X);
 			return Tx.t == NULL ? -1 : dense_buffer_route(Tx.t, Ty.t, false, O);
@@ -2640,8 +2899,9 @@
 	if (svt_dev_colstats(A, opcode, na_rm, center, inner, O.p, W.as<int>(), 0))
 		return -1;
 	int w = 0;
-	HIP_TRY(hipMemcpy(out_host, O.p, (size_t) nseg * osz, hipMemcpyDeviceToHost));
-	HIP_TRY(hipMemcpy(&w, W.p, 4, hipMemcpyDeviceToHost));
+	Fetch f;
+	if (f.add(out_host, O.p, (size_t) nseg * osz) || f.add(&w, W.p, 4) || f.wait())
+		return -1;
 	if (w) *warn = 1;
 	return 0;
 }
@@ -2657,7 +2917,7 @@
 		if (u1 <= u0) return 0;
 		SubView sv;
 		col_block_view(x, u0 * unit, u1 * unit, sv);
-		CscGuard A(svt_upload(&sv.v));
+		CscGuard A(upload_csc(&sv.v, true));
 		if (A.h == NULL) return -1;
 		return fn(A.h, u0, &f[(size_t) s]);
 	});
@@ -2745,7 +3005,6 @@
 	if (launch_order_stat(what, M->col_ptr, M->val, M->Rtype, M->nrow, nout, M->nnz, P.as<double>(), nprobs, constant,
 			      na_rm, O.as<double>(), W.p, 0))
 		return -1;
-	HIP_TRY(hipDeviceSynchronize());
 	return staged_download(out, O.p, out_bytes);
 }
 
@@ -2830,8 +3089,8 @@
 		return svt_set_unsupported("colRanks: more than 2^31-1 columns");
 	std::vector<int64_t> cp((size_t) mcol + 1);
 	std::vector<int32_t> ri((size_t) nnz);
-	HIP_TRY(hipMemcpy(cp.data(), M->col_ptr, cp.size() * 8, hipMemcpyDeviceToHost));
-	if (nnz > 0 && staged_download(ri.data(), M->row_idx, (size_t) nnz * 4))
+	Fetch f;
+	if (f.add(cp.data(), M->col_ptr, cp.size() * 8) || f.add(ri.data(), M->row_idx, (size_t) nnz * 4) || f.wait())
 		return -1;
 	int64_t long_nnz = 0;
 	for (int64_t j = 0; j < mcol; j++)
@@ -2845,14 +3104,12 @@
 		return -1;
 	if (launch_ranks(M->col_ptr, M->val, M->Rtype, mrow, mcol, nnz, ties, RN.p, RZ.p, F.as<int>(), W.p, wsb, 0))
 		return -1;
-	HIP_TRY(hipDeviceSynchronize());
 	int flag = 0;
-	HIP_TRY(hipMemcpy(&flag, F.p, sizeof(int), hipMemcpyDeviceToHost));
+	std::vector<char> rn((size_t) nnz * esz), rz((size_t) mcol * esz);
+	if (f.add(&flag, F.p, sizeof(int)) || f.add(rn.data(), RN.p, rn.size()) || f.add(rz.data(), RZ.p, rz.size()) || f.wait())
+		return -1;
 	if (flag)
 		return svt_set_error("colRanks: the workspace did not hold the long columns");
-	std::vector<char> rn((size_t) nnz * esz), rz((size_t) mcol * esz);
-	if ((nnz > 0 && staged_download(rn.data(), RN.p, rn.size())) || staged_download(rz.data(), RZ.p, rz.size()))
-		return -1;
 	const bool transposed = by_row || !preserve_shape;
 	if (esz == 8)
 		expand_ranks<double>(cp.data(), ri.data(), (const double *) rn.data(), (const double *) rz.data(), mrow, mcol,
@@ -2969,13 +3226,12 @@
 		DevBuf T;
 		if (T.alloc(rowstats_panel_ws_bytes(a.nrow, a.ncol)) || launch_rowstats_panel(a, T.p, 0))
 			return -1;
-		HIP_TRY(hipDeviceSynchronize());
 	} else if (launch_rowstats(a, 0)) {
 		return -1;
 	}
 	int w = 0;
-	if (staged_download(out, O.p, (size_t) out_len * osz)) return -1;
-	HIP_TRY(hipMemcpy(&w, W.p, 4, hipMemcpyDeviceToHost));
+	Fetch f;
+	if (f.add(out, O.p, (size_t) out_len * osz) || f.add(&w, W.p, 4) || f.wait()) return -1;
 	if (w) *warn = 1;
 	return 0;
 }
@@ -3031,10 +3287,9 @@
 	if (dev_rowstats_impl(A.h, opcode, na_rm, center ? C.as<double>() : NULL, inner, O.p, W.as<int>(), T.p,
 			      svt_dev_rowstats_ws_bytes_op(A.h, opcode, inner), 0))
 		return -1;
-	HIP_TRY(hipDeviceSynchronize());
 	int w = 0;
-	if (staged_download(out, O.p, (size_t) nout * osz)) return -1;
-	HIP_TRY(hipMemcpy(&w, W.p, 4, hipMemcpyDeviceToHost));
+	Fetch f;
+	if (f.add(out, O.p, (size_t) nout * osz) || f.add(&w, W.p, 4) || f.wait()) return -1;
 	if (w) *warn = 1;
 	return 0;
 }
@@ -3080,8 +3335,8 @@
 	a.scratch = S.p; a.ovflow_flag = W.as<int>();
 	if (colsum ? launch_colsum(a, 0) : launch_rowsum(a, 0)) return -1;
 	int w = 0;
-	if (staged_download(out, O.p, (size_t) out_len * osz)) return -1;
-	HIP_TRY(hipMemcpy(&w, W.p, 4, hipMemcpyDeviceToHost));
+	Fetch f;
+	if (f.add(out, O.p, (size_t) out_len * osz) || f.add(&w, W.p, 4) || f.wait()) return -1;
 	if (ovflow && w) *ovflow = 1;
 	return 0;
 }
@@ -3196,7 +3451,6 @@
 	default: rc = dev_colstats_ex(&A, SVT_OP_VAR1, na_rm, NA, 1, O.p, NULL, 0, 1); break;
 	}
 	if (rc) return -1;
-	HIP_TRY(hipDeviceSynchronize());
 	return staged_download(out, O.p, (size_t) ncol * 8 * (which == 2 ? 2 : 1));
 }
 
```

Result: no change. 57.66 (median of 2 runs) (+0.0%).
